# lukifer23/Matrix0

Hardware: AMD Instinct MI355X
Metric: self-play games/sec at 800 sims/move, ResNet-24 53M; 1/2/4/8 MI355X (higher is better)
Workload: dtype f16

## Files before the change

### include/m0_engine.h

```cpp
#ifndef M0_ENGINE_H
#define M0_ENGINE_H

#include <stdint.h>

#ifdef __cplusplus
extern "C" {
#endif

#define M0_OK 0
#define M0_ERR_INVALID (-1)
#define M0_ERR_UNSUPPORTED (-2)
#define M0_ERR_HIP (-3)
#define M0_ERR_STATE (-4)
#define M0_ERR_NONFINITE (-5)

#define M0_POLICY_SIZE 4672
#define M0_PLANES 19

#define M0_ACT_RELU 1
#define M0_ACT_SILU 2
#define M0_ACT_LEAKY 3

#define M0_SSL_PIECE 1
#define M0_SSL_THREAT 2
#define M0_SSL_PIN 4
#define M0_SSL_FORK 8
#define M0_SSL_CONTROL 16

typedef struct m0_net_cfg {
    int planes;
    int channels;
    int blocks;
    int attention;
    int attention_heads;
    int attention_every_k;
    int attention_relbias;
    float attention_unmasked_mix;
    int se;
    float se_ratio;
    int chess_features;
    int piece_square_tables;
    int policy_factor_rank;
    int norm_group;
    int activation;
    int value_activation;
    int preact;
    int self_supervised;
    int ssl_tasks;
    int infer_attention_stride;
} m0_net_cfg;

typedef struct m0_net m0_net;

const char* m0_last_error(void);
const char* m0_version(void);
int m0_device_count(void);

m0_net* m0_net_create(const m0_net_cfg* cfg, int hip_device);
void m0_net_destroy(m0_net* net);
int m0_net_load_weight(m0_net* net, const char* name, const void* data, int dtype, const int64_t* shape, int ndim);
int m0_net_finalize(m0_net* net);
int m0_net_infer(m0_net* net, const float* planes, int B, float* policy, float* value, float* ssl);
int m0_net_ssl_channels(const m0_net* net);
int64_t m0_net_param_count(const m0_net* net);
double m0_net_flops_per_position(const m0_net* net, int with_ssl);
int m0_net_bench_forward(m0_net* net, int B, int iters, int with_ssl, float* ms_per_forward);
int m0_net_profile_enable(m0_net* net, int on);
int m0_net_profile_get(m0_net* net, double* conv_ms, double* conv_flop, int64_t* launches, int reset);
int m0_net_profile_get_tail(m0_net* net, double* tail_ms, int64_t* tail_launches);


typedef struct m0_dist m0_dist;
int m0_dist_unique_id(void* id128);
m0_dist* m0_dist_create(int rank, int world, const void* id128, int hip_device);
void m0_dist_destroy(m0_dist* d);
int m0_dist_rank(const m0_dist* d);
int m0_dist_world(const m0_dist* d);
int m0_net_broadcast_weights(m0_net* net, m0_dist* d, int root);

int m0_encode_fens(int hip_device, const char* const* fens, int n, float* planes, uint8_t* mask, int32_t* nlegal,
                   uint16_t* moves, int32_t* idx);
int m0_encode_fens_nhwc(int hip_device, const char* const* fens, int n, uint16_t* nhwc);
int m0_decode_move_fen(int hip_device, const char* fen, int action_idx, char* uci_out);
int m0_ssl_targets_fens(int hip_device, const char* const* fens, int n, float* out);
int m0_move_to_index_fen(int hip_device, const char* fen, const char* uci, int32_t* idx);

typedef struct m0_selfplay_cfg {
    int num_simulations;
    double cpuct, cpuct_start, cpuct_end;
    int cpuct_plies;
    int use_c_base; double cpuct_c_base, cpuct_c_init;
    double dirichlet_alpha, dirichlet_frac;
    int dirichlet_plies;
    double selection_jitter, fpu_reduction, draw_penalty, virtual_loss;
    int legal_softmax, enable_entropy_noise, no_instant_backtrack, value_from_white;
    int inference_batch_size;
    double playout_random_frac;
    int max_game_len, min_resign_plies, opening_random_plies;
    double resign_threshold; int resign_window, resign_consecutive_bad; double resign_min_entropy, resign_value_margin;
    double temperature_start, temperature_end; int temperature_moves;
    int low_visit_threshold;
    int draw_enabled, draw_min_plies, draw_window, draw_min_unique, draw_halfmove_cap, draw_material_threshold, draw_stalemate;
    int concurrent_games;
    int total_games;
    int first_game_index;
    int arena_nodes;
    uint64_t seed;
    int virtual_loss_active;
    int ssl_in_forward;
    int ssl_targets;
    int record_games;
    int arena_mode;
    double arena_temp;
    int arena_temp_plies;
    int fresh_tree_per_move;
    int tt_merge;
    int raw_legal_priors;
    int max_children;
    double min_child_prior;
    int root_reinfer;
    int eval_cache;
    int eval_cache_entries;
    int tail_split;
    int arena_eval_cache;
    int arena_paired_openings;
} m0_selfplay_cfg;

typedef struct m0_selfplay m0_selfplay;

typedef struct m0_selfplay_stats {
    uint64_t steps, evals, sims, plies, games_finished, games_started;
    double ms_total, ms_net, ms_tree, ms_host;
    uint64_t arena_overflows;
    uint64_t ssl_dropped;
    uint64_t evals_cached;
    int active_games;
    uint64_t rows_tail;
} m0_selfplay_stats;

typedef struct m0_game_record {
    int game_index, moves, resigned, resigner , draw, total_plies ;
    float result;
    float avg_policy_entropy, avg_sims;
    double secs;
    const float* s;
    const float* pi;
    const float* z;
    const uint8_t* legal_mask;
    const float* search_values;
    const uint16_t* played;
    const float* ssl;
    void* owner;
    const char* start_fen;
} m0_game_record;

m0_selfplay* m0_selfplay_create(m0_net* net, const m0_selfplay_cfg* cfg);
void m0_selfplay_destroy(m0_selfplay* sp);
int m0_selfplay_step(m0_selfplay* sp, int steps);
int m0_selfplay_stats_get(m0_selfplay* sp, m0_selfplay_stats* out);
int m0_selfplay_poll(m0_selfplay* sp, m0_game_record* out);
void m0_game_record_free(m0_game_record* rec);
int m0_selfplay_running(m0_selfplay* sp);
int m0_selfplay_set_openings(m0_selfplay* sp, const char* const* fens, int n);
int m0_selfplay_ext_select(m0_selfplay* sp, int* rows, float* planes, int max_rows);
int m0_selfplay_ext_expand(m0_selfplay* sp, const float* logits, const float* values, int rows);
int m0_selfplay_last_batch_nhwc(m0_selfplay* sp, uint16_t* nhwc, int max_rows, int* rows);

m0_selfplay* m0_arena_create(m0_net* net_a, m0_net* net_b, const m0_selfplay_cfg* cfg);
m0_selfplay* m0_arena_create_ext(const m0_selfplay_cfg* cfg);
int m0_arena_ext_select(m0_selfplay* sp, int* rows_a, int* rows_b, float* planes_a, float* planes_b, int max_rows);
int m0_arena_ext_expand(m0_selfplay* sp, const float* logits_a, const float* values_a, int rows_a, const float* logits_b,
                        const float* values_b, int rows_b);
int m0_arena_choose_move(const int32_t* visits, int n, double temp, int ply, int temp_plies, double u);
int m0_san_legal_fen(const char* fen, uint16_t* moves, char* san, int* nlegal);
int m0_san_game(const uint16_t* moves, int n, char* out, int cap);
int m0_san_game_fen(const char* fen, const uint16_t* moves, int n, char* out, int cap);
int m0_fen_after(const char* fen, const char* const* ucis, int n, char* fen_out, int cap);

int m0_search_begin(m0_selfplay* sp, int g, const char* fen, int sims, int dirichlet, int game_uid);
int m0_search_select(m0_selfplay* sp, int* rows, float* planes, int max_rows);
int m0_search_expand(m0_selfplay* sp, const float* logits, const float* values, int rows);
int m0_search_result(m0_selfplay* sp, int g, int* nchild, int32_t* child_n, uint16_t* child_mv, int32_t* child_idx,
                     double* child_prior, double* child_q, double* root_q, int* root_n, int* finished);
int m0_search_advance(m0_selfplay* sp, int g, int slot, int sims, int dirichlet);

int m0_sample_move_index(const int32_t* visits, int n, double temperature, double u);
int m0_playout_cap(int sims, double frac, double u);
double m0_temperature_for(int fullmove_number, double t_start, double t_end, int t_moves);
int m0_rules_probe(const m0_selfplay_cfg* cfg, const char* fen, const char* const* ucis, int n, int* flags, float* result);

#ifdef __cplusplus
}
#endif
#endif
```

### matrix0_amd/csrc/capi_net.hip

```cpp
#include <hip/hip_runtime.h>
#include <math.h>
#include <string.h>
#include <mutex>
#include <string>
#include <vector>
#include "../../include/m0_engine.h"
#include "net.h"
#include "capi_common.h"

thread_local std::string g_m0_last_error;

void m0_set_error(const std::string& s) { g_m0_last_error = s; }

struct m0_net {
    Net* net = nullptr;
    int device = 0;
    hipStream_t stream = nullptr;
    std::mutex mu;
    float* planes_dev = nullptr;
    float* logits_dev = nullptr;
    float* value_dev = nullptr;
    float* ssl_dev = nullptr;
    int cap = 0;
};

Net* m0_net_impl(m0_net* n) { return n ? n->net : nullptr; }
hipStream_t m0_net_stream(m0_net* n) { return n ? n->stream : nullptr; }
int m0_net_device(m0_net* n) { return n ? n->device : 0; }
void m0_net_lock(m0_net* n) { if (n) n->mu.lock(); }
void m0_net_unlock(m0_net* n) { if (n) n->mu.unlock(); }

hipError_t create_stream_cu_mask_env(const char* env_name, hipStream_t* stream) {
    const char* mk = getenv(env_name);
    if (!mk || !*mk) return hipStreamCreateWithFlags(stream, hipStreamNonBlocking);
    uint32_t words[8] = {0, 0, 0, 0, 0, 0, 0, 0};
    int nw = 0;
    for (const char* q = mk; *q && nw < 8; ++nw) {
        char* end = nullptr;
        words[nw] = (uint32_t)strtoul(q, &end, 16);
        if (end == q) break;
        q = (*end == ',') ? end + 1 : end;
    }
    return hipExtStreamCreateWithCUMask(stream, 8, words);
}

extern "C" {

const char* m0_last_error(void) { return g_m0_last_error.c_str(); }
const char* m0_version(void) { return "m0engine 0.2 (gfx950)"; }
int m0_device_count(void) {
    int n = 0;
    if (hipGetDeviceCount(&n) != hipSuccess) { (void)hipGetLastError(); return 0; }
    return n;
}

m0_net* m0_net_create(const m0_net_cfg* cfg, int hip_device) {
    if (!cfg) { m0_set_error("cfg is null"); return nullptr; }
    const char* why = Net::check_supported(*cfg);
    if (why) { m0_set_error(std::string("unsupported network config: ") + why); return nullptr; }
    int ndev = 0;
    if (hipGetDeviceCount(&ndev) != hipSuccess || ndev <= 0) {
        m0_set_error("no HIP device available (the engine has no CPU fallback)");
        return nullptr;
    }
    if (hip_device < 0 || hip_device >= ndev) { m0_set_error("hip_device out of range"); return nullptr; }
    if (hipSetDevice(hip_device) != hipSuccess) { m0_set_error("hipSetDevice failed"); return nullptr; }
    m0_net* h = new m0_net();
    h->device = hip_device;
    const hipError_t se = create_stream_cu_mask_env("M0_NET_CU_MASK", &h->stream);
    if (se != hipSuccess) {
        m0_set_error("hipStreamCreate failed");
        delete h;
        return nullptr;
    }
    h->net = new Net(*cfg, hip_device, h->stream);
    return h;
}

void m0_net_destroy(m0_net* n) {
    if (!n) return;
    (void)hipSetDevice(n->device);
    if (n->stream) { (void)hipStreamSynchronize(n->stream); }
    if (n->planes_dev) (void)hipFree(n->planes_dev);
    if (n->logits_dev) (void)hipFree(n->logits_dev);
    if (n->value_dev) (void)hipFree(n->value_dev);
    if (n->ssl_dev) (void)hipFree(n->ssl_dev);
    delete n->net;
    if (n->stream) (void)hipStreamDestroy(n->stream);
    delete n;
}

int m0_net_load_weight(m0_net* n, const char* name, const void* data, int dtype, const int64_t* shape, int ndim) {
    if (!n) { m0_set_error("net is null"); return M0_ERR_INVALID; }
    std::lock_guard<std::mutex> lk(n->mu);
    std::string err;
    int rc = n->net->load(name, data, dtype, shape, ndim, err);
    if (rc != M0_OK) m0_set_error(err);
    return rc;
}

int m0_net_finalize(m0_net* n) {
    if (!n) { m0_set_error("net is null"); return M0_ERR_INVALID; }
    std::lock_guard<std::mutex> lk(n->mu);
    std::string err;
    int rc = n->net->finalize(err);
    if (rc != M0_OK) m0_set_error(err);
    return rc;
}

static int ensure_io(m0_net* n, int B) {
    if (B <= n->cap) return M0_OK;
    if (n->planes_dev) (void)hipFree(n->planes_dev);
    if (n->logits_dev) (void)hipFree(n->logits_dev);
    if (n->value_dev) (void)hipFree(n->value_dev);
    if (n->ssl_dev) (void)hipFree(n->ssl_dev);
    n->planes_dev = n->logits_dev = n->value_dev = n->ssl_dev = nullptr;
    n->cap = 0;
    int cap = B < 64 ? 64 : B;
    const int P = n->net->cfg().planes;
    int sslc = n->net->ssl_channels_total();
    if (hipMalloc((void**)&n->planes_dev, (size_t)cap * P * 64 * 4) != hipSuccess ||
        hipMalloc((void**)&n->logits_dev, (size_t)cap * M0_POLICY_SIZE * 4) != hipSuccess ||
        hipMalloc((void**)&n->value_dev, (size_t)cap * 4) != hipSuccess ||
        hipMalloc((void**)&n->ssl_dev, (size_t)cap * (sslc > 0 ? sslc : 1) * 64 * 4) != hipSuccess) {
        m0_set_error("hipMalloc failed for I/O staging");
        return M0_ERR_HIP;
    }
    n->cap = cap;
    return M0_OK;
}

int m0_net_infer(m0_net* n, const float* planes, int B, float* policy, float* value, float* ssl) {
    if (!n || !planes || !policy || !value) { m0_set_error("null argument"); return M0_ERR_INVALID; }
    if (B <= 0) { m0_set_error("batch must be positive"); return M0_ERR_INVALID; }
    std::lock_guard<std::mutex> lk(n->mu);
    if (hipSetDevice(n->device) != hipSuccess) { m0_set_error("hipSetDevice failed"); return M0_ERR_HIP; }
    int rc = ensure_io(n, B);
    if (rc != M0_OK) return rc;
    const int P = n->net->cfg().planes;
    const int sslc = n->net->ssl_channels_total();
    if (ssl && sslc == 0) { m0_set_error("ssl output requested but the net has no SSL heads"); return M0_ERR_INVALID; }
    std::string err;
    hipError_t e = hipMemcpyAsync(n->planes_dev, planes, (size_t)B * P * 64 * 4, hipMemcpyHostToDevice, n->stream);
    if (e != hipSuccess) { m0_set_error(std::string("H2D copy: ") + hipGetErrorString(e)); return M0_ERR_HIP; }
    rc = n->net->forward(n->planes_dev, nullptr, B, n->logits_dev, n->value_dev, ssl ? n->ssl_dev : nullptr, n->stream, err);
    if (rc != M0_OK) { m0_set_error(err); return rc; }
    (void)hipMemcpyAsync(policy, n->logits_dev, (size_t)B * M0_POLICY_SIZE * 4, hipMemcpyDeviceToHost, n->stream);
    (void)hipMemcpyAsync(value, n->value_dev, (size_t)B * 4, hipMemcpyDeviceToHost, n->stream);
    if (ssl) (void)hipMemcpyAsync(ssl, n->ssl_dev, (size_t)B * sslc * 64 * 4, hipMemcpyDeviceToHost, n->stream);
    e = hipStreamSynchronize(n->stream);
    if (e != hipSuccess) { m0_set_error(std::string("forward failed: ") + hipGetErrorString(e)); return M0_ERR_HIP; }
    for (size_t i = 0, nn = (size_t)B * M0_POLICY_SIZE; i < nn; ++i)
        if (!isfinite(policy[i])) { m0_set_error("network produced non-finite policy logits"); return M0_ERR_NONFINITE; }
    for (int i = 0; i < B; ++i)
        if (!isfinite(value[i])) { m0_set_error("network produced non-finite value"); return M0_ERR_NONFINITE; }
    return M0_OK;
}

int m0_net_ssl_channels(const m0_net* n) { return n ? n->net->ssl_channels_total() : 0; }
int64_t m0_net_param_count(const m0_net* n) { return n ? (int64_t)n->net->param_count() : 0; }
double m0_net_flops_per_position(const m0_net* n, int with_ssl) { return n ? n->net->flops_per_position(with_ssl != 0) : 0.0; }

int m0_net_profile_enable(m0_net* n, int on) {
    if (!n) { m0_set_error("net is null"); return M0_ERR_INVALID; }
    std::lock_guard<std::mutex> lk(n->mu);
    n->net->set_profile(on != 0);
    return M0_OK;
}

int m0_net_profile_get(m0_net* n, double* conv_ms, double* conv_flop, int64_t* launches, int reset) {
    if (!n) { m0_set_error("net is null"); return M0_ERR_INVALID; }
    std::lock_guard<std::mutex> lk(n->mu);
    if (conv_ms) *conv_ms = n->net->prof_conv_ms();
    if (conv_flop) *conv_flop = n->net->prof_conv_flop();
    if (launches) *launches = n->net->prof_conv_launches();
    if (reset) n->net->reset_profile();
    return M0_OK;
}

int m0_net_profile_get_tail(m0_net* n, double* tail_ms, int64_t* tail_launches) {
    if (!n) { m0_set_error("net is null"); return M0_ERR_INVALID; }
    std::lock_guard<std::mutex> lk(n->mu);
    if (tail_ms) *tail_ms = n->net->prof_tail_ms();
    if (tail_launches) *tail_launches = n->net->prof_tail_launches();
    return M0_OK;
}

int m0_net_bench_forward(m0_net* n, int B, int iters, int with_ssl, float* ms_per_forward) {
    if (!n || !ms_per_forward || B <= 0 || iters <= 0) { m0_set_error("invalid argument"); return M0_ERR_INVALID; }
    std::lock_guard<std::mutex> lk(n->mu);
    if (hipSetDevice(n->device) != hipSuccess) { m0_set_error("hipSetDevice failed"); return M0_ERR_HIP; }
    int rc = ensure_io(n, B);
    if (rc != M0_OK) return rc;
    std::string err;
    if (!(with_ssl & 2)) {
        const int P = n->net->cfg().planes;
        std::vector<float> h((size_t)B * P * 64, 0.f);
        uint64_t s = 0x9E3779B97F4A7C15ull;
        for (size_t i = 0; i < h.size(); ++i) {
            s ^= s << 13; s ^= s >> 7; s ^= s << 17;
            int p = (int)((i / 64) % P);
            if (p < 12) h[i] = ((s >> 20) % 100) < 8 ? 1.f : 0.f;
            else h[i] = (float)((((i / 64 / P) * 7 + p) % 10) / 10.0);
        }
        (void)hipMemcpy(n->planes_dev, h.data(), h.size() * 4, hipMemcpyHostToDevice);
    }
    float* ssl = ((with_ssl & 1) && n->net->ssl_channels_total() > 0) ? n->ssl_dev : nullptr;
    rc = n->net->forward(n->planes_dev, nullptr, B, n->logits_dev, n->value_dev, ssl, n->stream, err);
    if (rc != M0_OK) { m0_set_error(err); return rc; }
    hipEvent_t e0, e1;
    (void)hipEventCreate(&e0); (void)hipEventCreate(&e1);
    (void)hipEventRecord(e0, n->stream);
    for (int i = 0; i < iters; ++i) {
        rc = n->net->forward(n->planes_dev, nullptr, B, n->logits_dev, n->value_dev, ssl, n->stream, err);
        if (rc != M0_OK) { m0_set_error(err); return rc; }
    }
    (void)hipEventRecord(e1, n->stream);
    hipError_t e = hipEventSynchronize(e1);
    if (e != hipSuccess) { m0_set_error(std::string("bench forward failed: ") + hipGetErrorString(e)); return M0_ERR_HIP; }
    float ms = 0.f;
    (void)hipEventElapsedTime(&ms, e0, e1);
    (void)hipEventDestroy(e0); (void)hipEventDestroy(e1);
    *ms_per_forward = ms / iters;
    n->net->harvest_profile();
    return M0_OK;
}

}
```

### matrix0_amd/csrc/capi_selfplay.hip

```cpp
#include <string.h>
#include <algorithm>
#include <memory>
#include "selfplay_engine.h"

using namespace m0;

static void fill_tree_cfg(const m0_selfplay_cfg& c, bool arena, TreeCfg& t) {
    t.fpu_reduction = c.fpu_reduction; t.draw_penalty = c.draw_penalty; t.virtual_loss = c.virtual_loss;
    t.selection_jitter = c.selection_jitter; t.cpuct = c.cpuct; t.cpuct_start = c.cpuct_start; t.cpuct_end = c.cpuct_end;
    t.cpuct_plies = c.cpuct_plies; t.use_c_base = c.use_c_base; t.cpuct_c_base = c.cpuct_c_base; t.cpuct_c_init = c.cpuct_c_init;
    t.dirichlet_alpha = c.dirichlet_alpha; t.dirichlet_frac = c.dirichlet_frac; t.legal_softmax = c.legal_softmax;
    t.enable_entropy_noise = c.enable_entropy_noise; t.no_instant_backtrack = c.no_instant_backtrack;
    t.virtual_loss_active = c.virtual_loss_active; t.leaves_per_step = c.inference_batch_size;
    t.tt_merge = c.tt_merge; t.raw_legal_priors = c.raw_legal_priors; t.max_children = c.max_children;
    t.min_child_prior = c.min_child_prior;
    t.eval_cache = ((arena ? c.arena_eval_cache : c.eval_cache) && c.legal_softmax && !c.raw_legal_priors && !c.tt_merge) ? 1 : 0;
}

static void alloc_tree_arenas(m0_selfplay* sp) {
    const m0_selfplay_cfg& c = sp->cfg;
    long want = c.arena_nodes > 0 ? c.arena_nodes : (long)(c.num_simulations * 1.3 + 64) * 96;
    if (want < 4096) want = 4096;
    sp->cap = (int)want;
    const size_t N = (size_t)sp->G * 2 * sp->cap;
    TreeArrays& t = sp->d.t;
    t.cap = sp->cap;
    t.prior = dalloc<double>(sp, N); t.w = dalloc<double>(sp, N); t.q = dalloc<double>(sp, N);
    t.n = dalloc<int>(sp, N); t.vl = dalloc<int>(sp, N); t.cbase = dalloc<int>(sp, N);
    t.nch = dalloc<int16_t>(sp, N); t.mv = dalloc<uint16_t>(sp, N); t.midx = dalloc<uint16_t>(sp, N);
    sp->d.games = dalloc<GameDev>(sp, sp->G);
    const size_t LS = (size_t)sp->L + 1;
    sp->d.samples = dalloc<Sample>(sp, (size_t)sp->G * LS);
    sp->d.paths = dalloc<int>(sp, (size_t)sp->G * LS * M0_MAX_DEPTH);
    sp->d.leaf_moves = dalloc<uint16_t>(sp, (size_t)sp->G * LS * M0_MAX_CHILDREN);
}

static bool alloc_position_tables(m0_selfplay* sp) {
    sp->d.tt_sides = 1;
    if (!sp->cfg.tt_merge) return true;
    const size_t LS = (size_t)sp->L + 1;
    int tc = 1024;
    while (tc < 2 * sp->cap) tc <<= 1;
    sp->d.tt_cap = tc;
    sp->d.tt_sides = sp->cfg.arena_mode ? 2 : 1;
    sp->d.search_nodes = (int)std::min<long>((long)sp->cfg.num_simulations * 48 + 4 * M0_MAX_CHILDREN, (long)sp->cap / 2);
    sp->d.epaths = dalloc<int>(sp, (size_t)sp->G * LS * M0_MAX_DEPTH);
    sp->d.tt_keys = dalloc<uint64_t>(sp, (size_t)sp->G * sp->d.tt_sides * tc);
    sp->d.tt_nodes = dalloc<int>(sp, (size_t)sp->G * sp->d.tt_sides * tc);
    if (sp->d.epaths && sp->d.tt_keys && sp->d.tt_nodes) return true;
    m0_set_error("hipMalloc failed for the position tables (tt_merge): lower concurrent_games or arena_nodes");
    return false;
}

static bool alloc_eval_cache(m0_selfplay* sp) {
    if (!sp->tc.eval_cache) return true;
    const size_t LS = (size_t)sp->L + 1;
    int entries = sp->cfg.eval_cache_entries > 0 ? sp->cfg.eval_cache_entries : 16384;
    int sets = 64;
    while (sets * 4 < entries) sets <<= 1;
    EvalCache& ec = sp->d.ec;
    ec.sets = sets;
    ec.sides = sp->cfg.arena_mode ? 2 : 1;
    const size_t entries_all = (size_t)sp->G * ec.sides * sets * 4;
    ec.keys = dalloc<uint64_t>(sp, entries_all);
    ec.stamps = dalloc<uint32_t>(sp, entries_all);
    ec.payload = dalloc<float>(sp, entries_all * M0_EC_WORDS);
    ec.hit_stage = dalloc<float>(sp, (size_t)sp->G * LS * M0_EC_WORDS);
    if (ec.keys && ec.stamps && ec.payload && ec.hit_stage) return true;
    m0_set_error("hipMalloc failed for the evaluation cache: lower eval_cache_entries or concurrent_games");
    return false;
}

static bool alloc_batch_buffers(m0_selfplay* sp) {
    const int nreg = sp->cfg.arena_mode ? 2 : 1;
    sp->d.hist = dalloc<uint64_t>(sp, (size_t)sp->G * M0_HIST_CAP);
    sp->d.results = dalloc<RootResult>(sp, sp->G);
    sp->d.row_counter = dalloc<int>(sp, 4);
    sp->d.x0 = dalloc<_Float16>(sp, (size_t)(nreg * sp->rows_max + 4) * 64 * 32);
    sp->logits_dev = dalloc<float>(sp, (size_t)nreg * sp->rows_max * 4672);
    sp->values_dev = dalloc<float>(sp, (size_t)nreg * sp->rows_max + 4);
    sp->d.net_row_base = sp->rows_max;
    if (sp->cfg.ssl_in_forward && sp->net && sp->net->ssl_channels_total() > 0)
        sp->ssl_dev = dalloc<float>(sp, (size_t)sp->rows_max * sp->net->ssl_channels_total() * 64);
    if (sp->cfg.ssl_targets) {
        sp->ssl_cap = sp->cfg.max_game_len > 0 ? sp->cfg.max_game_len + 1 : 513;
        sp->ssl_pos_dev = dalloc<Pos>(sp, sp->ssl_cap);
        sp->ssl_out_dev = dalloc<float>(sp, (size_t)sp->ssl_cap * 17 * 64);
        if (!sp->ssl_pos_dev || !sp->ssl_out_dev) {
            m0_set_error("hipMalloc failed for the SSL target staging buffers");
            return false;
        }
    }
    sp->ids_dev = dalloc<int>(sp, sp->G);
    sp->slots_dev = dalloc<int>(sp, sp->G);
    sp->d.logits = sp->logits_dev; sp->d.values = sp->values_dev;
    sp->d.G = sp->G; sp->d.L = sp->L;
    return true;
}

static bool make_tail_view(m0_selfplay* sp) {
    if (!(sp->cfg.tail_split && sp->net && !sp->cfg.arena_mode && sp->net->cfg().channels > 256 && sp->net->cfg().channels <= 320 &&
          sp->rows_max >= 2048)) return true;
    if (create_stream_cu_mask_env("M0_TAIL_CU_MASK", &sp->stream_tail) != hipSuccess ||
        hipEventCreateWithFlags(&sp->ev_sel, hipEventDisableTiming) != hipSuccess ||
        hipEventCreateWithFlags(&sp->ev_tail, hipEventDisableTiming) != hipSuccess) {
        m0_set_error("hipStreamCreate / hipEventCreate failed (tail split)");
        return false;
    }
    sp->net_tail = sp->net->shared_view(sp->stream_tail);
    std::string werr;
    sp->half_split = sp->cfg.tail_split == 2;
    if (sp->net_tail->ensure_workspace(sp->half_split ? sp->rows_max / 2 + 1024 : 1023, werr) != M0_OK) {
        m0_set_error("tail split: " + werr);
        return false;
    }
    return true;
}

static bool build_engine(m0_selfplay* sp) {
    alloc_tree_arenas(sp);
    if (!alloc_position_tables(sp) || !alloc_eval_cache(sp) || !alloc_batch_buffers(sp)) return false;
    if (sp->alloc_failed) {
        m0_set_error("hipMalloc failed for the search arenas (lower concurrent_games or arena_nodes)");
        return false;
    }
    sp->hg.assign(sp->G, GameDev());
    for (auto& g : sp->hg) memset(&g, 0, sizeof(GameDev));
    sp->games.assign(sp->G, HostGame());
    sp->hres.resize(sp->G);
    sp->hsamples.resize((size_t)sp->G * (sp->L + 1));
    sp->prev_done.assign(sp->G, 0);
    (void)hipEventCreate(&sp->ev0); (void)hipEventCreate(&sp->ev1); (void)hipEventCreate(&sp->ev2); (void)hipEventCreate(&sp->ev3);
    if (!make_tail_view(sp)) return false;
    std::string err;
    if (sp->net && sp->net->ensure_workspace(sp->rows_max, err) != M0_OK) { m0_set_error(err); return false; }
    if (sp->net && sp->net_b && sp->net_b->ensure_workspace(sp->rows_max, err) != M0_OK) { m0_set_error(err); return false; }
    if (hipStreamSynchronize(sp->stream) != hipSuccess) {
        m0_set_error(std::string("clearing the search arenas failed: ") + hipGetErrorString(hipGetLastError()));
        return false;
    }
    return true;
}

extern "C" {

static m0_selfplay* selfplay_create_impl(m0_net* nh, m0_net* nh_b, const m0_selfplay_cfg* cfg, bool arena = false) {
    if (!cfg) { m0_set_error("cfg is null"); return nullptr; }
    if (cfg->concurrent_games <= 0 || cfg->inference_batch_size <= 0 || cfg->num_simulations <= 0) {
        m0_set_error("concurrent_games, inference_batch_size and num_simulations must be positive");
        return nullptr;
    }
    int ndev = 0;
    if (hipGetDeviceCount(&ndev) != hipSuccess || ndev <= 0) { m0_set_error("no HIP device available (no CPU fallback)"); return nullptr; }
    std::unique_ptr<m0_selfplay, decltype(&m0_selfplay_destroy)> owner(new m0_selfplay(), &m0_selfplay_destroy);
    m0_selfplay* sp = owner.get();
    sp->cfg = *cfg;
    sp->nethandle = nh;
    sp->nethandle_b = nh_b;
    sp->net = m0_net_impl(nh);
    sp->net_b = m0_net_impl(nh_b);
    sp->cfg.arena_mode = (nh_b || arena) ? 1 : 0;
    if (sp->cfg.arena_mode) sp->cfg.eval_cache = 0;
    else { sp->cfg.arena_eval_cache = 0; sp->cfg.arena_paired_openings = 0; }
    fill_tree_cfg(sp->cfg, sp->cfg.arena_mode != 0, sp->tc);
    sp->device = nh ? m0_net_device(nh) : 0;
    if (nh) forward_gate_join(sp);
    (void)hipSetDevice(sp->device);
    if (nh) sp->stream = m0_net_stream(nh);
    else { (void)hipStreamCreateWithFlags(&sp->stream, hipStreamNonBlocking); sp->own_stream = true; }
    sp->G = cfg->concurrent_games;
    sp->L = cfg->inference_batch_size;
    sp->rows_max = (sp->G * (sp->L + 1) + 3) & ~3;
    memset(&sp->stats, 0, sizeof(sp->stats));
    memset(&sp->d, 0, sizeof(sp->d));
    return build_engine(sp) ? owner.release() : nullptr;
}

m0_selfplay* m0_selfplay_create(m0_net* nh, const m0_selfplay_cfg* cfg) { return selfplay_create_impl(nh, nullptr, cfg); }

m0_selfplay* m0_arena_create(m0_net* net_a, m0_net* net_b, const m0_selfplay_cfg* cfg) {
    if (!net_a || !net_b) { m0_set_error("m0_arena_create needs two networks"); return nullptr; }
    if (m0_net_device(net_a) != m0_net_device(net_b)) { m0_set_error("both networks must live on the same HIP device"); return nullptr; }
    if (cfg && (cfg->ssl_in_forward || cfg->ssl_targets)) { m0_set_error("arena games carry no SSL outputs"); return nullptr; }
    return selfplay_create_impl(net_a, net_b, cfg);
}

m0_selfplay* m0_arena_create_ext(const m0_selfplay_cfg* cfg) {
    if (cfg && (cfg->ssl_in_forward || cfg->ssl_targets)) { m0_set_error("arena games carry no SSL outputs"); return nullptr; }
    return selfplay_create_impl(nullptr, nullptr, cfg, true);
}

void m0_selfplay_destroy(m0_selfplay* sp) {
    if (!sp) return;
    forward_gate_leave(sp);
    (void)hipSetDevice(sp->device);
    if (sp->stream) (void)hipStreamSynchronize(sp->stream);
    if (sp->stream_tail) (void)hipStreamSynchronize(sp->stream_tail);
    delete sp->net_tail;
    if (sp->ev_sel) (void)hipEventDestroy(sp->ev_sel);
    if (sp->ev_tail) (void)hipEventDestroy(sp->ev_tail);
    if (sp->stream_tail) (void)hipStreamDestroy(sp->stream_tail);
    for (void* p : sp->allocs) (void)hipFree(p);
    for (auto& r : sp->done_meta) delete (GameRecordOwner*)r.owner;
    if (sp->ev0) { (void)hipEventDestroy(sp->ev0); (void)hipEventDestroy(sp->ev1); (void)hipEventDestroy(sp->ev2); (void)hipEventDestroy(sp->ev3); }
    if (sp->own_stream && sp->stream) (void)hipStreamDestroy(sp->stream);
    delete sp;
}

int m0_selfplay_set_openings(m0_selfplay* sp, const char* const* fens, int n) {
    if (!sp || n < 0 || (n > 0 && !fens)) { m0_set_error("invalid argument"); return M0_ERR_INVALID; }
    std::lock_guard<std::mutex> lk(sp->mu);
    if (sp->stats.games_started != 0) { m0_set_error("set the opening book before the first step"); return M0_ERR_STATE; }
    std::vector<Pos> book(n);
    for (int i = 0; i < n; ++i)
        if (!fens[i] || parse_fen(fens[i], book[i]) != 0) { m0_set_error(std::string("bad FEN at index ") + std::to_string(i)); return M0_ERR_INVALID; }
    sp->book.swap(book);
    sp->book_fens.assign(fens, fens + n);
    return M0_OK;
}

static int leaf_planes(m0_selfplay* sp, int rows_a, float* planes_a, int rows_b, float* planes_b) {
    if (sync_games_d2h(sp) != 0) { m0_set_error("device sync failed"); return M0_ERR_HIP; }
    (void)hipMemcpy(sp->hsamples.data(), sp->d.samples, sizeof(Sample) * (size_t)sp->G * (sp->L + 1), hipMemcpyDeviceToHost);
    const int base = sp->d.net_row_base;
    for (int g = 0; g < sp->G; ++g) {
        if (!sp->hg[g].active) continue;
        for (int s = 0; s < sp->hg[g].nsamples; ++s) {
            const Sample& smp = sp->hsamples[(size_t)g * (sp->L + 1) + s];
            if (!sample_owns_row(smp.kind) || smp.row < 0) continue;
            if (smp.row < rows_a) encode_planes_f32(smp.pos, planes_a + (size_t)smp.row * 19 * 64);
            else if (smp.row >= base && smp.row < base + rows_b) encode_planes_f32(smp.pos, planes_b + (size_t)(smp.row - base) * 19 * 64);
        }
    }
    return M0_OK;
}

static void upload_eval(m0_selfplay* sp, size_t row_base, const float* logits, const float* values, int rows) {
    if (rows <= 0) return;
    (void)hipMemcpyAsync(sp->logits_dev + row_base * 4672, logits, (size_t)rows * 4672 * 4, hipMemcpyHostToDevice, sp->stream);
    (void)hipMemcpyAsync(sp->values_dev + row_base, values, (size_t)rows * 4, hipMemcpyHostToDevice, sp->stream);
}

static int ext_select_impl(m0_selfplay* sp, int* rows_a, int* rows_b, float* planes_a, float* planes_b, int max_rows) {
    (void)hipSetDevice(sp->device);
    if (sp->ext_pending) { m0_set_error("m0_selfplay_ext_expand outstanding"); return M0_ERR_STATE; }
    if (!planes_a || (sp->cfg.arena_mode && !planes_b) || max_rows < sp->G * (sp->L + 1)) {
        m0_set_error("planes buffer too small: concurrent_games * (inference_batch_size + 1) rows are required");
        return M0_ERR_INVALID;
    }
    int rc = start_first_games(sp);
    if (rc != M0_OK) return rc;
    int r = 0;
    if (run_select(sp, &r) != 0) { m0_set_error(std::string("select failed: ") + hipGetErrorString(hipGetLastError())); return M0_ERR_HIP; }
    const int rb = sp->cfg.arena_mode ? sp->rows2[1] : 0;
    if (r > sp->rows_max || rb > sp->rows_max) { m0_set_error("row counter overflow"); return M0_ERR_STATE; }
    *rows_a = r;
    if (rows_b) *rows_b = rb;
    sp->last_rows = r;
    sp->last_rows_b = rb;
    sp->ext_pending = true;
    if (r + rb > 0) return leaf_planes(sp, r, planes_a, rb, planes_b);
    return M0_OK;
}

static int ext_expand_impl(m0_selfplay* sp, const float* logits_a, const float* values_a, int rows_a, const float* logits_b,
                           const float* values_b, int rows_b) {
    (void)hipSetDevice(sp->device);
    if (!sp->ext_pending) { m0_set_error("no m0_selfplay_ext_select outstanding"); return M0_ERR_STATE; }
    if (rows_a != sp->last_rows || rows_b != sp->last_rows_b) { m0_set_error("rows does not match the last select"); return M0_ERR_INVALID; }
    if ((rows_a > 0 && (!logits_a || !values_a)) || (rows_b > 0 && (!logits_b || !values_b))) { m0_set_error("null argument"); return M0_ERR_INVALID; }
    upload_eval(sp, 0, logits_a, values_a, rows_a);
    upload_eval(sp, (size_t)sp->d.net_row_base, logits_b, values_b, rows_b);
    sp->ext_pending = false;
    std::string err;
    (void)hipEventRecord(sp->ev0, sp->stream); (void)hipEventRecord(sp->ev1, sp->stream);
    int rc = step_back(sp, rows_a + rows_b, now_ms(), err);
    if (rc != M0_OK) m0_set_error(err);
    return rc;
}

int m0_selfplay_ext_select(m0_selfplay* sp, int* rows, float* planes, int max_rows) {
    if (!sp || !rows) { m0_set_error("null argument"); return M0_ERR_INVALID; }
    std::lock_guard<std::mutex> lk(sp->mu);
    if (sp->cfg.arena_mode) { m0_set_error("a match engine has two evaluators: use m0_arena_ext_select"); return M0_ERR_STATE; }
    return ext_select_impl(sp, rows, nullptr, planes, nullptr, max_rows);
}

int m0_selfplay_ext_expand(m0_selfplay* sp, const float* logits, const float* values, int rows) {
    if (!sp) { m0_set_error("null argument"); return M0_ERR_INVALID; }
    std::lock_guard<std::mutex> lk(sp->mu);
    if (sp->cfg.arena_mode) { m0_set_error("a match engine has two evaluators: use m0_arena_ext_expand"); return M0_ERR_STATE; }
    return ext_expand_impl(sp, logits, values, rows, nullptr, nullptr, 0);
}

int m0_arena_ext_select(m0_selfplay* sp, int* rows_a, int* rows_b, float* planes_a, float* planes_b, int max_rows) {
    if (!sp || !rows_a || !rows_b) { m0_set_error("null argument"); return M0_ERR_INVALID; }
    std::lock_guard<std::mutex> lk(sp->mu);
    if (!sp->cfg.arena_mode) { m0_set_error("not a match engine"); return M0_ERR_STATE; }
    return ext_select_impl(sp, rows_a, rows_b, planes_a, planes_b, max_rows);
}

int m0_arena_ext_expand(m0_selfplay* sp, const float* logits_a, const float* values_a, int rows_a, const float* logits_b,
                        const float* values_b, int rows_b) {
    if (!sp) { m0_set_error("null argument"); return M0_ERR_INVALID; }
    std::lock_guard<std::mutex> lk(sp->mu);
    if (!sp->cfg.arena_mode) { m0_set_error("not a match engine"); return M0_ERR_STATE; }
    return ext_expand_impl(sp, logits_a, values_a, rows_a, logits_b, values_b, rows_b);
}

int m0_selfplay_step(m0_selfplay* sp, int steps) {
    if (!sp) { m0_set_error("sp is null"); return M0_ERR_INVALID; }
    std::lock_guard<std::mutex> lk(sp->mu);
    (void)hipSetDevice(sp->device);
    std::string err;
    if (sp->ext_pending) { m0_set_error("m0_selfplay_ext_expand outstanding"); return M0_ERR_STATE; }
    { int rc0 = start_first_games(sp); if (rc0 != M0_OK) return rc0; }
    for (int i = 0; i < steps; ++i) {
        if (sp->stats.active_games == 0 && sp->stats.steps > 0) break;
        int rc = one_step(sp, err);
        if (rc != M0_OK) { m0_set_error(err); return rc; }
    }
    return M0_OK;
}

int m0_selfplay_stats_get(m0_selfplay* sp, m0_selfplay_stats* out) {
    if (!sp || !out) { m0_set_error("null argument"); return M0_ERR_INVALID; }
    std::lock_guard<std::mutex> lk(sp->mu);
    *out = sp->stats;
    return M0_OK;
}

int m0_selfplay_poll(m0_selfplay* sp, m0_game_record* out) {
    if (!sp || !out) { m0_set_error("null argument"); return M0_ERR_INVALID; }
    std::lock_guard<std::mutex> lk(sp->mu);
    if (sp->done_meta.empty()) return 0;
    *out = sp->done_meta.front();
    sp->done_meta.pop_front();
    return 1;
}

void m0_game_record_free(m0_game_record* rec) {
    if (rec && rec->owner) { delete (GameRecordOwner*)rec->owner; rec->owner = nullptr; }
}

int m0_selfplay_running(m0_selfplay* sp) {
    if (!sp) return 0;
    std::lock_guard<std::mutex> lk(sp->mu);
    if (sp->stats.games_started == 0) return 1;
    if (sp->stats.active_games > 0) return 1;
    return (sp->cfg.total_games <= 0 || sp->next_game < sp->cfg.total_games) ? 1 : 0;
}

int m0_search_begin(m0_selfplay* sp, int g, const char* fen, int sims, int dirichlet, int game_uid) {
    if (!sp || !fen || g < 0 || g >= sp->G || sims <= 0) { m0_set_error("invalid argument"); return M0_ERR_INVALID; }
    std::lock_guard<std::mutex> lk(sp->mu);
    (void)hipSetDevice(sp->device);
    Pos p;
    if (parse_fen(fen, p) != 0) { m0_set_error("bad FEN"); return M0_ERR_INVALID; }
    if (sync_games_d2h(sp) != 0) { m0_set_error("device sync failed"); return M0_ERR_HIP; }
    HostGame& hgm = sp->games[g];
    hgm = HostGame();
    hgm.in_use = true; hgm.pos = p; hgm.game_index = game_uid;
    seed_game_dev(sp->hg[g], sp->cfg.seed, game_uid);
    sp->hg[g].evals = 0;
    arm_search(sp, g, p, hgm.win, sims, dirichlet != 0, true);
    std::vector<int> ids{g}, slots{-1};
    if (apply_advances(sp, ids, slots) != 0) { m0_set_error("advance failed"); return M0_ERR_HIP; }
    return M0_OK;
}

int m0_search_select(m0_selfplay* sp, int* rows, float* planes, int max_rows) {
    if (!sp || !rows) { m0_set_error("null argument"); return M0_ERR_INVALID; }
    std::lock_guard<std::mutex> lk(sp->mu);
    (void)hipSetDevice(sp->device);
    int r = 0;
    if (run_select(sp, &r) != 0) { m0_set_error(std::string("select failed: ") + hipGetErrorString(hipGetLastError())); return M0_ERR_HIP; }
    *rows = r;
    sp->last_rows = r;
    if (planes && r > 0) {
        if (r > max_rows) { m0_set_error("planes buffer too small"); return M0_ERR_INVALID; }
        return leaf_planes(sp, r, planes, 0, nullptr);
    }
    return M0_OK;
}

int m0_search_expand(m0_selfplay* sp, const float* logits, const float* values, int rows) {
    if (!sp) { m0_set_error("null argument"); return M0_ERR_INVALID; }
    std::lock_guard<std::mutex> lk(sp->mu);
    (void)hipSetDevice(sp->device);
    if (rows != sp->last_rows || rows > sp->rows_max) { m0_set_error("rows does not match the last select"); return M0_ERR_INVALID; }
    if (rows > 0 && (!logits || !values)) { m0_set_error("null argument"); return M0_ERR_INVALID; }
    upload_eval(sp, 0, logits, values, rows);
    if (launch_expand(sp->d, sp->tc, sp->stream) != hipSuccess) { m0_set_error("expand launch failed"); return M0_ERR_HIP; }
    if (sync_games_d2h(sp) != 0) { m0_set_error(std::string("expand failed: ") + hipGetErrorString(hipGetLastError())); return M0_ERR_HIP; }
    sp->stats.evals += (uint64_t)rows;
    return M0_OK;
}

int m0_search_result(m0_selfplay* sp, int g, int* nchild, int32_t* child_n, uint16_t* child_mv, int32_t* child_idx,
                     double* child_prior, double* child_q, double* root_q, int* root_n, int* finished) {
    if (!sp || g < 0 || g >= sp->G) { m0_set_error("invalid argument"); return M0_ERR_INVALID; }
    std::lock_guard<std::mutex> lk(sp->mu);
    (void)hipSetDevice(sp->device);
    if (finished) *finished = sp->hg[g].finished;
    if (!sp->hg[g].finished) { if (nchild) *nchild = 0; return M0_OK; }
    (void)hipMemcpy(&sp->hres[g], sp->d.results + g, sizeof(RootResult), hipMemcpyDeviceToHost);
    const RootResult& R = sp->hres[g];
    if (nchild) *nchild = R.nchild;
    for (int i = 0; i < R.nchild; ++i) {
        if (child_n) child_n[i] = R.child_n[i];
        if (child_mv) child_mv[i] = R.child_mv[i];
        if (child_idx) child_idx[i] = R.child_idx[i];
        if (child_prior) child_prior[i] = R.child_prior[i];
        if (child_q) child_q[i] = R.child_q[i];
    }
    if (root_q) *root_q = R.root_n > 0 ? R.root_q : sp->hg[g].root_v;
    if (root_n) *root_n = R.root_n;
    return M0_OK;
}

int m0_search_advance(m0_selfplay* sp, int g, int slot, int sims, int dirichlet) {
    if (!sp || g < 0 || g >= sp->G || sims <= 0) { m0_set_error("invalid argument"); return M0_ERR_INVALID; }
    std::lock_guard<std::mutex> lk(sp->mu);
    (void)hipSetDevice(sp->device);
    if (sync_games_d2h(sp) != 0) { m0_set_error("device sync failed"); return M0_ERR_HIP; }
    if (!sp->hg[g].finished) { m0_set_error("search not finished"); return M0_ERR_STATE; }
    (void)hipMemcpy(&sp->hres[g], sp->d.results + g, sizeof(RootResult), hipMemcpyDeviceToHost);
    const RootResult& R = sp->hres[g];
    if (slot < 0 || slot >= R.nchild) { m0_set_error("child slot out of range"); return M0_ERR_INVALID; }
    HostGame& hgm = sp->games[g];
    hgm.play(R.child_mv[slot]);
    const bool fresh = sp->cfg.fresh_tree_per_move || sp->cfg.tt_merge;
    arm_search(sp, g, hgm.pos, hgm.win, sims, dirichlet != 0, fresh);
    std::vector<int> ids{g}, slots{fresh ? -1 : slot};
    if (apply_advances(sp, ids, slots) != 0) { m0_set_error("advance failed"); return M0_ERR_HIP; }
    return M0_OK;
}

int m0_selfplay_last_batch_nhwc(m0_selfplay* sp, uint16_t* out, int max_rows, int* rows) {
    if (!sp || !out || !rows) { m0_set_error("null argument"); return M0_ERR_INVALID; }
    std::lock_guard<std::mutex> lk(sp->mu);
    (void)hipSetDevice(sp->device);
    const int r = sp->last_rows;
    if (r > max_rows) { m0_set_error("output buffer too small"); return M0_ERR_INVALID; }
    *rows = r;
    if (r > 0) {
        if (hipMemcpyAsync(out, sp->d.x0, (size_t)r * 64 * 32 * 2, hipMemcpyDeviceToHost, sp->stream) != hipSuccess ||
            hipStreamSynchronize(sp->stream) != hipSuccess) { m0_set_error("copy failed"); return M0_ERR_HIP; }
    }
    return M0_OK;
}

}
```

### matrix0_amd/csrc/net.h

```cpp
#pragma once
#include <hip/hip_runtime.h>
#include <stdint.h>
#include <map>
#include <string>
#include <vector>
#include "../../include/m0_engine.h"
#include "net_kernels.h"

struct HostTensor {
    std::vector<float> data;
    std::vector<int64_t> shape;
};

struct PackedGemm {
    _Float16* w = nullptr;
    float* bias = nullptr;
    int taps = 1, Cin = 0, N = 0;
    bool pp = false;
};

struct NormParams {
    float* gamma = nullptr;
    float* beta = nullptr;
};

struct ResBlockW {
    PackedGemm conv1, conv2;
    NormParams bn1, bn2;
    float *se_w1 = nullptr, *se_b1 = nullptr, *se_w2 = nullptr, *se_b2 = nullptr;
    void* se_wf = nullptr;
    int se_hidden = 0;
};

struct AttnW {
    PackedGemm qkv, proj;
    NormParams ln;
    float* rel_bias = nullptr;
    void* blk_w = nullptr;
    _Float16* blk_bias = nullptr;
};

struct TowerLayer {
    int kind;
    int index;
    bool skip;
    int next_bn1 = -1;
};

struct SslHeadW {
    PackedGemm c0, c1;
    NormParams n;
    int out_ch = 0;
};

struct ConvNormOpts {
    const float* posenc = nullptr;
    const _Float16* res = nullptr;
    const NormParams* next_bn1 = nullptr;
};

class Net {
public:
    explicit Net(const m0_net_cfg& cfg, int device, hipStream_t stream);
    ~Net();
    Net* shared_view(hipStream_t stream) const;
    static const char* check_supported(const m0_net_cfg& cfg);
    int load(const char* name, const void* data, int dtype, const int64_t* shape, int ndim, std::string& err);
    int finalize(std::string& err);
    bool ready() const { return finalized_; }
    const std::vector<void*>& device_buffers() const { return dev_allocs_; }
    const std::vector<size_t>& device_buffer_bytes() const { return dev_sizes_; }

    int forward(const float* planes_dev, const _Float16* nhwc_dev, int B, float* logits_dev, float* value_dev,
                float* ssl_dev, hipStream_t st, std::string& err);
    int ensure_workspace(int B, std::string& err);
    int ssl_channels_total() const;
    const m0_net_cfg& cfg() const { return cfg_; }
    size_t param_count() const { return nparams_; }
    double flops_per_position(bool with_ssl) const;
    _Float16* input_nhwc() { return X0_; }
    void set_profile(bool on) { profile_ = on; }
    void harvest_profile();
    double prof_conv_ms() const { return prof_ms_; }
    double prof_conv_flop() const { return prof_flop_; }
    long prof_conv_launches() const { return prof_launches_; }
    void reset_profile() { prof_ms_ = 0; prof_flop_ = 0; prof_launches_ = 0; prof_tail_ms_ = 0; prof_tail_launches_ = 0; }
    double prof_tail_ms() const { return prof_tail_ms_; }
    long prof_tail_launches() const { return prof_tail_launches_; }

private:
    m0_net_cfg cfg_;
    int device_;
    hipStream_t stream_ = nullptr;
    struct Switches { bool fuse_tail = true, fuse_attn = true; } sw_;
    struct Plan {
        bool fuse_tail = false;
        bool fuse_attn = false;
        bool gn_small = false;
        int act = 0, vact = 0;
        int first_bn1 = -1;
    } plan_;
    bool finalized_ = false;
    size_t nparams_ = 0;
    std::map<std::string, HostTensor> sd_;
    std::vector<void*> dev_allocs_;
    std::vector<size_t> dev_sizes_;
    std::vector<void*> ws_allocs_;

    int C_ = 0, Cs_ = 0 ;
    int Cp_ = 0;
    PackedGemm stem_;
    NormParams stem_n_;
    float* posenc_ = nullptr;
    PackedGemm pst_, inter_;
    NormParams pst_n_, inter_n_;
    std::vector<ResBlockW> res_;
    std::vector<AttnW> att_;
    std::vector<TowerLayer> tower_;
    PackedGemm ph_conv_, pfc1_, pfc2_;
    PackedGemm hv_;
    NormParams hv_n_;
    NormParams ph_n_;
    float logit_scale_ = 1.f;
    PackedGemm vh0_, vh3_, vfc1_, vfc2_, vgate_, vfc3_;
    NormParams vh1_n_, vh4_n_;
    std::vector<SslHeadW> ssl_;
    uint64_t* mask_dev_ = nullptr;

    bool profile_ = false;
    std::vector<hipEvent_t> pev_;
    std::vector<double> pflop_;
    std::vector<char> ptail_;
    size_t pev_used_ = 0;
    double prof_ms_ = 0, prof_flop_ = 0, prof_tail_ms_ = 0;
    long prof_launches_ = 0, prof_tail_launches_ = 0;

    int wsB_ = 0, wsM_ = 0;
    _Float16 *X0_ = nullptr, *XA_ = nullptr, *XB_ = nullptr, *T1_ = nullptr, *T2_ = nullptr, *QKV_ = nullptr,
             *O_ = nullptr, *AA_ = nullptr;
    float *S1_ = nullptr, *S2_ = nullptr, *G_ = nullptr;
    _Float16 *PH_ = nullptr, *PH2_ = nullptr, *VH_ = nullptr, *VH2_ = nullptr, *F1_ = nullptr, *F2_ = nullptr,
             *F3_ = nullptr, *F4_ = nullptr, *SH_ = nullptr, *SH2_ = nullptr, *SO_ = nullptr;
    float* VAL_ = nullptr;
    float* SPK_ = nullptr;

    const HostTensor* get(const std::string& k, std::string& err);
    int pack_gemm(PackedGemm& g, const std::string& wkey, const std::string& bkey, int taps, int Cin_real,
                  int Cin_pad, int N_real, int N_pad, int k_perm_ch, std::string& err, int qkv_heads = 0,
                  int qkv_heads_pad = 0);
    int pack_attn_block(AttnW& a, const std::string& prefix, std::string& err);
    int pack_chess_features(std::string& err);
    int pack_se(ResBlockW& r, const std::string& prefix, std::string& err);
    int pack_attn(AttnW& a, bool skip, const std::string& prefix, std::string& err);
    void upload_attn_mask();
    int pack_joint_head(std::string& err);
    int pack_ssl_heads(std::string& err);
    void make_plan();
    int upload_norm(NormParams& n, const std::string& prefix, int C_real, int C_pad, std::string& err);
    float* upload_f32(const std::vector<float>& v);
    void* dalloc(size_t bytes, bool ws);
    const NormParams* bn1(int res_index) const { return res_index < 0 ? nullptr : &res_[res_index].bn1; }
    template <class Launch>
    hipError_t profiled(bool on, hipStream_t st, double flop, bool tail, Launch&& launch);
    hipError_t run_gemm(const PackedGemm& g, GemmArgs a, hipStream_t st);
    hipError_t conv_norm_act(const PackedGemm& g, const NormParams& n, const _Float16* in, _Float16* out, _Float16* scratch,
                             int Mrows, hipStream_t st, const ConvNormOpts& o = ConvNormOpts());
    hipError_t se_gate(const ResBlockW& r, const float* stats, int boards, hipStream_t st);
};
```

### matrix0_amd/csrc/net.hip

```cpp
#include "net.h"
#include <math.h>
#include <string.h>
#include <algorithm>
#include <stdlib.h>

static inline int ceil_to(int v, int m) { return (v + m - 1) / m * m; }

static const char* kSslNames[5] = {"piece", "threat", "pin", "fork", "control"};
static const int kSslOut[5] = {13, 1, 1, 1, 3};

const char* Net::check_supported(const m0_net_cfg& c) {
    if (!c.norm_group) return "HIP path supports norm='group' only (BatchNorm configs are not built)";
    if (!c.preact) return "HIP path supports preact=true only";
    if (c.channels % 32 != 0 || c.channels < 32 || c.channels > 384) return "channels must be a multiple of 32 in [32,384]";
    if (c.planes < 1 || c.planes > 32) return "planes must be in [1,32]";
    if (c.attention && (c.attention_heads <= 0 || c.channels % c.attention_heads != 0 ||
                        c.channels / c.attention_heads != 16))
        return "attention head_dim (channels/attention_heads) must be 16";
    if (c.activation != M0_ACT_SILU && c.activation != M0_ACT_RELU) return "activation must be silu or relu";
    if (c.blocks < 1) return "blocks must be >= 1";
    if (c.policy_factor_rank < 0) return "policy_factor_rank must be >= 0";
    if (c.self_supervised && c.ssl_tasks && (c.channels / 2) % 16 != 0) return "ssl heads need channels/2 % 16 == 0";
    return nullptr;
}

Net::Net(const m0_net_cfg& cfg, int device, hipStream_t stream) : cfg_(cfg), device_(device), stream_(stream) {
    auto off = [](const char* name) { const char* e = getenv(name); return e && e[0] == '0'; };
    sw_.fuse_tail = !off("M0_FUSE_TAIL");
    sw_.fuse_attn = !off("M0_FUSE_ATTN");
    C_ = cfg.channels;
    Cp_ = (C_ > 256 && C_ < 320) ? 320 : C_;
    Cs_ = ceil_to(std::max(16, C_ / 2), 32);
    int k = cfg.attention_every_k;
    int stride = std::max(1, cfg.infer_attention_stride);
    int att_seen = 0;
    for (int i = 0; i < cfg.blocks; ++i) {
        tower_.push_back({0, (int)res_.size(), false});
        res_.emplace_back();
        if (cfg.attention && k > 0 && (i % k) == (k - 1)) {
            ++att_seen;
            bool skip = stride > 1 && (att_seen % stride) != 0;
            tower_.push_back({1, (int)att_.size(), skip});
            att_.emplace_back();
        }
    }
}

Net* Net::shared_view(hipStream_t stream) const {
    Net* v = new Net(*this);
    v->stream_ = stream;
    v->dev_allocs_.clear(); v->dev_sizes_.clear();
    v->ws_allocs_.clear(); v->wsB_ = 0; v->wsM_ = 0;
    v->sd_.clear();
    v->pev_.clear(); v->pflop_.clear(); v->ptail_.clear(); v->pev_used_ = 0; v->profile_ = false;
    v->prof_ms_ = v->prof_flop_ = v->prof_tail_ms_ = 0; v->prof_launches_ = v->prof_tail_launches_ = 0;
    return v;
}

Net::~Net() {
    for (hipEvent_t e : pev_) (void)hipEventDestroy(e);
    for (void* p : dev_allocs_) (void)hipFree(p);
    for (void* p : ws_allocs_) (void)hipFree(p);
}

void* Net::dalloc(size_t bytes, bool ws) {
    void* p = nullptr;
    if (bytes == 0) bytes = 16;
    if (hipMalloc(&p, bytes) != hipSuccess) return nullptr;
    (void)hipMemsetAsync(p, 0, bytes, stream_);
    if (!ws) (void)hipStreamSynchronize(stream_);
    (ws ? ws_allocs_ : dev_allocs_).push_back(p);
    if (!ws) dev_sizes_.push_back(bytes);
    return p;
}

float* Net::upload_f32(const std::vector<float>& v) {
    float* d = (float*)dalloc(v.size() * 4, false);
    if (d && !v.empty()) (void)hipMemcpy(d, v.data(), v.size() * 4, hipMemcpyHostToDevice);
    return d;
}

int Net::load(const char* name, const void* data, int dtype, const int64_t* shape, int ndim, std::string& err) {
    if (finalized_) { err = "weights already finalized"; return M0_ERR_STATE; }
    if (!name || (!data && ndim >= 0)) { err = "null argument"; return M0_ERR_INVALID; }
    HostTensor t;
    size_t n = 1;
    for (int i = 0; i < ndim; ++i) { t.shape.push_back(shape[i]); n *= (size_t)shape[i]; }
    t.data.resize(n);
    if (dtype == 0) memcpy(t.data.data(), data, n * 4);
    else if (dtype == 1) {
        const _Float16* h = (const _Float16*)data;
        for (size_t i = 0; i < n; ++i) t.data[i] = (float)h[i];
    } else { err = "dtype must be 0 (f32) or 1 (f16)"; return M0_ERR_INVALID; }
    std::string key(name);
    if (cfg_.policy_factor_rank > 0 && key.rfind("policy_fc.", 0) == 0) key = "policy_fc1." + key.substr(10);
    sd_[key] = std::move(t);
    return M0_OK;
}

const HostTensor* Net::get(const std::string& k, std::string& err) {
    auto it = sd_.find(k);
    if (it == sd_.end()) { err = "missing state-dict key: " + k; return nullptr; }
    return &it->second;
}

int Net::pack_gemm(PackedGemm& g, const std::string& wkey, const std::string& bkey, int taps, int Cin_real,
                   int Cin_pad, int N_real, int N_pad, int k_perm_ch, std::string& err, int qkv_heads, int qkv_heads_pad) {
    const HostTensor* w = get(wkey, err);
    if (!w) return M0_ERR_INVALID;
    size_t expect = (size_t)N_real * Cin_real * taps;
    if (w->data.size() != expect) { err = "shape mismatch for " + wkey; return M0_ERR_INVALID; }
    nparams_ += expect;
    const int KC = conv_gemm_kc(Cin_pad, N_pad);
    const int nchunk = Cin_pad / KC;
    const bool pp = KC == 64 && taps == 9;
    const int nblk = N_pad / 320;
    std::vector<_Float16> p((size_t)taps * Cin_pad * N_pad, (_Float16)0.f);
    for (int nr = 0; nr < N_real; ++nr)
        for (int k = 0; k < Cin_real; ++k)
            for (int t = 0; t < taps; ++t) {
                float v = w->data[((size_t)nr * Cin_real + k) * taps + t];
                int n = nr;
                if (qkv_heads > 0) {
                    const int d = nr % 16, th = nr / 16, hh = th % qkv_heads, tt = th / qkv_heads;
                    n = (tt * qkv_heads_pad + hh) * 16 + d;
                }
                int kk = k;
                if (k_perm_ch > 0) {
                    int c = k / 64, sq = k % 64;
                    kk = sq * k_perm_ch + c;
                }
                int chunk = kk / KC, kc = kk % KC;
                if (pp) {
                    const int kt = chunk * 9 + t, by = n / 320, nl = n % 320, h = kc >> 5, k32 = kc & 31;
                    const int kx = (((k32 >> 3) ^ ((4 - ((nl >> 2) & 3)) & 3)) << 3) | (k32 & 7);
                    p[((((size_t)kt * nblk + by) * 2 + h) * 320 + nl) * 32 + kx] = (_Float16)v;
                    continue;
                }
                if (KC == 64)
                    kc = (((kc >> 3) ^ ((n >> 1) & 7)) << 3) | (kc & 7);
                p[(((size_t)t * nchunk + chunk) * N_pad + n) * KC + kc] = (_Float16)v;
            }
    g.w = (_Float16*)dalloc(p.size() * 2, false);
    if (!g.w) { err = "hipMalloc failed"; return M0_ERR_HIP; }
    (void)hipMemcpy(g.w, p.data(), p.size() * 2, hipMemcpyHostToDevice);
    g.taps = taps; g.Cin = Cin_pad; g.N = N_pad; g.pp = pp;
    g.bias = nullptr;
    if (!bkey.empty()) {
        const HostTensor* b = get(bkey, err);
        if (!b) return M0_ERR_INVALID;
        if ((int)b->data.size() != N_real) { err = "shape mismatch for " + bkey; return M0_ERR_INVALID; }
        nparams_ += N_real;
        std::vector<float> bp(N_pad, 0.f);
        std::copy(b->data.begin(), b->data.end(), bp.begin());
        g.bias = upload_f32(bp);
    }
    return M0_OK;
}

int Net::pack_attn_block(AttnW& a, const std::string& prefix, std::string& err) {
    const HostTensor* wq = get(prefix + ".qkv.weight", err); if (!wq) return M0_ERR_INVALID;
    const HostTensor* wp = get(prefix + ".proj.weight", err); if (!wp) return M0_ERR_INVALID;
    const int Cr = C_, Hr = cfg_.attention_heads;
    if (Cp_ != 320 || Cr != Hr * 16 || wq->data.size() != (size_t)3 * Cr * Cr || wp->data.size() != (size_t)Cr * Cr) {
        err = "shape mismatch for " + prefix; return M0_ERR_INVALID;
    }
    std::vector<_Float16> buf(attn_block_pack_bytes() / 2, (_Float16)0.f);
    auto qkv_w = [&](int type, int h, int d, int k) -> float {
        return (h < Hr && k < Cr) ? wq->data[(size_t)((type * Hr + h) * 16 + d) * Cr + k] : 0.f;
    };
    auto proj_w = [&](int oc, int h, int d) -> float {
        return (oc < Cr && h < Hr) ? wp->data[(size_t)oc * Cr + h * 16 + d] : 0.f;
    };
    for (int g = 0; g < 10; ++g) {
        for (int pc = 0; pc < 5; ++pc) {
            const size_t base = (size_t)(g * 7 + pc) * 6144;
            for (int col = 0; col < 96; ++col) {
                const int J = col >> 4, type = J >> 1, hl = J & 1, d = col & 15;
                for (int k = 0; k < 64; ++k) {
                    const int pos = (k >> 3) ^ ((col >> 1) & 7);
                    buf[base + (size_t)col * 64 + pos * 8 + (k & 7)] = (_Float16)qkv_w(type, 2 * g + hl, d, 64 * pc + k);
                }
            }
        }
        for (int hh = 0; hh < 2; ++hh) {
            const size_t base = (size_t)(g * 7 + 5 + hh) * 6144;
            for (int cl = 0; cl < 160; ++cl)
                for (int k = 0; k < 32; ++k) {
                    const int pos = (k >> 3) ^ ((4 - ((cl >> 2) & 3)) & 3);
                    buf[base + (size_t)cl * 32 + pos * 8 + (k & 7)] = (_Float16)proj_w(160 * hh + cl, 2 * g + (k >> 4), k & 15);
                }
        }
    }
    a.blk_w = dalloc(buf.size() * 2, false);
    if (!a.blk_w) { err = "hipMalloc failed"; return M0_ERR_HIP; }
    (void)hipMemcpy(a.blk_w, buf.data(), buf.size() * 2, hipMemcpyHostToDevice);
    std::vector<_Float16> bb((size_t)20 * 2 * 64 * 32, (_Float16)0.f);
    if (cfg_.attention_relbias) {
        const HostTensor* rb = get(prefix + ".rel_bias", err); if (!rb) return M0_ERR_INVALID;
        for (int h = 0; h < Hr; ++h)
            for (int qt = 0; qt < 2; ++qt)
                for (int lane = 0; lane < 64; ++lane)
                    for (int e = 0; e < 32; ++e) {
                        const int kt = e >> 4, r = e & 15;
                        const int q = qt * 32 + (lane & 31), key = kt * 32 + 8 * (r >> 2) + 4 * (lane >> 5) + (r & 3);
                        bb[(((size_t)h * 2 + qt) * 64 + lane) * 32 + e] =
                            (_Float16)(rb->data[((size_t)h * 64 + q) * 64 + key] * 1.44269504088896f);
                    }
    }
    a.blk_bias = (_Float16*)dalloc(bb.size() * 2, false);
    if (!a.blk_bias) { err = "hipMalloc failed"; return M0_ERR_HIP; }
    (void)hipMemcpy(a.blk_bias, bb.data(), bb.size() * 2, hipMemcpyHostToDevice);
    return M0_OK;
}

int Net::upload_norm(NormParams& n, const std::string& prefix, int C_real, int C_pad, std::string& err) {
    const HostTensor* g = get(prefix + ".weight", err);
    if (!g) return M0_ERR_INVALID;
    const HostTensor* b = get(prefix + ".bias", err);
    if (!b) return M0_ERR_INVALID;
    if ((int)g->data.size() != C_real || (int)b->data.size() != C_real) { err = "shape mismatch for " + prefix; return M0_ERR_INVALID; }
    nparams_ += 2 * (size_t)C_real;
    std::vector<float> gp(C_pad, 0.f), bp(C_pad, 0.f);
    std::copy(g->data.begin(), g->data.end(), gp.begin());
    std::copy(b->data.begin(), b->data.end(), bp.begin());
    n.gamma = upload_f32(gp);
    n.beta = upload_f32(bp);
    return M0_OK;
}

#define TRY(x) do { int rc_ = (x); if (rc_ != M0_OK) return rc_; } while (0)

int Net::pack_chess_features(std::string& err) {
    const int C = C_, P = Cp_;
    const HostTensor* pe = get("chess_features.position_encoding", err);
    if (!pe) return M0_ERR_INVALID;
    if ((int)pe->data.size() != C * 64) { err = "shape mismatch for position_encoding"; return M0_ERR_INVALID; }
    nparams_ += pe->data.size();
    std::vector<float> t((size_t)64 * P, 0.f);
    for (int c = 0; c < C; ++c)
        for (int n = 0; n < 64; ++n) t[(size_t)n * P + c] = pe->data[(size_t)c * 64 + n];
    posenc_ = upload_f32(t);
    if (cfg_.piece_square_tables) {
        TRY(pack_gemm(pst_, "chess_features.pst_conv.weight", "", 1, C, P, C, P, 0, err));
        TRY(upload_norm(pst_n_, "chess_features.pst_norm", C, P, err));
    }
    TRY(pack_gemm(inter_, "chess_features.interaction_conv.weight", "", 9, C, P, C, P, 0, err));
    return upload_norm(inter_n_, "chess_features.interaction_norm", C, P, err);
}

int Net::pack_se(ResBlockW& r, const std::string& p, std::string& err) {
    const int C = C_, P = Cp_;
    const int hd = std::max(8, (int)(C * cfg_.se_ratio));
    r.se_hidden = hd;
    const HostTensor* w1 = get(p + ".se_fc1.weight", err); if (!w1) return M0_ERR_INVALID;
    const HostTensor* b1 = get(p + ".se_fc1.bias", err); if (!b1) return M0_ERR_INVALID;
    const HostTensor* w2 = get(p + ".se_fc2.weight", err); if (!w2) return M0_ERR_INVALID;
    const HostTensor* b2 = get(p + ".se_fc2.bias", err); if (!b2) return M0_ERR_INVALID;
    if ((int)w1->data.size() != hd * C || (int)w2->data.size() != hd * C || (int)b1->data.size() != hd ||
        (int)b2->data.size() != C) { err = "shape mismatch for " + p + ".se_*"; return M0_ERR_INVALID; }
    nparams_ += (size_t)2 * hd * C + hd + C;
    std::vector<float> w1t((size_t)P * hd, 0.f);
    for (int j = 0; j < hd; ++j)
        for (int c = 0; c < C; ++c) w1t[(size_t)c * hd + j] = w1->data[(size_t)j * C + c];
    r.se_w1 = upload_f32(w1t);
    r.se_b1 = upload_f32(b1->data);
    std::vector<float> w2t((size_t)hd * P, 0.f);
    for (int c = 0; c < C; ++c)
        for (int j = 0; j < hd; ++j) w2t[(size_t)j * P + c] = w2->data[(size_t)c * hd + j];
    r.se_w2 = upload_f32(w2t);
    if (P == 320 && hd <= TAIL_SE_HMAX) {
        const int NT1 = (hd + 15) / 16, KS2 = (hd + 31) / 32;
        std::vector<_Float16> wf((size_t)(10 * NT1 + 20 * KS2) * 512, (_Float16)0.f);
        for (int nt = 0; nt < NT1; ++nt)
            for (int ks = 0; ks < 10; ++ks)
                for (int l = 0; l < 64; ++l)
                    for (int e = 0; e < 8; ++e) {
                        const int c = 32 * ks + 8 * (l >> 4) + e, j = 16 * nt + (l & 15);
                        if (j < hd) wf[((size_t)(nt * 10 + ks) * 64 + l) * 8 + e] = (_Float16)w1t[(size_t)c * hd + j];
                    }
        for (int nt = 0; nt < 20; ++nt)
            for (int ks = 0; ks < KS2; ++ks)
                for (int l = 0; l < 64; ++l)
                    for (int e = 0; e < 8; ++e) {
                        const int j = 32 * ks + 8 * (l >> 4) + e, c = 16 * nt + (l & 15);
                        if (j < hd) wf[((size_t)(10 * NT1 + nt * KS2 + ks) * 64 + l) * 8 + e] = (_Float16)w2t[(size_t)j * P + c];
                    }
        r.se_wf = dalloc(wf.size() * 2, false);
        if (!r.se_wf) { err = "hipMalloc failed"; return M0_ERR_HIP; }
        (void)hipMemcpy(r.se_wf, wf.data(), wf.size() * 2, hipMemcpyHostToDevice);
    }
    std::vector<float> b2p(P, 0.f);
    std::copy(b2->data.begin(), b2->data.end(), b2p.begin());
    r.se_b2 = upload_f32(b2p);
    return M0_OK;
}

int Net::pack_attn(AttnW& a, bool skip, const std::string& p, std::string& err) {
    const int C = C_, P = Cp_;
    if (skip) {
        for (const char* k : {".qkv.weight", ".proj.weight", ".norm.weight", ".norm.bias", ".rel_bias"}) {
            auto it = sd_.find(p + k);
            if (it != sd_.end()) nparams_ += it->second.data.size();
        }
        return M0_OK;
    }
    TRY(pack_gemm(a.qkv, p + ".qkv.weight", "", 1, C, P, 3 * C, 3 * P, 0, err, P != C ? cfg_.attention_heads : 0, P / 16));
    TRY(pack_gemm(a.proj, p + ".proj.weight", "", 1, C, P, C, P, 0, err));
    TRY(upload_norm(a.ln, p + ".norm", C, P, err));
    if (P == 320) TRY(pack_attn_block(a, p, err));
    if (cfg_.attention_relbias) {
        const HostTensor* rb = get(p + ".rel_bias", err); if (!rb) return M0_ERR_INVALID;
        if ((int)rb->data.size() != cfg_.attention_heads * 4096) { err = "shape mismatch for rel_bias"; return M0_ERR_INVALID; }
        nparams_ += rb->data.size();
        std::vector<float> rbs((size_t)(P / 16) * 4096, 0.f);
        for (size_t i = 0; i < rb->data.size(); ++i) rbs[i] = rb->data[i] * 1.44269504088896f;
        a.rel_bias = upload_f32(rbs);
    }
    return M0_OK;
}

void Net::upload_attn_mask() {
    std::vector<uint64_t> m(64, 0);
    for (int i = 0; i < 64; ++i)
        for (int j = 0; j < 64; ++j) {
            int dr = i / 8 - j / 8, dc = i % 8 - j % 8;
            int adr = abs(dr), adc = abs(dc);
            bool vis = dr == 0 || dc == 0 || adr == adc || (adr == 2 && adc == 1) || (adr == 1 && adc == 2) ||
                       (adr <= 1 && adc <= 1);
            if (vis) m[i] |= (1ull << j);
        }
    mask_dev_ = (uint64_t*)dalloc(64 * 8, false);
    (void)hipMemcpy(mask_dev_, m.data(), 64 * 8, hipMemcpyHostToDevice);
}

int Net::pack_joint_head(std::string& err) {
    const int nch = Cp_ / 32;
    std::vector<_Float16> a((size_t)nch * 64 * 32), b((size_t)nch * 128 * 32), c((size_t)nch * 192 * 32);
    (void)hipMemcpy(a.data(), ph_conv_.w, a.size() * 2, hipMemcpyDeviceToHost);
    (void)hipMemcpy(b.data(), vh0_.w, b.size() * 2, hipMemcpyDeviceToHost);
    for (int ch = 0; ch < nch; ++ch) {
        std::copy(a.begin() + (size_t)ch * 64 * 32, a.begin() + (size_t)(ch + 1) * 64 * 32, c.begin() + (size_t)ch * 192 * 32);
        std::copy(b.begin() + (size_t)ch * 128 * 32, b.begin() + (size_t)(ch + 1) * 128 * 32, c.begin() + ((size_t)ch * 192 + 64) * 32);
    }
    hv_.w = (_Float16*)dalloc(c.size() * 2, false);
    if (!hv_.w) { err = "hipMalloc failed"; return M0_ERR_HIP; }
    (void)hipMemcpy(hv_.w, c.data(), c.size() * 2, hipMemcpyHostToDevice);
    hv_.taps = 1; hv_.Cin = Cp_; hv_.N = 192; hv_.pp = false; hv_.bias = nullptr;
    std::vector<float> g(192), be(192);
    (void)hipMemcpy(g.data(), ph_n_.gamma, 64 * 4, hipMemcpyDeviceToHost);
    (void)hipMemcpy(g.data() + 64, vh1_n_.gamma, 128 * 4, hipMemcpyDeviceToHost);
    (void)hipMemcpy(be.data(), ph_n_.beta, 64 * 4, hipMemcpyDeviceToHost);
    (void)hipMemcpy(be.data() + 64, vh1_n_.beta, 128 * 4, hipMemcpyDeviceToHost);
    hv_n_.gamma = upload_f32(g); hv_n_.beta = upload_f32(be);
    if (!hv_n_.gamma || !hv_n_.beta) { err = "hipMalloc failed"; return M0_ERR_HIP; }
    return M0_OK;
}

int Net::pack_ssl_heads(std::string& err) {
    for (int t = 0; t < 5; ++t) {
        if (!(cfg_.ssl_tasks & (1 << t))) continue;
        SslHeadW h;
        h.out_ch = kSslOut[t];
        std::string p = std::string("ssl_heads.") + kSslNames[t];
        TRY(pack_gemm(h.c0, p + ".0.weight", "", 1, C_, Cp_, C_ / 2, Cs_, 0, err));
        TRY(upload_norm(h.n, p + ".1", C_ / 2, Cs_, err));
        TRY(pack_gemm(h.c1, p + ".3.weight", "", 1, C_ / 2, Cs_, h.out_ch, 32, 0, err));
        ssl_.push_back(h);
    }
    return M0_OK;
}

void Net::make_plan() {
    const bool big = conv_gemm_tile_n(Cp_, Cp_) == 320;
    plan_.fuse_tail = big && sw_.fuse_tail &&
                      (!cfg_.se || (res_[0].se_hidden <= TAIL_SE_HMAX && res_[0].se_hidden % 4 == 0));
    plan_.fuse_attn = big && sw_.fuse_attn;
    plan_.gn_small = Cp_ % 64 == 0;
    plan_.act = cfg_.activation == M0_ACT_SILU ? ACT_SILU : ACT_RELU;
    plan_.vact = cfg_.value_activation == M0_ACT_SILU ? ACT_SILU : (cfg_.value_activation == M0_ACT_LEAKY ? ACT_LEAKY : ACT_RELU);
    int next = -1;
    for (size_t i = tower_.size(); i-- > 0;) {
        TowerLayer& L = tower_[i];
        if (L.kind == 1 && L.skip) continue;
        L.next_bn1 = next;
        next = L.kind == 0 ? L.index : -1;
    }
    plan_.first_bn1 = next;
}

int Net::finalize(std::string& err) {
    if (finalized_) return M0_OK;
    if (hipSetDevice(device_) != hipSuccess) { err = "hipSetDevice failed"; return M0_ERR_HIP; }
    const int C = C_, P = Cp_;
    nparams_ = 0;
    TRY(pack_gemm(stem_, "stem.0.weight", "", 9, cfg_.planes, 32, C, P, 0, err));
    TRY(upload_norm(stem_n_, "stem.1", C, P, err));
    if (cfg_.chess_features) TRY(pack_chess_features(err));
    int ti = 0;
    for (auto& L : tower_) {
        std::string p = "tower." + std::to_string(ti++);
        if (L.kind == 0) {
            ResBlockW& r = res_[L.index];
            TRY(pack_gemm(r.conv1, p + ".conv1.weight", "", 9, C, P, C, P, 0, err));
            TRY(pack_gemm(r.conv2, p + ".conv2.weight", "", 9, C, P, C, P, 0, err));
            TRY(upload_norm(r.bn1, p + ".bn1", C, P, err));
            TRY(upload_norm(r.bn2, p + ".bn2", C, P, err));
            if (cfg_.se) TRY(pack_se(r, p, err));
        } else {
            TRY(pack_attn(att_[L.index], L.skip, p, err));
        }
    }
    upload_attn_mask();
    TRY(pack_gemm(ph_conv_, "policy_head.0.weight", "", 1, C, P, 64, 64, 0, err));
    TRY(upload_norm(ph_n_, "policy_head.1", 64, 64, err));
    if (cfg_.policy_factor_rank > 0) {
        int r = cfg_.policy_factor_rank, rp = ceil_to(r, 32);
        TRY(pack_gemm(pfc1_, "policy_fc1.weight", "policy_fc1.bias", 1, 4096, 4096, r, rp, 64, err));
        TRY(pack_gemm(pfc2_, "policy_fc2.weight", "policy_fc2.bias", 1, r, rp, M0_POLICY_SIZE, M0_POLICY_SIZE, 0, err));
    } else {
        TRY(pack_gemm(pfc1_, "policy_fc.weight", "policy_fc.bias", 1, 4096, 4096, M0_POLICY_SIZE, M0_POLICY_SIZE, 64, err));
    }
    {
        const HostTensor* ls = get("_policy_logit_scale_raw", err); if (!ls) return M0_ERR_INVALID;
        nparams_ += 1;
        double raw = ls->data.empty() ? 0.0 : ls->data[0];
        double sp = raw > 20.0 ? raw : log1p(exp(raw));
        logit_scale_ = (float)std::min(5.0, sp + 1e-3);
    }
    TRY(pack_gemm(vh0_, "value_head.0.weight", "", 1, C, P, 128, 128, 0, err));
    TRY(upload_norm(vh1_n_, "value_head.1", 128, 128, err));
    TRY(pack_gemm(vh3_, "value_head.3.weight", "", 1, 128, 128, 128, 128, 0, err));
    TRY(upload_norm(vh4_n_, "value_head.4", 128, 128, err));
    TRY(pack_joint_head(err));
    const int h1 = 2 * C, h1p = ceil_to(h1, 32), h2 = C, h2p = ceil_to(C, 32);
    TRY(pack_gemm(vfc1_, "value_fc1.weight", "value_fc1.bias", 1, 8192, 8192, h1, h1p, 128, err));
    TRY(pack_gemm(vfc2_, "value_fc2.weight", "value_fc2.bias", 1, h1, h1p, h2, h2p, 0, err));
    TRY(pack_gemm(vgate_, "value_gate.0.weight", "value_gate.0.bias", 1, h2, h2p, h2, h2p, 0, err));
    TRY(pack_gemm(vfc3_, "value_fc3.weight", "value_fc3.bias", 1, h2, h2p, 1, 32, 0, err));
    if (cfg_.self_supervised) TRY(pack_ssl_heads(err));
    sd_.clear();
    (void)hipDeviceSynchronize();
    make_plan();
    finalized_ = true;
    return M0_OK;
}

int Net::ssl_channels_total() const {
    int n = 0;
    for (auto& h : ssl_) n += h.out_ch;
    return n;
}

double Net::flops_per_position(bool with_ssl) const {
    const double C = C_;
    double mac = 64.0 * cfg_.planes * 9 * C;
    if (cfg_.chess_features) mac += 64.0 * C * C * (cfg_.piece_square_tables ? 1 : 0) + 64.0 * C * C * 9;
    for (auto& L : tower_) {
        if (L.kind == 0) {
            mac += 2 * 64.0 * C * C * 9;
            if (cfg_.se) mac += 2.0 * C * res_[L.index].se_hidden;
        } else if (!L.skip) {
            mac += 64.0 * C * 3 * C + 64.0 * C * C;
            double nb = (cfg_.attention_unmasked_mix > 0.f && cfg_.attention_unmasked_mix < 1.f) ? 2.0 : 1.0;
            mac += 64.0 * 64.0 * C * (1.0 + nb);
        }
    }
    mac += 64.0 * C * 64;
    if (cfg_.policy_factor_rank > 0) mac += 4096.0 * cfg_.policy_factor_rank + (double)cfg_.policy_factor_rank * M0_POLICY_SIZE;
    else mac += 4096.0 * M0_POLICY_SIZE;
    mac += 64.0 * C * 128 + 64.0 * 128 * 128 + 8192.0 * 2 * C + 2.0 * C * C + C * C + C;
    if (with_ssl) for (auto& h : ssl_) mac += 64.0 * C * (C / 2) + 64.0 * (C / 2) * h.out_ch;
    return 2.0 * mac;
}

int Net::ensure_workspace(int B, std::string& err) {
    const int Bp = ceil_to(B, 4);
    const int Mfc = ceil_to(B, 256);
    if (Bp <= wsB_ && Mfc <= wsM_) return M0_OK;
    if (hipSetDevice(device_) != hipSuccess) { err = "hipSetDevice failed"; return M0_ERR_HIP; }
    (void)hipDeviceSynchronize();
    for (void* p : ws_allocs_) (void)hipFree(p);
    ws_allocs_.clear();
    const size_t C = Cp_;
    const size_t nb = Bp, nh = std::max(Bp, Mfc);
    const size_t Cst = std::max<size_t>(C, 128);
    auto H = [&](size_t elems) { return (_Float16*)dalloc(elems * 2, true); };
    auto F = [&](size_t elems) { return (float*)dalloc(elems * 4, true); };
    X0_ = H(nb * 64 * 32);
    XA_ = H(nb * 64 * C); XB_ = H(nb * 64 * C); T1_ = H(nb * 64 * C); T2_ = H(nb * 64 * C); AA_ = H(nb * 64 * C);
    QKV_ = H(nb * 64 * 3 * C); O_ = H(nb * 64 * C);
    S1_ = F(nb * Cst * 2); S2_ = F(nb * Cst * 2); G_ = F(nb * Cst);
    PH_ = H(nh * 64 * 64); PH2_ = H(nh * 64 * 64);
    VH_ = H(nh * 64 * 128); VH2_ = H(nh * 64 * 128);
    const size_t rp = cfg_.policy_factor_rank > 0 ? ceil_to(cfg_.policy_factor_rank, 32) : 32;
    F1_ = H((size_t)Mfc * rp);
    F2_ = H((size_t)Mfc * ceil_to(2 * C_, 32)); F3_ = H((size_t)Mfc * ceil_to(C_, 32)); F4_ = H((size_t)Mfc * ceil_to(C_, 32));
    SH_ = H(nb * 64 * Cs_); SH2_ = H(nb * 64 * Cs_); SO_ = H(nb * 64 * 32);
    VAL_ = F((size_t)Mfc * 32);
    SPK_ = F((size_t)8 * Mfc * ceil_to(2 * C_, 32));
    if (!X0_ || !XA_ || !XB_ || !AA_ || !T1_ || !T2_ || !QKV_ || !O_ || !S1_ || !S2_ || !PH_ || !PH2_ || !VH_ ||
        !VH2_ || !F1_ || !F2_ || !F3_ || !F4_ || !SH_ || !SH2_ || !SO_ || !VAL_ || !SPK_) {
        err = "workspace hipMalloc failed";
        wsB_ = wsM_ = 0;
        return M0_ERR_HIP;
    }
    if (hipStreamSynchronize(stream_) != hipSuccess || hipGetLastError() != hipSuccess) {
        err = "workspace clear failed"; wsB_ = wsM_ = 0; return M0_ERR_HIP;
    }
    wsB_ = Bp; wsM_ = Mfc;
    return M0_OK;
}

static GemmArgs gemm_args(const PackedGemm& g, const _Float16* in, void* out, int Mrows, int epi_act = ACT_NONE) {
    GemmArgs a;
    memset(&a, 0, sizeof(a));
    a.in = in; a.w = g.w; a.out = out; a.bias = g.bias;
    a.Mrows = Mrows; a.Mvalid = Mrows; a.Cin = g.Cin; a.N = g.N; a.Npad = g.N; a.ldo = g.N;
    a.epi_act = epi_act; a.out_scale = 1.f; a.w_pp = g.pp ? 1 : 0;
    return a;
}

static EwArgs ew_args(const _Float16* t, _Float16* y, int C, int act) {
    EwArgs e;
    memset(&e, 0, sizeof(e));
    e.t = t; e.y = y; e.C = C; e.act = act;
    return e;
}
static void ew_next_bn1(EwArgs& e, const NormParams* next_bn1, _Float16* y2) {
    if (next_bn1) { e.y2 = y2; e.gn2_gamma = next_bn1->gamma; e.gn2_beta = next_bn1->beta; }
}

static double conv3x3_flop(const PackedGemm& g, int rows) { return 2.0 * (double)rows * (double)g.N * (double)g.Cin * 9.0; }

template <class Launch>
hipError_t Net::profiled(bool on, hipStream_t st, double flop, bool tail, Launch&& launch) {
    if (!on) return launch();
    if (pev_used_ + 2 > pev_.size()) {
        for (int i = 0; i < 2; ++i) { hipEvent_t e; if (hipEventCreate(&e) != hipSuccess) return hipErrorOutOfMemory; pev_.push_back(e); }
    }
    (void)hipEventRecord(pev_[pev_used_], st);
    hipError_t rc = launch();
    (void)hipEventRecord(pev_[pev_used_ + 1], st);
    pev_used_ += 2;
    pflop_.push_back(flop);
    ptail_.push_back(tail ? 1 : 0);
    return rc;
}

hipError_t Net::run_gemm(const PackedGemm& g, GemmArgs a, hipStream_t st) {
    const bool big = conv_gemm_tile_n(g.Cin, g.N) == 320;
    const bool splitk = g.taps == 1 && big && g.Cin >= 4096 && (g.Cin >> 6) % 8 == 0 && !a.gn_gamma && !a.mul && !a.out_stats &&
                        !a.out_f32 && a.out_scale == 1.f && SPK_ != nullptr && (size_t)g.N <= (size_t)ceil_to(2 * C_, 32) &&
                        a.Mrows <= wsM_;
    return profiled(profile_ && g.taps == 9 && big, st, conv3x3_flop(g, a.Mvalid), false, [&]() -> hipError_t {
        if (!splitk) return launch_conv_gemm(a, g.taps, st);
        _Float16* out = (_Float16*)a.out;
        const int act = a.epi_act;
        a.out = SPK_; a.bias = nullptr; a.epi_act = ACT_NONE; a.out_f32 = 1; a.ksplit = 8;
        hipError_t rc = launch_conv_gemm(a, g.taps, st);
        return rc != hipSuccess ? rc : launch_splitk_reduce(SPK_, 8, a.Mrows, g.N, g.bias, act, out, st);
    });
}

hipError_t Net::se_gate(const ResBlockW& r, const float* stats, int boards, hipStream_t st) {
    SeGateArgs g;
    g.t_stats = stats; g.w1 = r.se_w1; g.b1 = r.se_b1; g.w2 = r.se_w2; g.b2 = r.se_b2;
    g.gate = G_; g.B = boards; g.C = Cp_; g.hidden = r.se_hidden; g.act = plan_.act;
    return launch_se_gate(g, st);
}

hipError_t Net::conv_norm_act(const PackedGemm& g, const NormParams& n, const _Float16* in, _Float16* out, _Float16* scratch,
                              int Mrows, hipStream_t st, const ConvNormOpts& o) {
    const bool big = conv_gemm_tile_n(g.Cin, g.N) == 320;
    GemmArgs a = gemm_args(g, in, out, Mrows);
    if (big && o.res && plan_.fuse_tail) {
        a.epi_act = plan_.act; a.res = o.res; a.pre_gamma = n.gamma; a.pre_beta = n.beta;
        if (o.next_bn1) { a.y2 = AA_; a.gn_gamma = o.next_bn1->gamma; a.gn_beta = o.next_bn1->beta; }
        return launch_conv_gemm(a, g.taps, st);
    }
    const bool epilogue = big ? g.taps == 9
                              : plan_.gn_small && (g.taps == 9 ? g.Cin == 32 : g.N == 32 || g.N == 64 || g.N == 128 || g.N == 160);
    if (epilogue && !o.res && !o.next_bn1) {
        a.gn_gamma = n.gamma; a.gn_beta = n.beta; a.epi_act = plan_.act; a.posenc = o.posenc;
        return run_gemm(g, a, st);
    }
    a.out = scratch; a.out_stats = S1_;
    hipError_t rc = run_gemm(g, a, st);
    if (rc != hipSuccess) return rc;
    EwArgs e = ew_args(scratch, out, g.N, plan_.act);
    e.t_stats = S1_; e.gn_gamma = n.gamma; e.gn_beta = n.beta; e.res = o.res; e.posenc = o.posenc;
    ew_next_bn1(e, o.next_bn1, AA_);
    return launch_ew_board(e, Mrows / 64, st);
}

void Net::harvest_profile() {
    for (size_t i = 0; i + 1 < pev_used_; i += 2) {
        float ms = 0.f;
        if (hipEventElapsedTime(&ms, pev_[i], pev_[i + 1]) == hipSuccess) {
            prof_ms_ += ms; prof_flop_ += pflop_[i / 2]; prof_launches_++;
            if (ptail_[i / 2]) { prof_tail_ms_ += ms; prof_tail_launches_++; }
        }
    }
    pev_used_ = 0;
    pflop_.clear();
    ptail_.clear();
}

#define KCHK(x)                                                                           \
    do {                                                                                  \
        hipError_t e_ = (x);                                                              \
        if (e_ != hipSuccess) {                                                           \
            err = std::string("kernel launch failed: ") + #x + ": " + hipGetErrorString(e_); \
            return M0_ERR_HIP;                                                            \
        }                                                                                 \
    } while (0)

int Net::forward(const float* planes_dev, const _Float16* nhwc_dev, int B, float* logits_dev, float* value_dev,
                 float* ssl_dev, hipStream_t st, std::string& err) {
    if (!finalized_) { err = "weights not finalized"; return M0_ERR_STATE; }
    if (B <= 0) { err = "batch must be positive"; return M0_ERR_INVALID; }
    TRY(ensure_workspace(B, err));
    const int Bp = ceil_to(B, 4);
    const int Mc = Bp * 64;
    const int Mfc = ceil_to(B, 256);
    const int act = plan_.act, vact = plan_.vact;
    const int C = Cp_;

    const _Float16* x0 = nhwc_dev;
    if (!x0) {
        if (!planes_dev) { err = "no input"; return M0_ERR_INVALID; }
        KCHK(launch_planes_to_nhwc(planes_dev, X0_, B, cfg_.planes, st));
        x0 = X0_;
    }
    _Float16* xa = XA_;
    _Float16* xb = XB_;
    const NormParams* first_bn1 = bn1(plan_.first_bn1);
    ConvNormOpts so;
    if (cfg_.chess_features) so.posenc = posenc_; else so.next_bn1 = first_bn1;
    KCHK(conv_norm_act(stem_, stem_n_, x0, xa, T1_, Mc, st, so));
    if (cfg_.chess_features) {
        if (cfg_.piece_square_tables) {
            ConvNormOpts po;
            po.res = xa;
            KCHK(conv_norm_act(pst_, pst_n_, xa, xb, T1_, Mc, st, po));
            std::swap(xa, xb);
        }
        ConvNormOpts io;
        io.res = xa; io.next_bn1 = first_bn1;
        KCHK(conv_norm_act(inter_, inter_n_, xa, xb, T1_, Mc, st, io));
        std::swap(xa, xb);
    }
    for (const TowerLayer& L : tower_) {
        const NormParams* next_bn1 = bn1(L.next_bn1);
        if (L.kind == 0) {
            const ResBlockW& r = res_[L.index];
            KCHK(conv_norm_act(r.conv1, r.bn2, AA_, T1_, T2_, Mc, st));
            if (plan_.fuse_tail) {
                GemmArgs a = gemm_args(r.conv2, T1_, xb, Mc, act);
                a.res = xa;
                if (next_bn1) { a.y2 = AA_; a.gn_gamma = next_bn1->gamma; a.gn_beta = next_bn1->beta; }
                if (cfg_.se) { a.se_w1 = r.se_w1; a.se_b1 = r.se_b1; a.se_w2 = r.se_w2; a.se_b2 = r.se_b2; a.se_hidden = r.se_hidden;
                               a.se_wf = r.se_wf; }
                KCHK(profiled(profile_, st, conv3x3_flop(r.conv2, Mc), true, [&] { return launch_conv_gemm(a, 9, st); }));
            } else {
                GemmArgs a = gemm_args(r.conv2, T1_, T2_, Mc);
                a.out_stats = S2_;
                KCHK(run_gemm(r.conv2, a, st));
                EwArgs e = ew_args(T2_, xb, C, act);
                e.t_stats = S2_; e.res = xa;
                if (cfg_.se) { KCHK(se_gate(r, S2_, Bp, st)); e.gate = G_; }
                ew_next_bn1(e, next_bn1, AA_);
                KCHK(launch_ew_board(e, Bp, st));
            }
        } else {
            if (L.skip) continue;
            const AttnW& w = att_[L.index];
            const float inv_sqrt_d = 1.f / sqrtf((float)(C_ / cfg_.attention_heads));
            if (plan_.fuse_attn && w.blk_w != nullptr) {
                AttnBlockArgs ab;
                memset(&ab, 0, sizeof(ab));
                ab.x = xa; ab.wpack = w.blk_w; ab.bias = w.blk_bias; ab.mask = mask_dev_;
                ab.ln_g = w.ln.gamma; ab.ln_b = w.ln.beta; ab.y = xb;
                if (next_bn1) { ab.y2 = AA_; ab.gn2_gamma = next_bn1->gamma; ab.gn2_beta = next_bn1->beta; }
                ab.B = Bp; ab.ln_count = C_; ab.act = act; ab.mix = cfg_.attention_unmasked_mix; ab.inv_sqrt_d = inv_sqrt_d;
                KCHK(launch_attn_block(ab, st));
            } else {
                KCHK(run_gemm(w.qkv, gemm_args(w.qkv, xa, QKV_, Mc), st));
                AttnArgs aa;
                aa.qkv = QKV_; aa.rel_bias = w.rel_bias; aa.mask = mask_dev_; aa.o = O_;
                aa.B = Bp; aa.H = C / 16; aa.C = C; aa.mix = cfg_.attention_unmasked_mix;
                aa.inv_sqrt_d = inv_sqrt_d;
                KCHK(launch_attn_core(aa, st));
                KCHK(run_gemm(w.proj, gemm_args(w.proj, O_, T1_, Mc), st));
                EwArgs e = ew_args(T1_, xb, C, act);
                e.res = xa; e.ln_g = w.ln.gamma; e.ln_b = w.ln.beta; e.ln_count = C_;
                ew_next_bn1(e, next_bn1, AA_);
                KCHK(launch_ew_board(e, Bp, st));
            }
        }
        std::swap(xa, xb);
    }
    const bool joint = plan_.gn_small;
    if (joint) {
        GemmArgs a = gemm_args(hv_, xa, PH2_, Mc, act);
        a.gn_gamma = hv_n_.gamma; a.gn_beta = hv_n_.beta;
        a.ldo = 64; a.out2 = VH2_; a.ldo2 = 128; a.nsplit = 64;
        KCHK(launch_conv_gemm(a, 1, st));
    } else {
        KCHK(conv_norm_act(ph_conv_, ph_n_, xa, PH2_, PH_, Mc, st));
    }
    const bool factored = cfg_.policy_factor_rank > 0;
    if (factored) KCHK(run_gemm(pfc1_, gemm_args(pfc1_, PH2_, F1_, Mfc, ACT_RELU), st));
    const PackedGemm& plast = factored ? pfc2_ : pfc1_;
    GemmArgs pl = gemm_args(plast, factored ? F1_ : PH2_, logits_dev, Mfc);
    pl.Mvalid = B; pl.out_f32 = 1; pl.out_scale = logit_scale_;
    KCHK(run_gemm(plast, pl, st));
    if (!joint) KCHK(conv_norm_act(vh0_, vh1_n_, xa, VH2_, VH_, Mc, st));
    _Float16* vflat = joint ? VH_ : VH2_;
    KCHK(conv_norm_act(vh3_, vh4_n_, VH2_, vflat, VH_, Mc, st));
    KCHK(run_gemm(vfc1_, gemm_args(vfc1_, vflat, F2_, Mfc, vact), st));
    KCHK(run_gemm(vfc2_, gemm_args(vfc2_, F2_, F3_, Mfc, vact), st));
    GemmArgs vg = gemm_args(vgate_, F3_, F4_, Mfc, ACT_SIGMOID);
    vg.mul = F3_;
    KCHK(run_gemm(vgate_, vg, st));
    GemmArgs v3 = gemm_args(vfc3_, F4_, VAL_, Mfc, ACT_TANH);
    v3.out_f32 = 1;
    KCHK(run_gemm(vfc3_, v3, st));
    KCHK(hipMemcpy2DAsync(value_dev, 4, VAL_, 32 * 4, 4, B, hipMemcpyDeviceToDevice, st));
    if (ssl_dev && !ssl_.empty()) {
        const int ctot = ssl_channels_total();
        int coff = 0;
        for (auto& h : ssl_) {
            KCHK(conv_norm_act(h.c0, h.n, xa, SH2_, SH_, Mc, st));
            KCHK(run_gemm(h.c1, gemm_args(h.c1, SH2_, SO_, Mc), st));
            KCHK(launch_nhwc_to_nchw_f32(SO_, ssl_dev, B, 32, h.out_ch, ctot, coff, st));
            coff += h.out_ch;
        }
    }
    return M0_OK;
}
```

### matrix0_amd/csrc/net_kernels.h

```cpp
#pragma once
#include <hip/hip_runtime.h>
#include <stdint.h>

enum { ACT_NONE = 0, ACT_RELU = 1, ACT_SILU = 2, ACT_LEAKY = 3, ACT_SIGMOID = 4, ACT_TANH = 5 };

constexpr int TAIL_SE_HMAX = 96;

struct GemmArgs {
    const _Float16* in;
    const _Float16* w;
    void* out;
    const float* gn_gamma;
    const float* gn_beta;
    const float* bias;
    const _Float16* mul;
    float* out_stats;
    int Mrows;
    int Mvalid;
    int Cin;
    int N;
    int Npad;
    int ldo;
    int epi_act;
    int out_f32;
    float out_scale;
    int ksplit;
    int w_pp;
    const _Float16* res;
    const float* pre_gamma;
    const float* pre_beta;
    _Float16* y2;
    const float* se_w1;
    const float* se_b1;
    const float* se_w2;
    const float* se_b2;
    int se_hidden;
    const void* se_wf;
    const float* posenc;
    void* out2;
    int ldo2;
    int nsplit;
};

struct EwArgs {
    const _Float16* t;
    const float* t_stats;
    const float* gn_gamma;
    const float* gn_beta;
    const float* gate;
    const _Float16* res;
    const float* posenc;
    const float* ln_g;
    const float* ln_b;
    int ln_count;
    _Float16* y;
    float* out_stats;
    _Float16* y2;
    const float* gn2_gamma;
    const float* gn2_beta;
    int C;
    int act;
};

struct SeGateArgs {
    const float* t_stats;
    const float* w1;
    const float* b1;
    const float* w2;
    const float* b2;
    float* gate;
    int B, C, hidden, act;
};

struct AttnArgs {
    const _Float16* qkv;
    const float* rel_bias;
    const uint64_t* mask;
    _Float16* o;
    int B, H, C;
    float mix;
    float inv_sqrt_d;
};

struct AttnBlockArgs {
    const _Float16* x;
    const void* wpack;
    const _Float16* bias;
    const uint64_t* mask;
    const float* ln_g;
    const float* ln_b;
    const float* gn2_gamma;
    const float* gn2_beta;
    _Float16* y;
    _Float16* y2;
    int B;
    int ln_count;
    int act;
    float mix;
    float inv_sqrt_d;
};
hipError_t launch_attn_block(const AttnBlockArgs& a, hipStream_t st);
hipError_t launch_splitk_reduce(const float* part, int splits, int M, int N, const float* bias, int act, _Float16* out,
                                hipStream_t st);
size_t attn_block_pack_bytes();

hipError_t launch_conv_gemm(const GemmArgs& a, int taps, hipStream_t st);
int conv_gemm_tile_n(int Cin, int Npad);
int conv_gemm_kc(int Cin, int Npad);
hipError_t launch_ew_board(const EwArgs& a, int boards, hipStream_t st);
hipError_t launch_se_gate(const SeGateArgs& a, hipStream_t st);
hipError_t launch_attn_core(const AttnArgs& a, hipStream_t st);
hipError_t launch_planes_to_nhwc(const float* x, void* y, int B, int P, hipStream_t st);
hipError_t launch_nhwc_to_nchw_f32(const void* x, float* y, int B, int ld, int n, int ctot, int coff, hipStream_t st);
```

### matrix0_amd/csrc/net_kernels.hip

```cpp
#include "kernel_common.h"
#include "conv_epilogue.h"

template <int TAPS, int WN, int NT, int KC, int EPI = 0, int ACT = 0>
__global__ __launch_bounds__(256 * WN) void conv_gemm_kernel(GemmArgs a) {
    constexpr int NB = WN * NT * 32;
    constexpr int NTHR = 256 * WN;
    constexpr int AST = KC + 8;
    constexpr int APIX = (TAPS == 9) ? 100 : 64;
    constexpr int A_ELEMS = 4 * APIX * AST;
    constexpr int W_ELEMS = NB * AST;
    constexpr int A_PIECES = 4 * 64 * KC / 8;
    constexpr int W_PIECES = NB * KC / 8;
    constexpr int A_PER = (A_PIECES + NTHR - 1) / NTHR;
    constexpr int W_PER = (W_PIECES + NTHR - 1) / NTHR;
    constexpr int K8 = KC / 8;

    extern __shared__ __attribute__((aligned(16))) char smem[];
    _Float16* A_lds = reinterpret_cast<_Float16*>(smem);
    _Float16* W_lds = A_lds + A_ELEMS;

    const int tid = threadIdx.x;
    const int lane = tid & 63;
    const int wave = tid >> 6;
    const int wm = wave % 4;
    const int wn = wave / 4;
    const int m0 = blockIdx.x * 256;
    const int n0 = blockIdx.y * NB;
    const int Cin = a.Cin;
    const int nchunk = Cin / KC;
    const int Npad = a.Npad;

    if (TAPS == 9) {
        for (int i = tid; i < A_ELEMS / 8; i += NTHR)
            reinterpret_cast<uint4*>(A_lds)[i] = make_uint4(0, 0, 0, 0);
    }
    __syncthreads();

    float16v acc[2][NT];
    static_for<0, 2>([&](auto mi) __attribute__((always_inline)) {
        static_for<0, NT>([&](auto ni) __attribute__((always_inline)) {
            acc[decltype(mi)::value][decltype(ni)::value] = float16v{0.f, 0.f, 0.f, 0.f, 0.f, 0.f, 0.f, 0.f,
                                                                      0.f, 0.f, 0.f, 0.f, 0.f, 0.f, 0.f, 0.f};
        });
    });

    int apix[2];
#pragma unroll
    for (int mi = 0; mi < 2; ++mi) {
        int px = mi * 32 + (lane & 31);
        if (TAPS == 9) apix[mi] = wm * 100 + ((px >> 3) + 1) * 10 + (px & 7) + 1;
        else apix[mi] = wm * 64 + px;
    }
    const int khalf = 8 * (lane >> 5);

    uint4 areg[A_PER];
    uint4 wreg[W_PER];

    auto load_A = [&](int chunk) {
#pragma unroll
        for (int i = 0; i < A_PER; ++i) {
            int p = tid + i * NTHR;
            if (A_PIECES % NTHR == 0 || p < A_PIECES) {
                int row = p / K8, c8 = p % K8;
                areg[i] = *reinterpret_cast<const uint4*>(a.in + (size_t)(m0 + row) * Cin + chunk * KC + c8 * 8);
            }
        }
    };
    auto store_A = [&](int chunk) {
#pragma unroll
        for (int i = 0; i < A_PER; ++i) {
            int p = tid + i * NTHR;
            if (A_PIECES % NTHR == 0 || p < A_PIECES) {
                int row = p / K8, c8 = p % K8;
                int b = row >> 6, px = row & 63;
                uint4 v = areg[i];
                int pix = (TAPS == 9) ? (b * 100 + ((px >> 3) + 1) * 10 + (px & 7) + 1) : row;
                *reinterpret_cast<uint4*>(A_lds + pix * AST + c8 * 8) = v;
            }
        }
    };
    auto load_W = [&](int step) {
        int chunk = step / TAPS, tap = step % TAPS;
        const _Float16* src = a.w + ((size_t)(tap * nchunk + chunk) * Npad + n0) * KC;
#pragma unroll
        for (int i = 0; i < W_PER; ++i) {
            int p = tid + i * NTHR;
            if (W_PIECES % NTHR == 0 || p < W_PIECES)
                wreg[i] = *reinterpret_cast<const uint4*>(src + (size_t)p * 8);
        }
    };
    auto store_W = [&](int buf) {
#pragma unroll
        for (int i = 0; i < W_PER; ++i) {
            int p = tid + i * NTHR;
            if (W_PIECES % NTHR == 0 || p < W_PIECES) {
                int n = p / K8, k8 = p % K8;
                *reinterpret_cast<uint4*>(W_lds + buf * W_ELEMS + n * AST + k8 * 8) = wreg[i];
            }
        }
    };

    const int nsteps = nchunk * TAPS;
    load_A(0);
    load_W(0);
    for (int s = 0; s < nsteps; ++s) {
        const int chunk = s / TAPS, tap = s % TAPS;
        if (tap == 0) {
            if (s > 0) __syncthreads();
            store_A(chunk);
        }
        store_W(s & 1);
        __syncthreads();
        if (s + 1 < nsteps) {
            load_W(s + 1);
            if ((s + 1) % TAPS == 0) load_A((s + 1) / TAPS);
        }
        const int tapoff = (TAPS == 9) ? ((tap / 3 - 1) * 10 + (tap % 3 - 1)) : 0;
        const _Float16* Wb = W_lds + (s & 1) * W_ELEMS + (wn * NT * 32 + (lane & 31)) * AST + khalf;
        static_for<0, KC / 16>([&](auto kk_) __attribute__((always_inline)) {
            constexpr int kk = decltype(kk_)::value;
            half8 af0 = *reinterpret_cast<const half8*>(A_lds + (apix[0] + tapoff) * AST + kk * 16 + khalf);
            half8 af1 = *reinterpret_cast<const half8*>(A_lds + (apix[1] + tapoff) * AST + kk * 16 + khalf);
            static_for<0, NT>([&](auto ni_) __attribute__((always_inline)) {
                constexpr int ni = decltype(ni_)::value;
                half8 bf = *reinterpret_cast<const half8*>(Wb + ni * 32 * AST + kk * 16);
                acc[0][ni] = __builtin_amdgcn_mfma_f32_32x32x16_f16(af0, bf, acc[0][ni], 0, 0, 0);
                acc[1][ni] = __builtin_amdgcn_mfma_f32_32x32x16_f16(af1, bf, acc[1][ni], 0, 0, 0);
            });
        });
    }

    if constexpr (EPI == 1) {
        __syncthreads();
        char* lds_wave = smem + wave * (64 * 64 * NT);
        const int cb = n0 + wn * NT * 32;
        const int r31 = lane & 31, half = lane >> 5;
        GemmArgs o = a;
        int lc = cb;
        if (a.out2 != nullptr && cb >= a.nsplit) { o.out = a.out2; o.ldo = a.ldo2; lc = cb - a.nsplit; }
        o.out = reinterpret_cast<_Float16*>(o.out) + lc;
        char* wbase = conv_stage_base<NT>(lds_wave, lane);
        static_for<0, NT>([&](auto ni_) __attribute__((always_inline)) {
            constexpr int ni = decltype(ni_)::value;
            const int col = cb + ni * 32 + r31;
            float s = 0.f, ss = 0.f;
            static_for<0, 2>([&](auto mi_) __attribute__((always_inline)) {
                const float16v av = acc[decltype(mi_)::value][ni];
                static_for<0, 16>([&](auto r_) __attribute__((always_inline)) { const float v = av[decltype(r_)::value]; s += v; ss += v * v; });
            });
#pragma unroll
            for (int o2 = 1; o2 <= 8; o2 <<= 1) { s += __shfl_xor(s, o2); ss += __shfl_xor(ss, o2); }
            s += __shfl_xor(s, 32); ss += __shfl_xor(ss, 32);
            const float mean = s * (1.f / 1024.f);
            float var = ss * (1.f / 1024.f) - mean * mean;
            var = var > 0.f ? var : 0.f;
            const float g = rsqrtf(var + 1e-5f) * a.gn_gamma[col];
            const float sh = a.gn_beta[col] - mean * g;
            static_for<0, 2>([&](auto mi_) __attribute__((always_inline)) {
                constexpr int mi = decltype(mi_)::value;
                float v[16];
                static_for<0, 16>([&](auto r_) __attribute__((always_inline)) {
                    constexpr int r = decltype(r_)::value;
                    v[r] = act_fast<ACT>(acc[mi][ni][r] * g + sh);
                });
                if (a.posenc != nullptr) {
                    static_for<0, 16>([&](auto r_) __attribute__((always_inline)) {
                        constexpr int r = decltype(r_)::value;
                        const int sq = mi * 32 + (r & 3) + 8 * (r >> 2) + 4 * half;
                        v[r] += a.posenc[(size_t)sq * a.N + col];
                    });
                }
                conv_stage_tile<NT, mi, ni>(v, wbase, lane);
            });
        });
        conv_stage_flush<NT>(o, lds_wave, m0, 0, wm, 0, lane);
        return;
    }
    const int ldo = a.ldo;
    const int rowbase = m0 + wm * 64 + 4 * (lane >> 5);
    const int colbase = n0 + wn * NT * 32 + (lane & 31);
    const int epi_act = a.epi_act;
    const float oscale = a.out_scale;
    const bool has_mul = a.mul != nullptr;
    const bool f32out = a.out_f32 != 0;
    const bool want_stats = a.out_stats != nullptr;
    static_for<0, NT>([&](auto ni_) __attribute__((always_inline)) {
        constexpr int ni = decltype(ni_)::value;
        const int col = colbase + ni * 32;
        const float bias = a.bias != nullptr ? a.bias[col] : 0.f;
        float s = 0.f, ss = 0.f;
        static_for<0, 2>([&](auto mi_) __attribute__((always_inline)) {
            constexpr int mi = decltype(mi_)::value;
            const float16v av = acc[mi][ni];
            static_for<0, 16>([&](auto r_) __attribute__((always_inline)) {
                constexpr int r = decltype(r_)::value;
                const int row = rowbase + mi * 32 + (r & 3) + 8 * (r >> 2);
                float v = av[r] + bias;
                if (epi_act != ACT_NONE) v = act_apply(v, epi_act);
                if (has_mul) v *= (float)a.mul[(size_t)row * ldo + col];
                v *= oscale;
                s += v; ss += v * v;
                if (row < a.Mvalid) {
                    if (f32out) reinterpret_cast<float*>(a.out)[(size_t)row * ldo + col] = v;
                    else reinterpret_cast<_Float16*>(a.out)[(size_t)row * ldo + col] = (_Float16)v;
                }
            });
        });
        if (want_stats) {
            s += __shfl_xor(s, 32);
            ss += __shfl_xor(ss, 32);
            if (lane < 32) {
                float* st = a.out_stats + ((size_t)(m0 / 64 + wm) * a.N + col) * 2;
                st[0] = s; st[1] = ss;
            }
        }
    });
}


template <int TAPS, int WN, int NT, int KC>
static size_t conv_gemm_lds(int Cin) {
    constexpr int NB = WN * NT * 32;
    constexpr int AST = KC + 8;
    constexpr int APIX = (TAPS == 9) ? 100 : 64;
    (void)Cin;
    const size_t main_loop = (size_t)(4 * APIX * AST + 2 * NB * AST) * 2 + 64;
    const size_t staging = (size_t)WN * 4 * 64 * 64 * NT;
    return main_loop > staging ? main_loop : staging;
}

template <int TAPS, int WN, int NT, int KC, int EPI = 0, int ACT = 0>
static hipError_t launch_conv_gemm_t(const GemmArgs& a, hipStream_t st) {
    constexpr int NB = WN * NT * 32;
    size_t lds = conv_gemm_lds<TAPS, WN, NT, KC>(a.Cin);
    static DeviceOnce once;
    hipError_t e = once.run([] {
        return hipFuncSetAttribute(reinterpret_cast<const void*>(&conv_gemm_kernel<TAPS, WN, NT, KC, EPI, ACT>),
                                   hipFuncAttributeMaxDynamicSharedMemorySize, 160 * 1024);
    });
    if (e != hipSuccess) return e;
    dim3 grid(a.Mrows / 256, a.Npad / NB);
    hipLaunchKernelGGL((conv_gemm_kernel<TAPS, WN, NT, KC, EPI, ACT>), grid, dim3(256 * WN), lds, st, a);
    return hipGetLastError();
}
template <int ACT>
static hipError_t launch_conv_gemm_gn(const GemmArgs& a, int taps, hipStream_t st) {
    if (a.bias != nullptr || a.mul != nullptr || a.out_stats != nullptr || a.out_f32 || a.out_scale != 1.f || a.Npad != a.N)
        return hipErrorInvalidValue;
    if (taps == 9) return a.Npad % 64 == 0 && a.out2 == nullptr ? launch_conv_gemm_t<9, 1, 2, 32, 1, ACT>(a, st) : hipErrorInvalidValue;
    if (a.posenc != nullptr) return hipErrorInvalidValue;
    if (a.out2 != nullptr) return a.Npad == 192 && a.nsplit == 64 ? launch_conv_gemm_t<1, 3, 2, 32, 1, ACT>(a, st) : hipErrorInvalidValue;
    if (a.Npad == 160) return launch_conv_gemm_t<1, 1, 5, 32, 1, ACT>(a, st);
    if (a.Npad == 128) return launch_conv_gemm_t<1, 2, 2, 32, 1, ACT>(a, st);
    if (a.Npad == 64) return launch_conv_gemm_t<1, 1, 2, 32, 1, ACT>(a, st);
    if (a.Npad == 32) return launch_conv_gemm_t<1, 1, 1, 32, 1, ACT>(a, st);
    return hipErrorInvalidValue;
}

hipError_t launch_conv_big(const GemmArgs& a, int taps, hipStream_t st);
hipError_t launch_conv_zs(const GemmArgs& a, hipStream_t st);

int conv_gemm_tile_n(int Cin, int Npad) {
    return (Npad % 320 == 0 && Cin % 64 == 0) ? 320 : 32;
}
int conv_gemm_kc(int Cin, int Npad) {
    return (Npad % 320 == 0 && Cin % 64 == 0) ? 64 : 32;
}

hipError_t launch_conv_gemm(const GemmArgs& a, int taps, hipStream_t st) {
    if (a.Mrows % 256 != 0 || a.Cin % 32 != 0 || a.Npad % 32 != 0) return hipErrorInvalidValue;
    const bool big = conv_gemm_tile_n(a.Cin, a.Npad) == 320;
    if (a.gn_gamma != nullptr && !big) {
        if (a.epi_act == ACT_SILU) return launch_conv_gemm_gn<ACT_SILU>(a, taps, st);
        if (a.epi_act == ACT_RELU) return launch_conv_gemm_gn<ACT_RELU>(a, taps, st);
        return hipErrorInvalidValue;
    }
    if (taps == 9) {
        if (big) {
            if (!a.w_pp) return hipErrorInvalidValue;
            return launch_conv_zs(a, st);
        }
        return launch_conv_gemm_t<9, 1, 1, 32>(a, st);
    } else if (taps == 1) {
        if (big) return a.w_pp ? hipErrorInvalidValue : launch_conv_big(a, 1, st);
        if (a.Mrows / 256 >= 256 && a.Npad % 64 == 0) return launch_conv_gemm_t<1, 1, 2, 32>(a, st);
        return launch_conv_gemm_t<1, 1, 1, 32>(a, st);
    }
    return hipErrorInvalidValue;
}

__global__ __launch_bounds__(768) void ew_board_kernel(EwArgs a) {
    extern __shared__ __attribute__((aligned(16))) char smem[];
    const int C = a.C, NC = C >> 3;
    float* sc = reinterpret_cast<float*>(smem);
    float* sh = sc + C;
    float* tot = sh + C;
    float* rowbuf = tot + 2 * C;
    float* red = rowbuf + 128;
    const int tid = threadIdx.x, lane = tid & 63, wave = tid >> 6;
    const int nthr = blockDim.x, nw = nthr >> 6;
    const int chunk = tid % NC, sg = tid / NC;
    const int c0 = chunk * 8;
    const int b = blockIdx.x;
    const _Float16* t = a.t + (size_t)b * 64 * C + (size_t)(sg * 4) * C + c0;
    const _Float16* res = a.res ? a.res + (size_t)b * 64 * C + (size_t)(sg * 4) * C + c0 : nullptr;
    const float* tst = a.t_stats ? a.t_stats + (size_t)b * C * 2 : nullptr;

    const bool gn = a.gn_gamma != nullptr;
    const bool se = (!gn) && a.gate != nullptr;
    float gatev[8];
    {
        const float4 g0 = se ? *reinterpret_cast<const float4*>(a.gate + (size_t)b * C + c0) : make_float4(1.f, 1.f, 1.f, 1.f);
        const float4 g1 = se ? *reinterpret_cast<const float4*>(a.gate + (size_t)b * C + c0 + 4) : make_float4(1.f, 1.f, 1.f, 1.f);
        gatev[0] = g0.x; gatev[1] = g0.y; gatev[2] = g0.z; gatev[3] = g0.w;
        gatev[4] = g1.x; gatev[5] = g1.y; gatev[6] = g1.z; gatev[7] = g1.w;
    }
    float g2w = 0.f, g2b = 0.f;
    if (a.y2 != nullptr && tid < C) { g2w = a.gn2_gamma[tid]; g2b = a.gn2_beta[tid]; }
    half8 tv[4], rv[4];
    static_for<0, 4>([&](auto k_) __attribute__((always_inline)) {
        constexpr int k = decltype(k_)::value;
        tv[k] = *reinterpret_cast<const half8*>(t + k * C);
        rv[k] = res ? *reinterpret_cast<const half8*>(res + k * C) : half8{0, 0, 0, 0, 0, 0, 0, 0};
    });

    if (gn) {
        for (int c = tid; c < C; c += nthr) {
            const int g0 = (c >> 4) << 4;
            float s = 0.f, ss = 0.f;
            for (int j = 0; j < 16; ++j) { s += tst[2 * (g0 + j)]; ss += tst[2 * (g0 + j) + 1]; }
            const float mean = s * (1.f / 1024.f);
            float var = ss * (1.f / 1024.f) - mean * mean;
            var = var > 0.f ? var : 0.f;
            const float g = a.gn_gamma[c] * rsqrtf(var + 1e-5f);
            sc[c] = g;
            sh[c] = a.gn_beta[c] - mean * g;
        }
    }
    __syncthreads();

    float scl[8], shl[8];
    static_for<0, 8>([&](auto i_) __attribute__((always_inline)) {
        constexpr int i = decltype(i_)::value;
        scl[i] = gn ? sc[c0 + i] : gatev[i];
        shl[i] = gn ? sh[c0 + i] : 0.f;
    });
    float x[4][8];
    float pe[4][8];
    if (a.posenc) {
        static_for<0, 4>([&](auto k_) __attribute__((always_inline)) {
            constexpr int k = decltype(k_)::value;
            const float4 p0 = *reinterpret_cast<const float4*>(a.posenc + (sg * 4 + k) * C + c0);
            const float4 p1 = *reinterpret_cast<const float4*>(a.posenc + (sg * 4 + k) * C + c0 + 4);
            pe[k][0] = p0.x; pe[k][1] = p0.y; pe[k][2] = p0.z; pe[k][3] = p0.w;
            pe[k][4] = p1.x; pe[k][5] = p1.y; pe[k][6] = p1.z; pe[k][7] = p1.w;
        });
    }
    static_for<0, 4>([&](auto k_) __attribute__((always_inline)) {
        constexpr int k = decltype(k_)::value;
        static_for<0, 8>([&](auto i_) __attribute__((always_inline)) {
            constexpr int i = decltype(i_)::value;
            float v = (float)tv[k][i];
            if (gn) v = act_apply(v * scl[i] + shl[i], a.act);
            else if (se) v *= scl[i];
            v += (float)rv[k][i];
            if (a.posenc) v += pe[k][i];
            x[k][i] = v;
        });
    });
    if (a.ln_g != nullptr) {
        float2* part = reinterpret_cast<float2*>(red);
        static_for<0, 4>([&](auto k_) __attribute__((always_inline)) {
            constexpr int k = decltype(k_)::value;
            float rs = 0.f, rss = 0.f;
            static_for<0, 8>([&](auto i_) __attribute__((always_inline)) { const float v = x[k][decltype(i_)::value]; rs += v; rss += v * v; });
            part[(sg * 4 + k) * NC + chunk] = make_float2(rs, rss);
        });
        __syncthreads();
        float2* rowp = reinterpret_cast<float2*>(rowbuf);
        for (int u = tid; u < 512; u += nthr) {
            const int sq = u >> 3, p8 = u & 7;
            float rs = 0.f, rss = 0.f;
            for (int ch = p8; ch < NC; ch += 8) { const float2 v = part[sq * NC + ch]; rs += v.x; rss += v.y; }
#pragma unroll
            for (int o = 1; o < 8; o <<= 1) { rs += __shfl_xor(rs, o); rss += __shfl_xor(rss, o); }
            if (p8 == 0) {
                const float cnt = (float)(a.ln_count > 0 ? a.ln_count : C);
                const float mean = rs / cnt;
                float var = rss / cnt - mean * mean;
                var = var > 0.f ? var : 0.f;
                rowp[sq] = make_float2(mean, rsqrtf(var + 1e-5f));
            }
        }
        __syncthreads();
        float lg[8], lb[8];
        static_for<0, 8>([&](auto i_) __attribute__((always_inline)) {
            constexpr int i = decltype(i_)::value;
            lg[i] = a.ln_g[c0 + i]; lb[i] = a.ln_b[c0 + i];
        });
        static_for<0, 4>([&](auto k_) __attribute__((always_inline)) {
            constexpr int k = decltype(k_)::value;
            const float2 mr = rowp[sg * 4 + k];
            static_for<0, 8>([&](auto i_) __attribute__((always_inline)) {
                constexpr int i = decltype(i_)::value;
                x[k][i] = (x[k][i] - mr.x) * mr.y * lg[i] + lb[i];
            });
        });
        __syncthreads();
    }

    _Float16* y = a.y + (size_t)b * 64 * C + (size_t)(sg * 4) * C + c0;
    half8 yv[4];
    float csum[8], csq[8];
    static_for<0, 8>([&](auto i_) __attribute__((always_inline)) { csum[decltype(i_)::value] = 0.f; csq[decltype(i_)::value] = 0.f; });
    static_for<0, 4>([&](auto k_) __attribute__((always_inline)) {
        constexpr int k = decltype(k_)::value;
        static_for<0, 8>([&](auto i_) __attribute__((always_inline)) {
            constexpr int i = decltype(i_)::value;
            yv[k][i] = (_Float16)x[k][i];
            csum[i] += x[k][i]; csq[i] += x[k][i] * x[k][i];
        });
        *reinterpret_cast<half8*>(y + k * C) = yv[k];
    });
    if (a.out_stats == nullptr && a.y2 == nullptr) return;
    static_for<0, 8>([&](auto i_) __attribute__((always_inline)) {
        constexpr int i = decltype(i_)::value;
        reinterpret_cast<float2*>(red)[sg * C + c0 + i] = make_float2(csum[i], csq[i]);
    });
    __syncthreads();
    for (int c = tid; c < C; c += nthr) {
        float s = 0.f, ss = 0.f;
        for (int g = 0; g < 16; ++g) { const float2 v = reinterpret_cast<const float2*>(red)[g * C + c]; s += v.x; ss += v.y; }
        tot[2 * c] = s; tot[2 * c + 1] = ss;
        if (a.out_stats != nullptr) {
            a.out_stats[((size_t)b * C + c) * 2] = s;
            a.out_stats[((size_t)b * C + c) * 2 + 1] = ss;
        }
    }
    if (a.y2 == nullptr) return;
    __syncthreads();
    if (tid < C) {
        const int c = tid, g0 = (c >> 4) << 4;
        float s = 0.f, ss = 0.f;
        for (int j = 0; j < 16; ++j) { s += tot[2 * (g0 + j)]; ss += tot[2 * (g0 + j) + 1]; }
        const float mean = s * (1.f / 1024.f);
        float var = ss * (1.f / 1024.f) - mean * mean;
        var = var > 0.f ? var : 0.f;
        const float g = g2w * rsqrtf(var + 1e-5f);
        sc[c] = g;
        sh[c] = g2b - mean * g;
    }
    __syncthreads();
    _Float16* y2 = a.y2 + (size_t)b * 64 * C + (size_t)(sg * 4) * C + c0;
    static_for<0, 8>([&](auto i_) __attribute__((always_inline)) { constexpr int i = decltype(i_)::value; scl[i] = sc[c0 + i]; shl[i] = sh[c0 + i]; });
    static_for<0, 4>([&](auto k_) __attribute__((always_inline)) {
        constexpr int k = decltype(k_)::value;
        half8 ov;
        static_for<0, 8>([&](auto i_) __attribute__((always_inline)) {
            constexpr int i = decltype(i_)::value;
            ov[i] = (_Float16)act_apply((float)yv[k][i] * scl[i] + shl[i], a.act);
        });
        *reinterpret_cast<half8*>(y2 + k * C) = ov;
    });
}

hipError_t launch_ew_board(const EwArgs& a, int boards, hipStream_t st) {
    if (a.C > 384 || a.C % 32 != 0) return hipErrorInvalidValue;
    const int nthr = 2 * a.C;
    const size_t lds = (size_t)(4 * a.C + 128 + 32 * a.C) * 4;
    hipLaunchKernelGGL(ew_board_kernel, dim3(boards), dim3(nthr), lds, st, a);
    return hipGetLastError();
}

__global__ __launch_bounds__(384) void se_gate_kernel(SeGateArgs a) {
    extern __shared__ __attribute__((aligned(16))) char smem[];
    const int C = a.C, Hd = a.hidden;
    float* pool = reinterpret_cast<float*>(smem);
    float* part = pool + 8 * C;
    float* hid = part + 8 * C;
    const int tid = threadIdx.x, nthr = blockDim.x;
    const int b0 = blockIdx.x * 8;
    const int nb = a.B - b0 < 8 ? a.B - b0 : 8;
    for (int q = 0; q < 8; ++q)
        pool[q * C + tid] = q < nb ? a.t_stats[((size_t)(b0 + q) * C + tid) * 2] * (1.f / 64.f) : 0.f;
    __syncthreads();
    const int parts = nthr / Hd;
    {
        const int j = tid % Hd, p = tid / Hd;
        if (p < parts) {
            const int cpp = (C + parts - 1) / parts;
            const int cbeg = p * cpp, cend = cbeg + cpp < C ? cbeg + cpp : C;
            float s[8] = {0.f, 0.f, 0.f, 0.f, 0.f, 0.f, 0.f, 0.f};
            for (int cb = cbeg; cb < cend; cb += 16) {
                float w[16];
#pragma unroll
                for (int u = 0; u < 16; ++u) w[u] = cb + u < cend ? a.w1[(size_t)(cb + u) * Hd + j] : 0.f;
#pragma unroll
                for (int u = 0; u < 16; ++u) {
                    const int c = cb + u < cend ? cb + u : cbeg;
#pragma unroll
                    for (int q = 0; q < 8; ++q) s[q] = __builtin_fmaf(w[u], pool[q * C + c], s[q]);
                }
            }
#pragma unroll
            for (int q = 0; q < 8; ++q) part[(p * 8 + q) * Hd + j] = s[q];
        }
    }
    __syncthreads();
    for (int i = tid; i < 8 * Hd; i += nthr) {
        const int q = i / Hd, j = i - q * Hd;
        float s = a.b1[j];
        for (int p = 0; p < parts; ++p) s += part[(p * 8 + q) * Hd + j];
        hid[q * Hd + j] = act_apply(s, a.act);
    }
    __syncthreads();
    {
        const int c = tid;
        const float bias = a.b2[c];
        float s[8] = {bias, bias, bias, bias, bias, bias, bias, bias};
        for (int jb = 0; jb < Hd; jb += 16) {
            float w[16];
#pragma unroll
            for (int u = 0; u < 16; ++u) w[u] = jb + u < Hd ? a.w2[(size_t)(jb + u) * C + c] : 0.f;
#pragma unroll
            for (int u = 0; u < 16; ++u) {
                const int j = jb + u < Hd ? jb + u : 0;
#pragma unroll
                for (int q = 0; q < 8; ++q) s[q] = __builtin_fmaf(w[u], hid[q * Hd + j], s[q]);
            }
        }
        for (int q = 0; q < nb; ++q) a.gate[(size_t)(b0 + q) * C + c] = 1.f / (1.f + __expf(-s[q]));
    }
}

hipError_t launch_se_gate(const SeGateArgs& a, hipStream_t st) {
    if (a.C > 384 || a.C % 32 != 0 || a.hidden < 1 || a.hidden > a.C) return hipErrorInvalidValue;
    const size_t lds = (size_t)(8 * a.C + 8 * a.C + 8 * a.hidden) * 4;
    hipLaunchKernelGGL(se_gate_kernel, dim3((a.B + 7) / 8), dim3(a.C), lds, st, a);
    return hipGetLastError();
}

#define ATT_BOARDS 16
__global__ __launch_bounds__(256) void attn_core_kernel(AttnArgs a) {
    constexpr int VROW = 68;
    __shared__ __attribute__((aligned(16))) _Float16 Vt[4][16][VROW];
    __shared__ __attribute__((aligned(16))) _Float16 Bs[4][64][VROW];
    __shared__ __attribute__((aligned(16))) _Float16 Ms[64][VROW];
    const int tid = threadIdx.x, lane = tid & 63, wave = tid >> 6;
    const int H = a.H, C = a.C;
    const int hgroups = (H + 3) >> 2;
    const int hg = blockIdx.x % hgroups, bgroup = blockIdx.x / hgroups;
    const int h = hg * 4 + wave;
    const bool hlive = h < H;
    const int r31 = lane & 31, half = lane >> 5;
    if (a.rel_bias != nullptr) {
        for (int i = tid; i < 4 * 64 * 16; i += 256) {
            const int hh = i >> 10, q = (i >> 4) & 63, k4 = (i & 15) * 4;
            if (hg * 4 + hh < H) {
                const float4 v = *reinterpret_cast<const float4*>(a.rel_bias + ((size_t)(hg * 4 + hh) * 64 + q) * 64 + k4);
                typedef _Float16 half4s __attribute__((ext_vector_type(4)));
                *reinterpret_cast<half4s*>(&Bs[hh][q][k4]) = half4s{(_Float16)v.x, (_Float16)v.y, (_Float16)v.z, (_Float16)v.w};
            }
        }
    }
    for (int i = tid; i < 64 * 16; i += 256) {
        const int q = i >> 4, k4 = (i & 15) * 4;
        const uint64_t m = a.mask[q] >> k4;
        typedef _Float16 half4s __attribute__((ext_vector_type(4)));
        *reinterpret_cast<half4s*>(&Ms[q][k4]) = half4s{(_Float16)(float)(m & 1), (_Float16)(float)((m >> 1) & 1),
                                                        (_Float16)(float)((m >> 2) & 1), (_Float16)(float)((m >> 3) & 1)};
    }
    __syncthreads();
    for (int it = 0; it < ATT_BOARDS; ++it) {
    const int b = bgroup * ATT_BOARDS + it;
    const bool live = hlive && b < a.B;
    if (!live) continue;
    const _Float16* base = a.qkv + (size_t)b * 64 * 3 * C;
    {
        const _Float16* vp = base + (size_t)lane * 3 * C + (2 * H + h) * 16;
        const half8 v0 = *reinterpret_cast<const half8*>(vp), v1 = *reinterpret_cast<const half8*>(vp + 8);
#pragma unroll
        for (int d = 0; d < 8; ++d) { Vt[wave][d][lane] = v0[d]; Vt[wave][8 + d][lane] = v1[d]; }
    }
    half8 kf[2], qf[2];
#pragma unroll
    for (int t = 0; t < 2; ++t) {
        kf[t] = *reinterpret_cast<const half8*>(base + (size_t)(t * 32 + r31) * 3 * C + (1 * H + h) * 16 + 8 * half);
        qf[t] = *reinterpret_cast<const half8*>(base + (size_t)(t * 32 + r31) * 3 * C + (0 * H + h) * 16 + 8 * half);
    }
    const float16v zero = {0.f, 0.f, 0.f, 0.f, 0.f, 0.f, 0.f, 0.f, 0.f, 0.f, 0.f, 0.f, 0.f, 0.f, 0.f, 0.f};
    typedef _Float16 half4v __attribute__((ext_vector_type(4)));
    half8 vf[2][2];
    {
        const _Float16* vrow = &Vt[wave][lane & 15][0];
        static_for<0, 2>([&](auto kt_) __attribute__((always_inline)) {
            static_for<0, 2>([&](auto jb_) __attribute__((always_inline)) {
                constexpr int kt = decltype(kt_)::value, jb = decltype(jb_)::value;
                const half4v lo = *reinterpret_cast<const half4v*>(vrow + kt * 32 + 16 * jb + 4 * half);
                const half4v hi = *reinterpret_cast<const half4v*>(vrow + kt * 32 + 16 * jb + 8 + 4 * half);
                vf[kt][jb] = half8{lo[0], lo[1], lo[2], lo[3], hi[0], hi[1], hi[2], hi[3]};
            });
        });
    }
    float wm_, wu_;
    if (a.mix > 0.f && a.mix < 1.f) { wm_ = 1.f - a.mix; wu_ = 1.f - (1.f - a.mix); }
    else if (a.mix >= 1.f) { wm_ = 1.f; wu_ = 0.f; }
    else { wm_ = 0.f; wu_ = 1.f; }
    const float isd = a.inv_sqrt_d * 1.44269504088896f;
    const float clampv = 50.f * 1.44269504088896f;
    static_for<0, 2>([&](auto qt_) __attribute__((always_inline)) {
        constexpr int qt = decltype(qt_)::value;
        const int q = qt * 32 + r31;
        const half8 qfr = qf[qt];
        float16v st[2];
        st[0] = __builtin_amdgcn_mfma_f32_32x32x16_f16(kf[0], qfr, zero, 0, 0, 0);
        st[1] = __builtin_amdgcn_mfma_f32_32x32x16_f16(kf[1], qfr, zero, 0, 0, 0);
        const _Float16* rb = a.rel_bias ? &Bs[wave][q][0] : nullptr;
        const _Float16* vm = &Ms[q][0];
        float e[2][16];
        float su = 0.f, sm = 0.f;
        static_for<0, 2>([&](auto kt_) __attribute__((always_inline)) {
            constexpr int kt = decltype(kt_)::value;
            static_for<0, 4>([&](auto g_) __attribute__((always_inline)) {
                constexpr int g = decltype(g_)::value;
                const int key0 = kt * 32 + 8 * g + 4 * half;
                half4v bias = {0, 0, 0, 0};
                if (rb) bias = *reinterpret_cast<const half4v*>(rb + key0);
                const half4v vis = *reinterpret_cast<const half4v*>(vm + key0);
                static_for<0, 4>([&](auto j_) __attribute__((always_inline)) {
                    constexpr int j = decltype(j_)::value;
                    float d = st[kt][4 * g + j] * isd + (float)bias[j];
                    d = __builtin_amdgcn_fmed3f(d, -clampv, clampv);
                    const float eu = __builtin_amdgcn_exp2f(d);
                    e[kt][4 * g + j] = eu;
                    su += eu;
                    sm += eu * (float)vis[j];
                });
            });
        });
        su += __shfl_xor(su, 32);
        sm += __shfl_xor(sm, 32);
        const float cu = wu_ / su, cm = wm_ / sm;
        float16v oacc = zero;
        static_for<0, 2>([&](auto kt_) __attribute__((always_inline)) {
            constexpr int kt = decltype(kt_)::value;
            static_for<0, 2>([&](auto jb_) __attribute__((always_inline)) {
                constexpr int jb = decltype(jb_)::value;
                half8 pf;
                const half4v v0 = *reinterpret_cast<const half4v*>(vm + kt * 32 + 16 * jb + 4 * half);
                const half4v v1 = *reinterpret_cast<const half4v*>(vm + kt * 32 + 16 * jb + 8 + 4 * half);
                static_for<0, 8>([&](auto u_) __attribute__((always_inline)) {
                    constexpr int u = decltype(u_)::value;
                    constexpr int r = 8 * jb + u;
                    const float vis = (float)(u < 4 ? v0[u & 3] : v1[u & 3]);
                    pf[u] = (_Float16)(e[kt][r] * (vis * cm + cu));
                });
                oacc = __builtin_amdgcn_mfma_f32_32x32x16_f16(vf[kt][jb], pf, oacc, 0, 0, 0);
            });
        });
        typedef _Float16 half2v_ __attribute__((ext_vector_type(2)));
        union { half2v_ h2[2]; uint32_t u[2]; } lo4, hi4, rcv;
        lo4.h2[0] = half2v_{(_Float16)oacc[0], (_Float16)oacc[1]}; lo4.h2[1] = half2v_{(_Float16)oacc[2], (_Float16)oacc[3]};
        hi4.h2[0] = half2v_{(_Float16)oacc[4], (_Float16)oacc[5]}; hi4.h2[1] = half2v_{(_Float16)oacc[6], (_Float16)oacc[7]};
        rcv.u[0] = __shfl_xor(half ? lo4.u[0] : hi4.u[0], 32);
        rcv.u[1] = __shfl_xor(half ? lo4.u[1] : hi4.u[1], 32);
        uint4 ov;
        if (half == 0) ov = make_uint4(lo4.u[0], lo4.u[1], rcv.u[0], rcv.u[1]);
        else ov = make_uint4(rcv.u[0], rcv.u[1], hi4.u[0], hi4.u[1]);
        *reinterpret_cast<uint4*>(a.o + ((size_t)b * 64 + q) * C + h * 16 + 8 * half) = ov;
    });
    }
}

hipError_t launch_attn_core(const AttnArgs& a, hipStream_t st) {
    const int hgroups = (a.H + 3) / 4, bgroups = (a.B + ATT_BOARDS - 1) / ATT_BOARDS;
    hipLaunchKernelGGL(attn_core_kernel, dim3((unsigned)(hgroups * bgroups)), dim3(256), 0, st, a);
    return hipGetLastError();
}

__global__ void planes_to_nhwc_kernel(const float* __restrict__ x, _Float16* __restrict__ y, int B, int P) {
    long i = (long)blockIdx.x * blockDim.x + threadIdx.x;
    long total = (long)B * 64 * 32;
    if (i >= total) return;
    int c = (int)(i % 32);
    long bn = i / 32;
    int n = (int)(bn % 64);
    long b = bn / 64;
    float v = (c < P) ? x[(b * P + c) * 64 + n] : 0.f;
    y[i] = (_Float16)v;
}

hipError_t launch_planes_to_nhwc(const float* x, void* y, int B, int P, hipStream_t st) {
    long total = (long)B * 64 * 32;
    hipLaunchKernelGGL(planes_to_nhwc_kernel, dim3((unsigned)((total + 255) / 256)), dim3(256), 0, st, x,
                       reinterpret_cast<_Float16*>(y), B, P);
    return hipGetLastError();
}

__global__ void nhwc_to_nchw_f32_kernel(const _Float16* __restrict__ x, float* __restrict__ y, int B, int ld, int n,
                                        int ctot, int coff) {
    long i = (long)blockIdx.x * blockDim.x + threadIdx.x;
    long total = (long)B * n * 64;
    if (i >= total) return;
    int sq = (int)(i % 64);
    long bc = i / 64;
    int c = (int)(bc % n);
    long b = bc / n;
    y[(b * ctot + coff + c) * 64 + sq] = (float)x[(b * 64 + sq) * ld + c];
}

hipError_t launch_nhwc_to_nchw_f32(const void* x, float* y, int B, int ld, int n, int ctot, int coff, hipStream_t st) {
    long total = (long)B * n * 64;
    hipLaunchKernelGGL(nhwc_to_nchw_f32_kernel, dim3((unsigned)((total + 255) / 256)), dim3(256), 0, st,
                       reinterpret_cast<const _Float16*>(x), y, B, ld, n, ctot, coff);
    return hipGetLastError();
}
```

### matrix0_amd/csrc/selfplay.hip

```cpp
#include <math.h>
#include <string.h>
#include <atomic>
#include "selfplay_engine.h"

namespace m0 {

static bool nn_cache_miss(m0_selfplay* sp, uint64_t key) {
    auto it = sp->nn_map.find(key);
    if (it != sp->nn_map.end()) {
        sp->nn_lru.splice(sp->nn_lru.end(), sp->nn_lru, it->second);
        return false;
    }
    sp->nn_lru.push_back(key);
    sp->nn_map[key] = std::prev(sp->nn_lru.end());
    if (sp->nn_lru.size() > 10000) { sp->nn_map.erase(sp->nn_lru.front()); sp->nn_lru.pop_front(); }
    return true;
}

void seed_game_dev(GameDev& g, uint64_t base, int uid) {
    g.seed_jitter = derive_seed(base, uid, PURPOSE_JITTER);
    g.seed_noise = derive_seed(base, uid, PURPOSE_NOISE);
    g.seed_dir = derive_seed(base, uid, PURPOSE_DIRICHLET);
    g.ctr_jitter = g.ctr_noise = g.ctr_dir = 0;
}

int sync_games_d2h(m0_selfplay* sp) {
    if (hipMemcpyAsync(sp->hg.data(), sp->d.games, sizeof(GameDev) * sp->G, hipMemcpyDeviceToHost, sp->stream) != hipSuccess) return -1;
    return hipStreamSynchronize(sp->stream) == hipSuccess ? 0 : -1;
}
static int sync_games_h2d(m0_selfplay* sp) {
    return hipMemcpyAsync(sp->d.games, sp->hg.data(), sizeof(GameDev) * sp->G, hipMemcpyHostToDevice, sp->stream) == hipSuccess ? 0 : -1;
}
static void push_hist(m0_selfplay* sp, int slot, const RepWindow& w) {
    int n = (int)w.keys.size();
    const uint64_t* src = w.keys.data();
    if (n > M0_HIST_CAP) { src += n - M0_HIST_CAP; n = M0_HIST_CAP; }
    sp->hg[slot].hist_len = n;
    if (n > 0) (void)hipMemcpyAsync(sp->d.hist + (size_t)slot * M0_HIST_CAP, src, (size_t)n * 8, hipMemcpyHostToDevice, sp->stream);
}

void arm_search(m0_selfplay* sp, int slot, const Pos& pos, const RepWindow& win, int sims, bool dirichlet, bool fresh) {
    GameDev& g = sp->hg[slot];
    g.root_pos = pos;
    g.active = 1; g.sims_done = 0; g.sims_target = sims;
    g.need_dirichlet = dirichlet ? 1 : 0;
    g.root_q_from_v = 0;
    g.root_fresh = fresh ? 1 : 0;
    g.flip_root_v = (sp->cfg.value_from_white && pos.turn == BLACK) ? 1 : 0;
    g.finished = 0; g.nsamples = 0;
    g.reinfer = (sp->cfg.root_reinfer && !fresh && nn_cache_miss(sp, tkey(pos))) ? 1 : 0;
    sp->prev_done[slot] = 0;
    push_hist(sp, slot, win);
}

static void finish_game(m0_selfplay* sp, int slot, bool resigned, int resigner, bool have_z, float z_in) {
    HostGame& hgm = sp->games[slot];
    const m0_selfplay_cfg& c = sp->cfg;
    float z = z_in;
    if (!have_z) {
        if (is_game_over(hgm.pos, hgm.win, true)) z = game_result(hgm.pos);
        else if (c.arena_mode) z = 0.f;
        else z = hgm.search_values.empty() ? 0.f : hgm.search_values.back();
    }
    sp->stats.games_finished++;
    if ((c.record_games && hgm.nstates > 0) || c.arena_mode) {
        GameRecordOwner* o = new GameRecordOwner();
        o->s.swap(hgm.states); o->pi.swap(hgm.pis); o->legal_mask.swap(hgm.masks);
        o->search_values = hgm.search_values;
        o->z.resize(hgm.nstates);
        for (int i = 0; i < hgm.nstates; ++i) o->z[i] = z * (float)hgm.turns[i];
        o->played.assign(hgm.history.begin(), hgm.history.end());
        if (hgm.book_index >= 0) o->start_fen = sp->book_fens[hgm.book_index];
        if (c.ssl_targets && (int)hgm.rec_pos.size() == hgm.nstates) {
            const int T = hgm.nstates;
            if (T > sp->ssl_cap) {
                Pos* np = dalloc<Pos>(sp, (size_t)T + 64);
                float* no = dalloc<float>(sp, ((size_t)T + 64) * 17 * 64);
                if (np && no) { sp->ssl_pos_dev = np; sp->ssl_out_dev = no; sp->ssl_cap = T + 64; }
                else sp->stats.ssl_dropped++;
            }
            if (T <= sp->ssl_cap) {
                o->ssl.resize((size_t)T * 17 * 64);
                (void)hipMemcpyAsync(sp->ssl_pos_dev, hgm.rec_pos.data(), sizeof(Pos) * T, hipMemcpyHostToDevice, sp->stream);
                (void)launch_ssl_targets(sp->ssl_pos_dev, T, sp->ssl_out_dev, sp->stream);
                (void)hipMemcpyAsync(o->ssl.data(), sp->ssl_out_dev, (size_t)T * 17 * 64 * 4, hipMemcpyDeviceToHost, sp->stream);
                (void)hipStreamSynchronize(sp->stream);
            }
        }
        m0_game_record r;
        memset(&r, 0, sizeof(r));
        r.game_index = hgm.game_index; r.moves = hgm.nstates; r.resigned = resigned ? 1 : 0; r.resigner = resigner;
        r.draw = z == 0.0f ? 1 : 0; r.total_plies = (int)hgm.history.size(); r.result = z;
        r.avg_policy_entropy = (float)(hgm.entropy_sum / (double)(hgm.entropy_count > 0 ? hgm.entropy_count : 1));
        double ss = 0; for (int v : hgm.sims_used) ss += v;
        r.avg_sims = hgm.sims_used.empty() ? 0.f : (float)(ss / (double)hgm.sims_used.size());
        r.secs = (now_ms() - hgm.t0) / 1000.0;
        r.s = o->s.data(); r.pi = o->pi.data(); r.z = o->z.data(); r.legal_mask = o->legal_mask.data();
        r.search_values = o->search_values.data(); r.played = o->played.data(); r.owner = o;
        r.ssl = o->ssl.empty() ? nullptr : o->ssl.data();
        r.start_fen = hgm.book_index >= 0 ? o->start_fen.c_str() : nullptr;
        sp->done_meta.push_back(r);
    }
    hgm.in_use = false;
    sp->hg[slot].active = 0;
}

static void begin_move(m0_selfplay* sp, int slot, int child_slot, std::vector<int>& adv_ids, std::vector<int>& adv_slots) {
    HostGame& hgm = sp->games[slot];
    const m0_selfplay_cfg& c = sp->cfg;
    DrawCfg dc = draw_cfg_from(c);
    if (is_game_over(hgm.pos, hgm.win, c.arena_mode != 0) || hgm.nstates >= c.max_game_len ||
        should_adjudicate_draw(hgm.pos, hgm.win, hgm.history, dc)) {
        finish_game(sp, slot, false, 0, false, 0.f);
        return;
    }
    if (c.arena_mode) {
        child_slot = -1;
        sp->hg[slot].net_id = ((hgm.pos.turn == WHITE) == hgm.a_is_white) ? 0 : 1;
    }
    const bool cap_draws = c.playout_random_frac > 0.0 && c.num_simulations > 0;
    int sims = playout_cap(c.num_simulations, c.playout_random_frac, cap_draws ? hgm.rng.next() : 0.0);
    hgm.cur_sims = sims;
    if (c.fresh_tree_per_move || c.tt_merge) child_slot = -1;
    if (c.arena_mode && c.tt_merge) child_slot = hgm.nstates == 0 ? -3 : -2;
    const bool dir = c.dirichlet_plies < 0 || hgm.nstates < c.dirichlet_plies;
    arm_search(sp, slot, hgm.pos, hgm.win, sims, dir, child_slot < 0);
    adv_ids.push_back(slot);
    adv_slots.push_back(child_slot);
}

static void start_game(m0_selfplay* sp, int slot, std::vector<int>& adv_ids, std::vector<int>& adv_slots) {
    HostGame& hgm = sp->games[slot];
    hgm = HostGame();
    hgm.in_use = true;
    hgm.game_index = sp->cfg.first_game_index + sp->next_game++;
    sp->stats.games_started++;
    parse_fen(START_FEN, hgm.pos);
    hgm.rng = HStream(derive_seed(sp->cfg.seed, hgm.game_index, PURPOSE_GAME));
    if (!sp->book.empty()) {
        const bool paired = sp->cfg.arena_mode && sp->cfg.arena_paired_openings;
        const double u = paired ? HStream(derive_seed(sp->cfg.seed, hgm.game_index / 2, PURPOSE_PAIR_OPENING)).next() : hgm.rng.next();
        size_t k = (size_t)(u * (double)sp->book.size());
        if (k >= sp->book.size()) k = sp->book.size() - 1;
        hgm.pos = sp->book[k];
        hgm.book_index = (int)k;
    }
    hgm.t0 = now_ms();
    hgm.a_is_white = (hgm.game_index % 2) == 0;
    seed_game_dev(sp->hg[slot], sp->cfg.seed, hgm.game_index);
    sp->hg[slot].evals = 0;
    if (sp->cfg.arena_mode && sp->tc.eval_cache) sp->hg[slot].ec_clear = 1;
    for (int i = 0; i < sp->cfg.opening_random_plies; ++i) {
        if (is_game_over(hgm.pos, hgm.win, false)) break;
        Move mv[M0_MAX_MOVES];
        int n = gen_legal(hgm.pos, mv);
        if (n <= 0) break;
        int k = (int)(hgm.rng.next() * n);
        if (k >= n) k = n - 1;
        hgm.play(mv[k]);
    }
    begin_move(sp, slot, -1, adv_ids, adv_slots);
}

static void finish_search(m0_selfplay* sp, int slot, std::vector<int>& adv_ids, std::vector<int>& adv_slots) {
    HostGame& hgm = sp->games[slot];
    const m0_selfplay_cfg& c = sp->cfg;
    const RootResult& R = sp->hres[slot];
    const GameDev& g = sp->hg[slot];
    const int k = R.nchild;
    long total = 0;
    int maxv = 0;
    for (int i = 0; i < k; ++i) { total += R.child_n[i]; if (R.child_n[i] > maxv) maxv = R.child_n[i]; }
    if (k <= 0 || total <= 0) {
        sp->stats.arena_overflows++;
        hgm.nstates = 0;
        hgm.states.clear(); hgm.pis.clear(); hgm.masks.clear(); hgm.search_values.clear(); hgm.turns.clear();
        hgm.sims_used.clear(); hgm.rec_pos.clear();
        finish_game(sp, slot, false, 0, true, 0.f);
        return;
    }
    const double root_q = R.root_n > 0 ? R.root_q : g.root_v;
    const size_t T = (size_t)hgm.nstates;
    if (c.record_games) {
        hgm.pis.resize((T + 1) * 4672, 0.f);
        float* pi = hgm.pis.data() + T * 4672;
        for (int i = 0; i < k; ++i) pi[R.child_idx[i]] = (float)((double)R.child_n[i] / (double)total);
        hgm.states.resize((T + 1) * 19 * 64);
        encode_planes_f32(hgm.pos, hgm.states.data() + T * 19 * 64);
        if (c.ssl_targets) hgm.rec_pos.push_back(hgm.pos);
        hgm.masks.resize((T + 1) * 4672, 0);
        uint8_t* mk = hgm.masks.data() + T * 4672;
        if (c.max_children > 0 || c.min_child_prior > 0.0) {
            Move lm[M0_MAX_MOVES];
            const int nl = gen_legal(hgm.pos, lm);
            for (int i = 0; i < nl; ++i) mk[move_to_index(hgm.pos, lm[i])] = 1;
        } else {
            for (int i = 0; i < k; ++i) mk[R.child_idx[i]] = 1;
        }
    }
    {
        double ent = 0.0;
        for (int i = 0; i < k; ++i) {
            double p = (double)(float)((double)R.child_n[i] / (double)total);
            if (p < 1e-12) p = 1e-12;
            ent -= p * log(p);
        }
        ent -= (double)(4672 - k) * (1e-12 * log(1e-12));
        hgm.entropy_sum += ent; hgm.entropy_count++;
        hgm.resign.recent_entropies.push_back(ent);
        if ((int)hgm.resign.recent_entropies.size() > c.resign_window) hgm.resign.recent_entropies.erase(hgm.resign.recent_entropies.begin());
    }
    double temp = temperature_for(hgm.pos.fullmove, c.temperature_start, c.temperature_end, c.temperature_moves);
    if (c.low_visit_threshold > 0 && maxv < c.low_visit_threshold && temp < 0.8) temp = 0.8;
    std::vector<int32_t> visits(R.child_n, R.child_n + k);
    int pick;
    if (c.arena_mode) {
        const bool sampling = c.arena_temp > 1e-3 && hgm.nstates < c.arena_temp_plies;
        pick = arena_choose_move(visits.data(), k, c.arena_temp, hgm.nstates, c.arena_temp_plies, sampling ? hgm.rng.next() : 0.0);
    } else {
        pick = sample_move_index(visits.data(), k, temp, sample_move_draws(visits.data(), k, temp) ? hgm.rng.next() : 0.0);
    }
    const Move mv = R.child_mv[pick];
    hgm.search_values.push_back((float)root_q);
    hgm.turns.push_back(hgm.pos.turn == WHITE ? 1 : -1);
    hgm.sims_used.push_back(hgm.cur_sims);
    hgm.nstates++;
    sp->stats.plies++;
    if (!c.arena_mode && resign_update(hgm.resign, root_q, hgm.nstates, c)) {
        const bool white = hgm.pos.turn == WHITE;
        finish_game(sp, slot, true, white ? 1 : 2, true, white ? -1.f : 1.f);
        return;
    }
    hgm.play(mv);
    begin_move(sp, slot, pick, adv_ids, adv_slots);
}

int run_select(m0_selfplay* sp, int* rows_out) {
    if (hipMemsetAsync(sp->d.row_counter, 0, 8, sp->stream) != hipSuccess) return -1;
    if (launch_select(sp->d, sp->tc, sp->stream) != hipSuccess) return -1;
    if (hipMemcpyAsync(sp->rows2, sp->d.row_counter, 8, hipMemcpyDeviceToHost, sp->stream) != hipSuccess) return -1;
    if (hipStreamSynchronize(sp->stream) != hipSuccess) return -1;
    *rows_out = sp->rows2[0];
    return 0;
}

int apply_advances(m0_selfplay* sp, std::vector<int>& ids, std::vector<int>& slots) {
    if (sync_games_h2d(sp) != 0) return -1;
    if (!ids.empty()) {
        (void)hipMemcpyAsync(sp->ids_dev, ids.data(), ids.size() * 4, hipMemcpyHostToDevice, sp->stream);
        (void)hipMemcpyAsync(sp->slots_dev, slots.data(), slots.size() * 4, hipMemcpyHostToDevice, sp->stream);
        if (launch_advance(sp->d, sp->ids_dev, sp->slots_dev, (int)ids.size(), sp->stream) != hipSuccess) return -1;
        if (hipStreamSynchronize(sp->stream) != hipSuccess) return -1;
        if (sp->d.tt_sides == 2) {
            if (sync_games_d2h(sp) != 0) return -1;
            bool any = false;
            for (size_t k = 0; k < ids.size(); ++k) {
                if (slots[k] > -2) continue;
                GameDev& g = sp->hg[ids[k]];
                const uint64_t salt = (g.net_id & 1) ? 0x9E3779B97F4A7C15ull : 0ull;
                const uint64_t gsalt = (uint64_t)(uint32_t)sp->games[ids[k]].game_index * 0xD6E8FEB86659FD93ull;
                g.reinfer = (g.root_found && nn_cache_miss(sp, tkey(g.root_pos) ^ salt ^ gsalt)) ? 1 : 0;
                any = any || g.reinfer;
            }
            if (any && sync_games_h2d(sp) != 0) return -1;
        }
    }
    return 0;
}

static void count_active_games(m0_selfplay* sp) {
    int act = 0;
    for (int s = 0; s < sp->G; ++s) act += sp->games[s].in_use ? 1 : 0;
    sp->stats.active_games = act;
}

int start_first_games(m0_selfplay* sp) {
    if (sp->stats.games_started != 0) return M0_OK;
    std::vector<int> ids, slots;
    if (sync_games_d2h(sp) != 0) { m0_set_error("device sync failed"); return M0_ERR_HIP; }
    for (int s = 0; s < sp->G; ++s) {
        if (sp->cfg.total_games > 0 && sp->next_game >= sp->cfg.total_games) break;
        start_game(sp, s, ids, slots);
    }
    if (apply_advances(sp, ids, slots) != 0) { m0_set_error("advance failed"); return M0_ERR_HIP; }
    count_active_games(sp);
    return M0_OK;
}

static constexpr int M0_MAX_DEVICES = 16;
static std::mutex g_forward_gate[M0_MAX_DEVICES];
static std::atomic<int> g_engines_with_net[M0_MAX_DEVICES];
static bool forward_gate_enabled() {
    static const bool on = [] { const char* v = getenv("M0_FORWARD_GATE"); return v && v[0] == '1'; }();
    return on;
}

struct ForwardGate {
    std::mutex* m = nullptr;
    hipStream_t st = nullptr;
    ForwardGate(int device, hipStream_t stream, bool has_rows) : st(stream) {
        if (has_rows && forward_gate_enabled() && (unsigned)device < (unsigned)M0_MAX_DEVICES &&
            g_engines_with_net[device].load(std::memory_order_relaxed) > 1) {
            m = &g_forward_gate[device];
            m->lock();
        }
    }
    void release() {
        if (m) { (void)hipStreamSynchronize(st); m->unlock(); m = nullptr; }
    }
    ~ForwardGate() { release(); }
};

void forward_gate_join(m0_selfplay* sp) {
    if ((unsigned)sp->device < (unsigned)M0_MAX_DEVICES) { g_engines_with_net[sp->device].fetch_add(1); sp->counted = true; }
}
void forward_gate_leave(m0_selfplay* sp) {
    if (sp->counted) g_engines_with_net[sp->device].fetch_sub(1);
}

int step_back(m0_selfplay* sp, int rows, double t0, std::string& err) {
    (void)hipEventRecord(sp->ev2, sp->stream);
    if (launch_expand(sp->d, sp->tc, sp->stream) != hipSuccess) { err = "expand launch failed"; return M0_ERR_HIP; }
    (void)hipEventRecord(sp->ev3, sp->stream);
    if (sync_games_d2h(sp) != 0) { err = std::string("step failed: ") + hipGetErrorString(hipGetLastError()); return M0_ERR_HIP; }
    if (sp->net) sp->net->harvest_profile();
    if (sp->net_b) sp->net_b->harvest_profile();
    float ms_sel = 0, ms_net = 0, ms_exp = 0;
    (void)hipEventElapsedTime(&ms_sel, sp->ev0, sp->ev1);
    (void)hipEventElapsedTime(&ms_net, sp->ev1, sp->ev2);
    (void)hipEventElapsedTime(&ms_exp, sp->ev2, sp->ev3);
    sp->stats.ms_net += ms_net; sp->stats.ms_tree += ms_sel + ms_exp;
    sp->stats.steps++; sp->stats.evals += (uint64_t)rows;
    const double t1 = now_ms();
    bool any = false;
    if (sp->tc.eval_cache) {
        uint64_t h = 0;
        for (int s = 0; s < sp->G; ++s) h += sp->hg[s].cache_hits;
        sp->stats.evals_cached = h;
    }
    for (int s = 0; s < sp->G; ++s) {
        if (!sp->hg[s].active) continue;
        const int delta = sp->hg[s].sims_done - sp->prev_done[s];
        if (delta > 0) { sp->stats.sims += (uint64_t)delta; sp->prev_done[s] = sp->hg[s].sims_done; }
        if (sp->hg[s].finished) any = true;
    }
    std::vector<int> ids, slots;
    if (any) {
        (void)hipMemcpy(sp->hres.data(), sp->d.results, sizeof(RootResult) * sp->G, hipMemcpyDeviceToHost);
        for (int s = 0; s < sp->G; ++s) {
            if (!(sp->hg[s].active && sp->hg[s].finished)) continue;
            if (sp->hg[s].overflow) sp->stats.arena_overflows++;
            finish_search(sp, s, ids, slots);
        }
        for (int s = 0; s < sp->G; ++s) {
            if (sp->games[s].in_use) continue;
            if (sp->cfg.total_games > 0 && sp->next_game >= sp->cfg.total_games) continue;
            start_game(sp, s, ids, slots);
        }
        if (apply_advances(sp, ids, slots) != 0) { err = "advance failed"; return M0_ERR_HIP; }
    }
    count_active_games(sp);
    const double t2 = now_ms();
    sp->stats.ms_host += t2 - t1;
    sp->stats.ms_total += t2 - t0;
    return M0_OK;
}

struct RowSplit { int main_rows, tail_rows; };
static RowSplit split_rows(int rows, bool have_tail, bool half_split) {
    int main_rows = rows;
    if (have_tail && rows >= 2048 && (rows & 1023) != 0) main_rows = rows & ~1023;
    if (have_tail && half_split && rows >= 4096) main_rows = ((rows / 2) + 1023) & ~1023;
    return {main_rows, rows - main_rows};
}

int one_step(m0_selfplay* sp, std::string& err) {
    const double t0 = now_ms();
    (void)hipEventRecord(sp->ev0, sp->stream);
    int rows = 0;
    if (run_select(sp, &rows) != 0) { err = std::string("select failed: ") + hipGetErrorString(hipGetLastError()); return M0_ERR_HIP; }
    (void)hipEventRecord(sp->ev1, sp->stream);
    if (rows > sp->rows_max || sp->rows2[1] > sp->rows_max) { err = "row counter overflow"; return M0_ERR_STATE; }
    ForwardGate gate(sp->device, sp->stream, rows > 0 || sp->rows2[1] > 0);
    if (rows > 0) {
        if (!sp->net) { err = "m0_selfplay_step needs a network (use the split-step API without one)"; return M0_ERR_STATE; }
        const auto [main_rows, tail_rows] = split_rows(rows, sp->net_tail != nullptr, sp->half_split);
        float* ssl = sp->cfg.ssl_in_forward ? sp->ssl_dev : nullptr;
        m0_net_lock(sp->nethandle);
        int rc = M0_OK;
        if (tail_rows > 0) (void)hipEventRecord(sp->ev_sel, sp->stream);
        rc = sp->net->forward(nullptr, sp->d.x0, main_rows, sp->logits_dev, sp->values_dev, ssl, sp->stream, err);
        if (rc == M0_OK && tail_rows > 0) {
            (void)hipStreamWaitEvent(sp->stream_tail, sp->ev_sel, 0);
            const size_t sslw = ssl ? (size_t)sp->net->ssl_channels_total() * 64 : 0;
            rc = sp->net_tail->forward(nullptr, sp->d.x0 + (size_t)main_rows * 64 * 32, tail_rows, sp->logits_dev + (size_t)main_rows * 4672,
                                       sp->values_dev + main_rows, ssl ? ssl + (size_t)main_rows * sslw : nullptr, sp->stream_tail, err);
            (void)hipEventRecord(sp->ev_tail, sp->stream_tail);
            (void)hipStreamWaitEvent(sp->stream, sp->ev_tail, 0);
        }
        m0_net_unlock(sp->nethandle);
        if (rc != M0_OK) return rc;
        sp->stats.rows_tail += (uint64_t)tail_rows;
    }
    if (sp->rows2[1] > 0) {
        if (!sp->net_b) { err = "rows for a second network without one"; return M0_ERR_STATE; }
        const size_t b = (size_t)sp->d.net_row_base;
        m0_net_lock(sp->nethandle_b);
        int rc = sp->net_b->forward(nullptr, sp->d.x0 + b * 64 * 32, sp->rows2[1], sp->logits_dev + b * 4672,
                                    sp->values_dev + b, nullptr, sp->stream, err);
        m0_net_unlock(sp->nethandle_b);
        if (rc != M0_OK) return rc;
        rows += sp->rows2[1];
    }
    gate.release();
    return step_back(sp, rows, t0, err);
}

}
```

### matrix0_amd/csrc/selfplay_engine.h

```cpp
#pragma once
#include <hip/hip_runtime.h>
#include <chrono>
#include <deque>
#include <list>
#include <mutex>
#include <string>
#include <unordered_map>
#include <vector>
#include "../../include/m0_engine.h"
#include "capi_common.h"
#include "chess_core.h"
#include "host_rules.h"
#include "net.h"
#include "tree.h"

namespace m0 {

inline double now_ms() {
    return std::chrono::duration<double, std::milli>(std::chrono::steady_clock::now().time_since_epoch()).count();
}

struct GameRecordOwner {
    std::vector<float> s, pi, z, search_values, ssl;
    std::vector<uint8_t> legal_mask;
    std::vector<uint16_t> played;
    std::string start_fen;
};

struct HostGame : Line {
    bool in_use = false;
    int game_index = 0;
    std::vector<Pos> rec_pos;
    std::vector<float> states, pis, search_values;
    std::vector<int8_t> turns;
    std::vector<uint8_t> masks;
    std::vector<int> sims_used;
    int nstates = 0;
    double entropy_sum = 0.0;
    int entropy_count = 0;
    ResignState resign;
    HStream rng;
    double t0 = 0.0;
    int cur_sims = 0;
    bool a_is_white = true;
    int book_index = -1;
};

}

struct m0_selfplay {
    m0_selfplay_cfg cfg;
    TreeCfg tc;
    m0_net* nethandle = nullptr;
    m0_net* nethandle_b = nullptr;
    Net* net = nullptr;
    Net* net_b = nullptr;
    Net* net_tail = nullptr;
    hipStream_t stream_tail = nullptr;
    hipEvent_t ev_sel = nullptr, ev_tail = nullptr;
    bool half_split = false;
    int device = 0;
    hipStream_t stream = nullptr;
    bool own_stream = false;
    int G = 0, L = 0, cap = 0, rows_max = 0;
    TreeDev d;
    std::vector<void*> allocs;
    bool alloc_failed = false;
    std::vector<GameDev> hg;
    std::vector<m0::HostGame> games;
    std::vector<RootResult> hres;
    float* logits_dev = nullptr;
    float* values_dev = nullptr;
    float* ssl_dev = nullptr;
    m0::Pos* ssl_pos_dev = nullptr;
    float* ssl_out_dev = nullptr;
    int ssl_cap = 0;
    int* ids_dev = nullptr;
    int* slots_dev = nullptr;
    std::deque<m0_game_record> done_meta;
    m0_selfplay_stats stats;
    int next_game = 0;
    hipEvent_t ev0 = nullptr, ev1 = nullptr, ev2 = nullptr, ev3 = nullptr;
    std::mutex mu;
    std::vector<Sample> hsamples;
    std::vector<int> prev_done;
    int last_rows = 0, last_rows_b = 0;
    int rows2[2] = {0, 0};
    std::vector<m0::Pos> book;
    std::vector<std::string> book_fens;
    std::list<uint64_t> nn_lru;
    std::unordered_map<uint64_t, std::list<uint64_t>::iterator> nn_map;
    bool ext_pending = false;
    bool counted = false;
};

namespace m0 {

template <typename T>
T* dalloc(m0_selfplay* sp, size_t count) {
    void* p = nullptr;
    size_t bytes = count * sizeof(T);
    if (bytes == 0) bytes = 16;
    if (hipMalloc(&p, bytes) != hipSuccess) { sp->alloc_failed = true; return nullptr; }
    (void)hipMemsetAsync(p, 0, bytes, sp->stream);
    sp->allocs.push_back(p);
    return (T*)p;
}

void forward_gate_join(m0_selfplay* sp);
void forward_gate_leave(m0_selfplay* sp);
void seed_game_dev(GameDev& g, uint64_t base, int uid);
int sync_games_d2h(m0_selfplay* sp);
void arm_search(m0_selfplay* sp, int slot, const Pos& pos, const RepWindow& win, int sims, bool dirichlet, bool fresh);
int apply_advances(m0_selfplay* sp, std::vector<int>& ids, std::vector<int>& slots);
int start_first_games(m0_selfplay* sp);
int run_select(m0_selfplay* sp, int* rows_out);
int one_step(m0_selfplay* sp, std::string& err);
int step_back(m0_selfplay* sp, int rows, double t0, std::string& err);

}
```

### matrix0_amd/csrc/tree.h

```cpp
#pragma once
#include <hip/hip_runtime.h>
#include <stdint.h>
#include "chess_core.h"
#include "../../include/m0_engine.h"

#define M0_MAX_DEPTH 256
#define M0_HIST_CAP 192
#define M0_MAX_CHILDREN 256
constexpr int M0_NHWC_C = 32;

struct TreeCfg {
    double fpu_reduction;
    double draw_penalty;
    double virtual_loss;
    double selection_jitter;
    double cpuct;
    double cpuct_start, cpuct_end;
    int cpuct_plies;
    int use_c_base;
    double cpuct_c_base, cpuct_c_init;
    double dirichlet_alpha, dirichlet_frac;
    int legal_softmax;
    int enable_entropy_noise;
    int no_instant_backtrack;
    int virtual_loss_active;
    int leaves_per_step;
    int tt_merge;
    int raw_legal_priors;
    int max_children;
    double min_child_prior;
    int eval_cache;
};

#define M0_EC_MAXLEGAL 64
#define M0_EC_WORDS 66
struct EvalCache {
    uint64_t* keys;
    uint32_t* stamps;
    float* payload;
    float* hit_stage;
    int sets;
    int sides;
};

struct GameDev {
    m0::Pos root_pos;
    int root;
    int next;
    int arena;
    int active;
    int sims_done, sims_target;
    int need_dirichlet;
    int root_q_from_v;
    int flip_root_v;
    int root_fresh;
    int hist_len;
    int nsamples;
    int overflow;
    int finished;
    int root_n;
    double root_q;
    double root_v;
    uint64_t seed_jitter, seed_noise, seed_dir;
    uint64_t ctr_jitter, ctr_noise, ctr_dir;
    uint64_t evals;
    int net_id;
    int reinfer;
    uint64_t cache_hits;
    uint32_t cache_clock[2];
    int ec_clear;
    int side_next[2];
    int root_found;
};

enum SampleKind : int {
    SK_NONE = 0,
    SK_EVAL = 1,
    SK_ROOT_INIT = 2,
    SK_TERMINAL = 3,
    SK_ROOT_VALUE = 4,
    SK_CACHED = 5,
    SK_SHARED = 6,
};
M0_HD bool sample_owns_row(int kind) { return kind == SK_EVAL || kind == SK_ROOT_INIT || kind == SK_ROOT_VALUE; }
M0_HD bool sample_holds_inflight(int kind) { return kind == SK_EVAL || kind == SK_TERMINAL || kind == SK_CACHED || kind == SK_SHARED; }

struct Sample {
    m0::Pos pos;
    int kind;
    uint64_t ckey;
    int leaf;
    int depth;
    int row;
    int nlegal;
};
static_assert(sizeof(Sample) == 104, "the host copies Sample arrays device-to-host: the layout must not move");

struct TreeArrays {
    double* prior;
    double* w;
    double* q;
    int* n;
    int* vl;
    int* cbase;
    int16_t* nch;
    uint16_t* mv;
    uint16_t* midx;
    int cap;
};

struct RootResult {
    int nchild;
    int root_n;
    double root_q;
    int child_node[M0_MAX_CHILDREN];
    int child_n[M0_MAX_CHILDREN];
    uint16_t child_mv[M0_MAX_CHILDREN];
    uint16_t child_idx[M0_MAX_CHILDREN];
    double child_prior[M0_MAX_CHILDREN];
    double child_q[M0_MAX_CHILDREN];
};

struct TreeDev {
    TreeArrays t;
    GameDev* games;
    Sample* samples;
    int* paths;
    int* epaths;
    uint64_t* tt_keys;
    int* tt_nodes;
    int tt_cap;
    EvalCache ec;
    int search_nodes;
    int tt_sides;
    uint16_t* leaf_moves;
    uint64_t* hist;
    RootResult* results;
    int* row_counter;
    int net_row_base;
    _Float16* x0;
    const float* logits;
    const float* values;
    int G;
    int L;
};

hipError_t launch_select(const TreeDev& d, const TreeCfg& c, hipStream_t st);
hipError_t launch_expand(const TreeDev& d, const TreeCfg& c, hipStream_t st);
hipError_t launch_advance(const TreeDev& d, const int* game_ids_dev, const int* child_slots_dev, int count, hipStream_t st);

hipError_t launch_encode_positions(const m0::Pos* pos_dev, int n, float* planes_f32_dev ,
                                   _Float16* nhwc_dev , uint8_t* mask_dev ,
                                   int32_t* nlegal_dev, uint16_t* moves_dev , int32_t* idx_dev ,
                                   hipStream_t st);

hipError_t launch_ssl_targets(const m0::Pos* pos_dev, int n, float* out_dev, hipStream_t st);
```

### matrix0_amd/csrc/tree_expand.hip

```cpp
#include "tree_device.h"
#include "eval_cache.h"

struct ExpandScratch {
    float pr[M0_MAX_CHILDREN];
    uint8_t keep[M0_MAX_CHILDREN];
    float total;
    int bad;
};

struct ExpandEnv {
    Arena A;
    int cap;
    GameDev* gd;
    uint64_t* TK; int* TN; int tt_cap;
    ExpandScratch* X;
    int lane;
};
struct LeafLogits {
    const float* row;
    const float* legal;
    float* store;
};
__device__ __forceinline__ LeafLogits logits_of_row(const float* row, float* store) { return LeafLogits{row, nullptr, store}; }
__device__ __forceinline__ LeafLogits logits_of_cache(const float* payload) { return LeafLogits{nullptr, payload + EC_LOGITS, nullptr}; }
constexpr int CPL = M0_MAX_CHILDREN / 64;
static_assert(M0_POLICY_SIZE % 4 == 0, "logit rows are read as 16-byte pieces");

static __device__ float np_sum_f32_dev(const float* a, int n) {
    auto block = [&](const float* b, int m) -> float {
        if (m < 8) { float r = 0.f; for (int i = 0; i < m; ++i) r += b[i]; return r; }
        float r[8];
        for (int j = 0; j < 8; ++j) r[j] = b[j];
        int i;
        for (i = 8; i < m - (m % 8); i += 8)
            for (int j = 0; j < 8; ++j) r[j] += b[i + j];
        float res = ((r[0] + r[1]) + (r[2] + r[3])) + ((r[4] + r[5]) + (r[6] + r[7]));
        for (; i < m; ++i) res += b[i];
        return res;
    };
    if (n <= 128) return block(a, n);
    int n2 = n / 2;
    n2 -= n2 % 8;
    return block(a, n2) + block(a + n2, n - n2);
}

__device__ __forceinline__ bool row_nonfinite(const float* lg, int lane) {
    constexpr int N4 = M0_POLICY_SIZE / 4, PER_LANE = (N4 + 63) / 64;
    const uint4* lg4 = reinterpret_cast<const uint4*>(lg);
    uint4 v[PER_LANE];
#pragma unroll
    for (int k = 0; k < PER_LANE; ++k) { const int j = lane + 64 * k; v[k] = lg4[j < N4 ? j : N4 - 1]; }
    uint32_t acc = 0;
#pragma unroll
    for (int k = 0; k < PER_LANE; ++k) {
        acc |= (uint32_t)((v[k].x & 0x7f800000u) == 0x7f800000u) | (uint32_t)((v[k].y & 0x7f800000u) == 0x7f800000u) |
               (uint32_t)((v[k].z & 0x7f800000u) == 0x7f800000u) | (uint32_t)((v[k].w & 0x7f800000u) == 0x7f800000u);
    }
    return acc != 0;
}

__device__ __forceinline__ void priors_raw(const float* lg, const int (&idx)[CPL], int n, int lane, ExpandScratch* X, float (&pr)[CPL]) {
#pragma unroll
    for (int k = 0; k < CPL; ++k) { const int i = lane + 64 * k; if (i < n) X->pr[i] = lg[idx[k]]; }
    __syncthreads();
    if (lane == 0) X->total = np_sum_f32_dev(X->pr, n);
    __syncthreads();
    const float total = X->total;
    const bool ok = isfinite(total) && total > 0.f;
#pragma unroll
    for (int k = 0; k < CPL; ++k) { const int i = lane + 64 * k; pr[k] = i < n ? (ok ? X->pr[i] / total : 1.0f / (float)n) : 0.f; }
    __syncthreads();
}

__device__ __forceinline__ void priors_uniform(int n, float (&pr)[CPL]) {
#pragma unroll
    for (int k = 0; k < CPL; ++k) pr[k] = 1.0f / (float)n;
}

__device__ __forceinline__ void priors_legal_softmax(const LeafLogits& src, const int (&idx)[CPL], int n, int lane, GameDev* gd,
                                                     const TreeCfg& c, float (&pr)[CPL]) {
    float mx = -3.0e38f;
    double ent = 0.0;
    float l[CPL];
#pragma unroll
    for (int k = 0; k < CPL; ++k) {
        const int i = lane + 64 * k;
        l[k] = i < n ? (src.legal ? src.legal[i] : src.row[idx[k]]) : -3.0e38f;
        mx = fmaxf(mx, l[k]);
        if (src.store && i < n && i < M0_EC_MAXLEGAL) src.store[EC_LOGITS + i] = l[k];
    }
    mx = wave_max_f(mx);
    double e[CPL], sum = 0.0;
#pragma unroll
    for (int k = 0; k < CPL; ++k) { const int i = lane + 64 * k; e[k] = i < n ? exp((double)(l[k] - mx)) : 0.0; sum += e[k]; }
    sum = wave_sum_d(sum);
#pragma unroll
    for (int k = 0; k < CPL; ++k) {
        const int i = lane + 64 * k;
        pr[k] = (float)(e[k] / sum);
        if (i < n) ent -= (double)pr[k] * log((double)pr[k] + 1e-8);
    }
    ent = wave_sum_d(ent);
    const double ratio = ent / fmax(1e-9, log((double)(n > 1 ? n : 1)));
    if (c.enable_entropy_noise && ratio > 0.9) {
        const uint64_t ctr = gd->ctr_noise;
        const uint64_t seed = gd->seed_noise;
        double dd[CPL], ds = 0.0;
#pragma unroll
        for (int k = 0; k < CPL; ++k) {
            const int i = lane + 64 * k;
            dd[k] = 0.0;
            if (i < n) { dd[k] = fmax((double)pr[k] + 0.1 * normal_at(seed, ctr + 2ull * (uint64_t)i), 1e-8); ds += dd[k]; }
        }
        ds = wave_sum_d(ds);
#pragma unroll
        for (int k = 0; k < CPL; ++k) pr[k] = (float)(dd[k] / ds);
        if (lane == 0) gd->ctr_noise = ctr + 2ull * (uint64_t)n;
    }
}

__device__ __forceinline__ void priors_full_softmax(const float* lg, const int (&idx)[CPL], int n, int lane, GameDev* gd,
                                                    const TreeCfg& c, float (&pr)[CPL]) {
    float mx = -3.0e38f;
    double ent = 0.0;
    for (int j = lane; j < M0_POLICY_SIZE; j += 64) mx = fmaxf(mx, lg[j]);
    mx = wave_max_f(mx);
    double sum = 0.0;
    for (int j = lane; j < M0_POLICY_SIZE; j += 64) sum += exp((double)(lg[j] - mx));
    sum = wave_sum_d(sum);
    const double fsum = sum;
    for (int j = lane; j < M0_POLICY_SIZE; j += 64) {
        const double pj = (double)(float)(exp((double)(lg[j] - mx)) / sum);
        ent -= pj * log(pj + 1e-8);
    }
#pragma unroll
    for (int k = 0; k < CPL; ++k) { const int i = lane + 64 * k; pr[k] = i < n ? (float)(exp((double)(lg[idx[k]] - mx)) / sum) : 0.f; }
    ent = wave_sum_d(ent);
    const double ratio = ent / fmax(1e-9, log((double)(n > 1 ? n : 1)));
    if (c.enable_entropy_noise && ratio > 0.9) {
        const uint64_t ctr = gd->ctr_noise;
        const uint64_t seed = gd->seed_noise;
        double ds = 0.0;
        for (int j = lane; j < M0_POLICY_SIZE; j += 64)
            ds += fmax((double)(float)(exp((double)(lg[j] - mx)) / fsum) + 0.1 * normal_at(seed, ctr + 2ull * (uint64_t)j), 1e-8);
        ds = wave_sum_d(ds);
#pragma unroll
        for (int k = 0; k < CPL; ++k) {
            const int i = lane + 64 * k;
            if (i < n) {
                const int j = idx[k];
                pr[k] = (float)(fmax((double)pr[k] + 0.1 * normal_at(seed, ctr + 2ull * (uint64_t)j), 1e-8) / ds);
            }
        }
        if (lane == 0) gd->ctr_noise = ctr + 2ull * (uint64_t)M0_POLICY_SIZE;
    }
}

__device__ __forceinline__ void priors_renormalise(int n, int lane, float (&pr)[CPL]) {
    double tot = 0.0;
#pragma unroll
    for (int k = 0; k < CPL; ++k) { const int i = lane + 64 * k; if (i < n) { if (!(pr[k] >= 0.f) || !isfinite(pr[k])) pr[k] = 0.f; tot += (double)pr[k]; } }
    tot = wave_sum_d(tot);
    const float totf = (float)tot;
    if (totf > 0.f && isfinite(totf)) {
#pragma unroll
        for (int k = 0; k < CPL; ++k) pr[k] = pr[k] / totf;
    } else priors_uniform(n, pr);
}

__device__ __forceinline__ int prune_children(const TreeCfg& c, const float (&pr)[CPL], int n, int lane, ExpandScratch* X, int (&slot)[CPL]) {
#pragma unroll
    for (int k = 0; k < CPL; ++k) slot[k] = lane + 64 * k;
    if (!(c.max_children > 0 || c.min_child_prior > 0.0)) return n;
#pragma unroll
    for (int k = 0; k < CPL; ++k) {
        const int i = lane + 64 * k;
        if (i < n) { X->pr[i] = pr[k]; X->keep[i] = (c.min_child_prior > 0.0 && !((double)pr[k] >= c.min_child_prior)) ? 0 : 1; }
    }
    __syncthreads();
    int kept = 0;
    for (int j = 0; j < n; ++j) kept += X->keep[j];
    const bool topk = c.max_children > 0 && kept > c.max_children;
    const int nkeep = topk ? c.max_children : kept;
#pragma unroll
    for (int k = 0; k < CPL; ++k) {
        const int i = lane + 64 * k;
        slot[k] = -1;
        if (i < n && X->keep[i]) {
            int r = 0;
            if (topk) { for (int j = 0; j < n; ++j) r += (X->keep[j] && (X->pr[j] > pr[k] || (X->pr[j] == pr[k] && j < i))) ? 1 : 0; }
            else { for (int j = 0; j < i; ++j) r += X->keep[j]; }
            if (r < nkeep) slot[k] = r;
        }
    }
    __syncthreads();
    return nkeep;
}

__device__ __forceinline__ bool write_children(const ExpandEnv& E, int leaf, const Pos& pos, const Move (&mvv)[CPL], const int (&idx)[CPL],
                                               const float (&pr)[CPL], const int (&slot)[CPL], int n, int nkeep, bool reg_children) {
    const Arena& A = E.A;
    GameDev* gd = E.gd;
    const int lane = E.lane;
    const int cb = gd->next;
    if (cb + nkeep > E.cap) { if (lane == 0) gd->overflow = 1; return false; }
#pragma unroll
    for (int k = 0; k < CPL; ++k) {
        const int i = lane + 64 * k;
        if (i < n && slot[k] >= 0) {
            const int ci = cb + slot[k];
            node_reset(A, ci, (double)pr[k], mvv[k], (uint16_t)idx[k]);
            if (E.TK && reg_children) {
                Pos q = pos;
                make_move(q, mvv[k]);
                tt_insert(E.TK, E.TN, E.tt_cap, tt_key_of(q), ci);
            }
        }
    }
    if (E.TK && !reg_children && lane == 0) tt_insert(E.TK, E.TN, E.tt_cap, tt_key_of(pos), leaf);
    if (lane == 0) { A.cbase[leaf] = cb; A.nch[leaf] = (int16_t)nkeep; gd->next = cb + nkeep; }
    __syncthreads();
    return true;
}

__device__ __forceinline__ bool expand_node(const ExpandEnv& E, const TreeCfg& c, int leaf, const Pos& pos, const uint16_t* smoves, int n,
                                   const LeafLogits& src, bool is_root, bool reg_children) {
    const int lane = E.lane;
    if (n <= 0) return true;
    bool bad = false;
    if (!src.legal) bad = row_nonfinite(src.row, lane);
    bad = __any(bad);
    if (lane == 0) E.X->bad = bad ? 1 : 0;
    float pr[CPL];
    int idx[CPL];
    Move mvv[CPL];
#pragma unroll
    for (int k = 0; k < CPL; ++k) {
        const int i = lane + 64 * k;
        pr[k] = 0.f; idx[k] = 0; mvv[k] = 0;
        if (i < n) { mvv[k] = smoves[i]; idx[k] = move_to_index(pos, mvv[k]); }
    }
    if (c.raw_legal_priors && c.legal_softmax && !is_root) priors_raw(src.row, idx, n, lane, E.X, pr);
    else if (bad) priors_uniform(n, pr);
    else {
        if (c.legal_softmax) priors_legal_softmax(src, idx, n, lane, E.gd, c, pr);
        else priors_full_softmax(src.row, idx, n, lane, E.gd, c, pr);
        priors_renormalise(n, lane, pr);
    }
    int slot[CPL];
    const int nkeep = prune_children(c, pr, n, lane, E.X, slot);
    return write_children(E, leaf, pos, mvv, idx, pr, slot, n, nkeep, reg_children);
}

__device__ __forceinline__ void expand_evaluated(const TreeDev& d, const TreeCfg& c, const ExpandEnv& E, int g, const Sample& smp,
                                                 const uint16_t* moves, const float* lg, float v) {
    const Arena& A = E.A;
    GameDev* gd = E.gd;
    const int lane = E.lane, kind = smp.kind, leaf = smp.leaf;
    const Pos pos = smp.pos;
    float* cw = nullptr;
    size_t ce = 0;
    const uint64_t ckey = kind == SK_EVAL ? smp.ckey : 0ull;
    if (ckey != 0 && isfinite(v)) {
        ce = ec_choose_victim(d.ec, gd, g, ckey, lane);
        cw = ec_payload(d.ec, ce);
        ec_invalidate(d.ec, ce, lane);
    }
    const bool ok = expand_node(E, c, leaf, pos, moves, smp.nlegal, logits_of_row(lg, cw), kind == SK_ROOT_INIT,
                                !(kind == SK_ROOT_INIT && gd->root_fresh));
    if (c.eval_cache && kind == SK_EVAL && lane == 0 && A.nch[leaf] < 0) A.cbase[leaf] = -1;
    const int sig = cw ? legal_sig(moves, smp.nlegal, lane) : 0;
    if (cw && lane == 0) {
        if (ok && !E.X->bad) ec_publish(d.ec, gd, ce, ckey, v, sig);
    }
}

__device__ __forceinline__ void release_inflight(const TreeDev& d, const TreeCfg& c, const Arena& A, int g, const Sample* S, const int* P,
                                                 int ns, int lane) {
    for (int s = lane; s < ns; s += 64) {
        if (sample_holds_inflight(S[s].kind)) {
            const int* path = (c.tt_merge ? d.epaths + (size_t)g * (d.L + 1) * M0_MAX_DEPTH : P) + (size_t)s * M0_MAX_DEPTH;
            for (int dd = 1; dd <= S[s].depth; ++dd) atomicSub(&A.vl[path[dd]], 1);
        }
    }
}

__device__ __forceinline__ void write_root_result(RootResult* R, const Arena& A, int root, int lane) {
    const int k = A.nch[root] > 0 ? A.nch[root] : 0;
    const int cb = A.cbase[root];
    for (int i = lane; i < k; i += 64) {
        R->child_node[i] = cb + i; R->child_n[i] = A.n[cb + i];
        R->child_mv[i] = A.mv[cb + i]; R->child_idx[i] = A.midx[cb + i];
        R->child_prior[i] = A.prior[cb + i]; R->child_q[i] = A.q[cb + i];
    }
    if (lane == 0) { R->nchild = k; R->root_n = A.n[root]; R->root_q = A.q[root]; }
}

__global__ __launch_bounds__(64) void expand_kernel(TreeDev d, TreeCfg c) {
    __shared__ ExpandScratch X;
    const int g = blockIdx.x, lane = threadIdx.x;
    GameDev* gd = &d.games[g];
    if (!gd->active) return;
    uint64_t* TK = c.tt_merge ? d.tt_keys + tt_table_of(d, g, gd) : nullptr;
    int* TN = c.tt_merge ? d.tt_nodes + tt_table_of(d, g, gd) : nullptr;
    const uint16_t* LM = d.leaf_moves + (size_t)g * (d.L + 1) * M0_MAX_CHILDREN;
    const int ns = gd->nsamples;
    if (ns <= 0) return;
    const Arena A = arena_of(d.t, g, gd->arena);
    const ExpandEnv E{A, d.t.cap, gd, TK, TN, d.tt_cap, &X, lane};
    const Sample* S = d.samples + (size_t)g * (d.L + 1);
    const int* P = d.paths + (size_t)g * (d.L + 1) * M0_MAX_DEPTH;
    const bool may_repeat = c.tt_merge != 0;
    int sims = 0;
    uint64_t evals = 0, hits = 0;
    for (int s = 0; s < ns; ++s) {
        const int kind = S[s].kind;
        const int* path = P + (size_t)s * M0_MAX_DEPTH;
        const uint16_t* moves = LM + (size_t)s * M0_MAX_CHILDREN;
        if (kind == SK_SHARED) {
            const float v = d.values[S[s].row];
            backprop(A, path, S[s].depth, (double)v, lane, may_repeat, NoMirror{});
            ++sims; ++hits;
            __syncthreads();
        } else if (kind == SK_CACHED) {
            const int leaf = S[s].leaf, depth = S[s].depth;
            const float* pay = ec_hit_stage(d, g, s);
            const float v = pay[EC_VALUE];
            if (A.nch[leaf] < 0) {
                const Pos pos = S[s].pos;
                expand_node(E, c, leaf, pos, moves, S[s].nlegal, logits_of_cache(pay), false, true);
            }
            backprop(A, path, depth, (double)v, lane, may_repeat, NoMirror{});
            ++sims; ++hits;
            __syncthreads();
        } else if (kind == SK_EVAL || kind == SK_ROOT_INIT) {
            const int leaf = S[s].leaf, depth = S[s].depth, row = S[s].row;
            const float* lg = d.logits + (size_t)row * M0_POLICY_SIZE;
            const float v = d.values[row];
            if (A.nch[leaf] < 0) expand_evaluated(d, c, E, g, S[s], moves, lg, v);
            ++evals;
            if (kind == SK_EVAL) {
                backprop(A, path, depth, (double)v, lane, may_repeat, NoMirror{});
                ++sims;
            } else {
                const double rv = root_value(gd, v);
                if (lane == 0) {
                    gd->root_v = rv;
                    if (gd->root_q_from_v) { A.q[leaf] = rv; gd->root_q_from_v = 0; }
                }
            }
            __syncthreads();
        } else if (kind == SK_TERMINAL) {
            ++sims;
        } else if (kind == SK_ROOT_VALUE) {
            const double rv = root_value(gd, d.values[S[s].row]);
            if (lane == 0) gd->root_v = rv;
            ++evals;
        }
    }
    if (c.virtual_loss_active) release_inflight(d, c, A, g, S, P, ns, lane);
    __syncthreads();
    const int done = gd->sims_done + sims;
    const int root = gd->root;
    const bool fin = (A.nch[root] >= 0 || gd->overflow) && done >= gd->sims_target;
    if (lane == 0) {
        gd->sims_done = done;
        gd->evals += evals;
        gd->cache_hits += hits;
        gd->finished = fin ? 1 : 0;
        gd->root_n = A.n[root];
        gd->root_q = A.q[root];
    }
    if (fin) write_root_result(d.results + g, A, root, lane);
}

hipError_t launch_expand(const TreeDev& d, const TreeCfg& c, hipStream_t st) {
    hipLaunchKernelGGL(expand_kernel, dim3(d.G), dim3(64), 0, st, d, c);
    return hipGetLastError();
}
```

Measured before the change: 1.135.

## Fork value head onto side stream and flag non-finite logit rows in GEMM epilogue

```diff
diff --git a/include/m0_engine.h b/include/m0_engine.h
--- a/include/m0_engine.h
+++ b/include/m0_engine.h
@@ -61,6 +61,7 @@
 int m0_net_load_weight(m0_net* net, const char* name, const void* data, int dtype, const int64_t* shape, int ndim);
 int m0_net_finalize(m0_net* net);
 int m0_net_infer(m0_net* net, const float* planes, int B, float* policy, float* value, float* ssl);
+int m0_net_debug_row_nonfinite(m0_net* net, uint32_t* out, int rows);
 int m0_net_ssl_channels(const m0_net* net);
 int64_t m0_net_param_count(const m0_net* net);
 double m0_net_flops_per_position(const m0_net* net, int with_ssl);
@@ -180,6 +181,7 @@
 int m0_search_begin(m0_selfplay* sp, int g, const char* fen, int sims, int dirichlet, int game_uid);
 int m0_search_select(m0_selfplay* sp, int* rows, float* planes, int max_rows);
 int m0_search_expand(m0_selfplay* sp, const float* logits, const float* values, int rows);
+int m0_search_expand_flagged(m0_selfplay* sp, const float* logits, const float* values, const uint32_t* row_nonfinite, int rows);
 int m0_search_result(m0_selfplay* sp, int g, int* nchild, int32_t* child_n, uint16_t* child_mv, int32_t* child_idx,
                      double* child_prior, double* child_q, double* root_q, int* root_n, int* finished);
 int m0_search_advance(m0_selfplay* sp, int g, int slot, int sims, int dirichlet);
diff --git a/matrix0_amd/csrc/capi_net.hip b/matrix0_amd/csrc/capi_net.hip
--- a/matrix0_amd/csrc/capi_net.hip
+++ b/matrix0_amd/csrc/capi_net.hip
@@ -157,6 +157,16 @@
     return M0_OK;
 }
 
+int m0_net_debug_row_nonfinite(m0_net* n, uint32_t* out, int rows) {
+    if (!n || !out || rows <= 0) { m0_set_error("invalid argument"); return M0_ERR_INVALID; }
+    std::lock_guard<std::mutex> lk(n->mu);
+    if (hipSetDevice(n->device) != hipSuccess) { m0_set_error("hipSetDevice failed"); return M0_ERR_HIP; }
+    if (!n->net->nonfinite_flags() || rows > n->net->workspace_rows()) { m0_set_error("more rows than the last forward's workspace holds"); return M0_ERR_INVALID; }
+    if (hipMemcpyAsync(out, n->net->nonfinite_flags(), (size_t)rows * 4, hipMemcpyDeviceToHost, n->stream) != hipSuccess ||
+        hipStreamSynchronize(n->stream) != hipSuccess) { m0_set_error("copy failed"); return M0_ERR_HIP; }
+    return M0_OK;
+}
+
 int m0_net_ssl_channels(const m0_net* n) { return n ? n->net->ssl_channels_total() : 0; }
 int64_t m0_net_param_count(const m0_net* n) { return n ? (int64_t)n->net->param_count() : 0; }
 double m0_net_flops_per_position(const m0_net* n, int with_ssl) { return n ? n->net->flops_per_position(with_ssl != 0) : 0.0; }
diff --git a/matrix0_amd/csrc/capi_selfplay.hip b/matrix0_amd/csrc/capi_selfplay.hip
--- a/matrix0_amd/csrc/capi_selfplay.hip
+++ b/matrix0_amd/csrc/capi_selfplay.hip
@@ -79,6 +79,7 @@
     sp->d.x0 = dalloc<_Float16>(sp, (size_t)(nreg * sp->rows_max + 4) * 64 * 32);
     sp->logits_dev = dalloc<float>(sp, (size_t)nreg * sp->rows_max * 4672);
     sp->values_dev = dalloc<float>(sp, (size_t)nreg * sp->rows_max + 4);
+    sp->nonfinite_dev = dalloc<uint32_t>(sp, (size_t)nreg * sp->rows_max + 4);
     sp->d.net_row_base = sp->rows_max;
     if (sp->cfg.ssl_in_forward && sp->net && sp->net->ssl_channels_total() > 0)
         sp->ssl_dev = dalloc<float>(sp, (size_t)sp->rows_max * sp->net->ssl_channels_total() * 64);
@@ -274,7 +275,7 @@
     sp->ext_pending = false;
     std::string err;
     (void)hipEventRecord(sp->ev0, sp->stream); (void)hipEventRecord(sp->ev1, sp->stream);
-    int rc = step_back(sp, rows_a + rows_b, now_ms(), err);
+    int rc = step_back(sp, rows_a + rows_b, now_ms(), err, nullptr);
     if (rc != M0_OK) m0_set_error(err);
     return rc;
 }
@@ -385,12 +386,21 @@
 }
 
 int m0_search_expand(m0_selfplay* sp, const float* logits, const float* values, int rows) {
+    return m0_search_expand_flagged(sp, logits, values, nullptr, rows);
+}
+
+int m0_search_expand_flagged(m0_selfplay* sp, const float* logits, const float* values, const uint32_t* row_nonfinite, int rows) {
     if (!sp) { m0_set_error("null argument"); return M0_ERR_INVALID; }
     std::lock_guard<std::mutex> lk(sp->mu);
     (void)hipSetDevice(sp->device);
     if (rows != sp->last_rows || rows > sp->rows_max) { m0_set_error("rows does not match the last select"); return M0_ERR_INVALID; }
     if (rows > 0 && (!logits || !values)) { m0_set_error("null argument"); return M0_ERR_INVALID; }
     upload_eval(sp, 0, logits, values, rows);
+    sp->d.row_nonfinite = nullptr;
+    if (row_nonfinite && rows > 0) {
+        (void)hipMemcpyAsync(sp->nonfinite_dev, row_nonfinite, (size_t)rows * 4, hipMemcpyHostToDevice, sp->stream);
+        sp->d.row_nonfinite = sp->nonfinite_dev;
+    }
     if (launch_expand(sp->d, sp->tc, sp->stream) != hipSuccess) { m0_set_error("expand launch failed"); return M0_ERR_HIP; }
     if (sync_games_d2h(sp) != 0) { m0_set_error(std::string("expand failed: ") + hipGetErrorString(hipGetLastError())); return M0_ERR_HIP; }
     sp->stats.evals += (uint64_t)rows;
diff --git a/matrix0_amd/csrc/net.h b/matrix0_amd/csrc/net.h
--- a/matrix0_amd/csrc/net.h
+++ b/matrix0_amd/csrc/net.h
@@ -72,7 +72,9 @@
     const std::vector<size_t>& device_buffer_bytes() const { return dev_sizes_; }
 
     int forward(const float* planes_dev, const _Float16* nhwc_dev, int B, float* logits_dev, float* value_dev,
-                float* ssl_dev, hipStream_t st, std::string& err);
+                float* ssl_dev, hipStream_t st, std::string& err, uint32_t* nonfinite_dev = nullptr);
+    const uint32_t* nonfinite_flags() const { return NF_; }
+    int workspace_rows() const { return wsM_; }
     int ensure_workspace(int B, std::string& err);
     int ssl_channels_total() const;
     const m0_net_cfg& cfg() const { return cfg_; }
@@ -92,7 +94,7 @@
     m0_net_cfg cfg_;
     int device_;
     hipStream_t stream_ = nullptr;
-    struct Switches { bool fuse_tail = true, fuse_attn = true; } sw_;
+    struct Switches { bool fuse_tail = true, fuse_attn = true, fork_heads = true; } sw_;
     struct Plan {
         bool fuse_tail = false;
         bool fuse_attn = false;
@@ -143,6 +145,11 @@
              *F3_ = nullptr, *F4_ = nullptr, *SH_ = nullptr, *SH2_ = nullptr, *SO_ = nullptr;
     float* VAL_ = nullptr;
     float* SPK_ = nullptr;
+    uint32_t* NF_ = nullptr;
+
+    hipStream_t side_ = nullptr;
+    hipEvent_t ev_fork_ = nullptr, ev_join_ = nullptr;
+    int ensure_side_stream(std::string& err);
 
     const HostTensor* get(const std::string& k, std::string& err);
     int pack_gemm(PackedGemm& g, const std::string& wkey, const std::string& bkey, int taps, int Cin_real,
diff --git a/matrix0_amd/csrc/net.hip b/matrix0_amd/csrc/net.hip
--- a/matrix0_amd/csrc/net.hip
+++ b/matrix0_amd/csrc/net.hip
@@ -28,6 +28,7 @@
     auto off = [](const char* name) { const char* e = getenv(name); return e && e[0] == '0'; };
     sw_.fuse_tail = !off("M0_FUSE_TAIL");
     sw_.fuse_attn = !off("M0_FUSE_ATTN");
+    sw_.fork_heads = !off("M0_FORK_HEADS");
     C_ = cfg.channels;
     Cp_ = (C_ > 256 && C_ < 320) ? 320 : C_;
     Cs_ = ceil_to(std::max(16, C_ / 2), 32);
@@ -54,10 +55,14 @@
     v->sd_.clear();
     v->pev_.clear(); v->pflop_.clear(); v->ptail_.clear(); v->pev_used_ = 0; v->profile_ = false;
     v->prof_ms_ = v->prof_flop_ = v->prof_tail_ms_ = 0; v->prof_launches_ = v->prof_tail_launches_ = 0;
+    v->side_ = nullptr; v->ev_fork_ = nullptr; v->ev_join_ = nullptr;
     return v;
 }
 
 Net::~Net() {
+    if (side_) { (void)hipStreamSynchronize(side_); (void)hipStreamDestroy(side_); }
+    if (ev_fork_) (void)hipEventDestroy(ev_fork_);
+    if (ev_join_) (void)hipEventDestroy(ev_join_);
     for (hipEvent_t e : pev_) (void)hipEventDestroy(e);
     for (void* p : dev_allocs_) (void)hipFree(p);
     for (void* p : ws_allocs_) (void)hipFree(p);
@@ -499,8 +504,9 @@
     SH_ = H(nb * 64 * Cs_); SH2_ = H(nb * 64 * Cs_); SO_ = H(nb * 64 * 32);
     VAL_ = F((size_t)Mfc * 32);
     SPK_ = F((size_t)8 * Mfc * ceil_to(2 * C_, 32));
+    NF_ = (uint32_t*)dalloc((size_t)Mfc * 4, true);
     if (!X0_ || !XA_ || !XB_ || !AA_ || !T1_ || !T2_ || !QKV_ || !O_ || !S1_ || !S2_ || !PH_ || !PH2_ || !VH_ ||
-        !VH2_ || !F1_ || !F2_ || !F3_ || !F4_ || !SH_ || !SH2_ || !SO_ || !VAL_ || !SPK_) {
+        !VH2_ || !F1_ || !F2_ || !F3_ || !F4_ || !SH_ || !SH2_ || !SO_ || !VAL_ || !SPK_ || !NF_) {
         err = "workspace hipMalloc failed";
         wsB_ = wsM_ = 0;
         return M0_ERR_HIP;
@@ -616,8 +622,19 @@
         }                                                                                 \
     } while (0)
 
+int Net::ensure_side_stream(std::string& err) {
+    if (side_) return M0_OK;
+    if (hipStreamCreateWithFlags(&side_, hipStreamNonBlocking) != hipSuccess ||
+        hipEventCreateWithFlags(&ev_fork_, hipEventDisableTiming) != hipSuccess ||
+        hipEventCreateWithFlags(&ev_join_, hipEventDisableTiming) != hipSuccess) {
+        err = "hipStreamCreate / hipEventCreate failed (forked heads)";
+        return M0_ERR_HIP;
+    }
+    return M0_OK;
+}
+
 int Net::forward(const float* planes_dev, const _Float16* nhwc_dev, int B, float* logits_dev, float* value_dev,
-                 float* ssl_dev, hipStream_t st, std::string& err) {
+                 float* ssl_dev, hipStream_t st, std::string& err, uint32_t* nonfinite_dev) {
     if (!finalized_) { err = "weights not finalized"; return M0_ERR_STATE; }
     if (B <= 0) { err = "batch must be positive"; return M0_ERR_INVALID; }
     TRY(ensure_workspace(B, err));
@@ -709,25 +726,38 @@
         KCHK(launch_conv_gemm(a, 1, st));
     } else {
         KCHK(conv_norm_act(ph_conv_, ph_n_, xa, PH2_, PH_, Mc, st));
+        KCHK(conv_norm_act(vh0_, vh1_n_, xa, VH2_, VH_, Mc, st));
+    }
+    hipStream_t vs = st;
+    if (sw_.fork_heads) {
+        TRY(ensure_side_stream(err));
+        KCHK(hipEventRecord(ev_fork_, st));
+        KCHK(hipStreamWaitEvent(side_, ev_fork_, 0));
+        vs = side_;
     }
     const bool factored = cfg_.policy_factor_rank > 0;
     if (factored) KCHK(run_gemm(pfc1_, gemm_args(pfc1_, PH2_, F1_, Mfc, ACT_RELU), st));
     const PackedGemm& plast = factored ? pfc2_ : pfc1_;
     GemmArgs pl = gemm_args(plast, factored ? F1_ : PH2_, logits_dev, Mfc);
     pl.Mvalid = B; pl.out_f32 = 1; pl.out_scale = logit_scale_;
+    pl.row_nonfinite = nonfinite_dev ? nonfinite_dev : NF_;
+    KCHK(hipMemsetAsync(pl.row_nonfinite, 0, (size_t)(nonfinite_dev ? B : Mfc) * 4, st));
     KCHK(run_gemm(plast, pl, st));
-    if (!joint) KCHK(conv_norm_act(vh0_, vh1_n_, xa, VH2_, VH_, Mc, st));
     _Float16* vflat = joint ? VH_ : VH2_;
-    KCHK(conv_norm_act(vh3_, vh4_n_, VH2_, vflat, VH_, Mc, st));
-    KCHK(run_gemm(vfc1_, gemm_args(vfc1_, vflat, F2_, Mfc, vact), st));
-    KCHK(run_gemm(vfc2_, gemm_args(vfc2_, F2_, F3_, Mfc, vact), st));
+    KCHK(conv_norm_act(vh3_, vh4_n_, VH2_, vflat, VH_, Mc, vs));
+    KCHK(run_gemm(vfc1_, gemm_args(vfc1_, vflat, F2_, Mfc, vact), vs));
+    KCHK(run_gemm(vfc2_, gemm_args(vfc2_, F2_, F3_, Mfc, vact), vs));
     GemmArgs vg = gemm_args(vgate_, F3_, F4_, Mfc, ACT_SIGMOID);
     vg.mul = F3_;
-    KCHK(run_gemm(vgate_, vg, st));
+    KCHK(run_gemm(vgate_, vg, vs));
     GemmArgs v3 = gemm_args(vfc3_, F4_, VAL_, Mfc, ACT_TANH);
     v3.out_f32 = 1;
-    KCHK(run_gemm(vfc3_, v3, st));
-    KCHK(hipMemcpy2DAsync(value_dev, 4, VAL_, 32 * 4, 4, B, hipMemcpyDeviceToDevice, st));
+    KCHK(run_gemm(vfc3_, v3, vs));
+    KCHK(hipMemcpy2DAsync(value_dev, 4, VAL_, 32 * 4, 4, B, hipMemcpyDeviceToDevice, vs));
+    if (vs != st) {
+        KCHK(hipEventRecord(ev_join_, vs));
+        KCHK(hipStreamWaitEvent(st, ev_join_, 0));
+    }
     if (ssl_dev && !ssl_.empty()) {
         const int ctot = ssl_channels_total();
         int coff = 0;
diff --git a/matrix0_amd/csrc/net_kernels.h b/matrix0_amd/csrc/net_kernels.h
--- a/matrix0_amd/csrc/net_kernels.h
+++ b/matrix0_amd/csrc/net_kernels.h
@@ -40,6 +40,7 @@
     void* out2;
     int ldo2;
     int nsplit;
+    uint32_t* row_nonfinite;
 };
 
 struct EwArgs {
diff --git a/matrix0_amd/csrc/net_kernels.hip b/matrix0_amd/csrc/net_kernels.hip
--- a/matrix0_amd/csrc/net_kernels.hip
+++ b/matrix0_amd/csrc/net_kernels.hip
@@ -1,7 +1,7 @@
 #include "kernel_common.h"
 #include "conv_epilogue.h"
 
-template <int TAPS, int WN, int NT, int KC, int EPI = 0, int ACT = 0>
+template <int TAPS, int WN, int NT, int KC, int EPI = 0, int ACT = 0, int NF = 0>
 __global__ __launch_bounds__(256 * WN) void conv_gemm_kernel(GemmArgs a) {
     constexpr int NB = WN * NT * 32;
     constexpr int NTHR = 256 * WN;
@@ -203,6 +203,9 @@
                 if (row < a.Mvalid) {
                     if (f32out) reinterpret_cast<float*>(a.out)[(size_t)row * ldo + col] = v;
                     else reinterpret_cast<_Float16*>(a.out)[(size_t)row * ldo + col] = (_Float16)v;
+                    if constexpr (NF != 0) {
+                        if ((__float_as_uint(v) & 0x7f800000u) == 0x7f800000u) a.row_nonfinite[row] = 1u;
+                    }
                 }
             });
         });
@@ -229,18 +232,18 @@
     return main_loop > staging ? main_loop : staging;
 }
 
-template <int TAPS, int WN, int NT, int KC, int EPI = 0, int ACT = 0>
+template <int TAPS, int WN, int NT, int KC, int EPI = 0, int ACT = 0, int NF = 0>
 static hipError_t launch_conv_gemm_t(const GemmArgs& a, hipStream_t st) {
     constexpr int NB = WN * NT * 32;
     size_t lds = conv_gemm_lds<TAPS, WN, NT, KC>(a.Cin);
     static DeviceOnce once;
     hipError_t e = once.run([] {
-        return hipFuncSetAttribute(reinterpret_cast<const void*>(&conv_gemm_kernel<TAPS, WN, NT, KC, EPI, ACT>),
+        return hipFuncSetAttribute(reinterpret_cast<const void*>(&conv_gemm_kernel<TAPS, WN, NT, KC, EPI, ACT, NF>),
                                    hipFuncAttributeMaxDynamicSharedMemorySize, 160 * 1024);
     });
     if (e != hipSuccess) return e;
     dim3 grid(a.Mrows / 256, a.Npad / NB);
-    hipLaunchKernelGGL((conv_gemm_kernel<TAPS, WN, NT, KC, EPI, ACT>), grid, dim3(256 * WN), lds, st, a);
+    hipLaunchKernelGGL((conv_gemm_kernel<TAPS, WN, NT, KC, EPI, ACT, NF>), grid, dim3(256 * WN), lds, st, a);
     return hipGetLastError();
 }
 template <int ACT>
@@ -270,6 +273,7 @@
 hipError_t launch_conv_gemm(const GemmArgs& a, int taps, hipStream_t st) {
     if (a.Mrows % 256 != 0 || a.Cin % 32 != 0 || a.Npad % 32 != 0) return hipErrorInvalidValue;
     const bool big = conv_gemm_tile_n(a.Cin, a.Npad) == 320;
+    if (a.row_nonfinite != nullptr && (big || taps != 1 || a.gn_gamma != nullptr || !a.out_f32)) return hipErrorInvalidValue;
     if (a.gn_gamma != nullptr && !big) {
         if (a.epi_act == ACT_SILU) return launch_conv_gemm_gn<ACT_SILU>(a, taps, st);
         if (a.epi_act == ACT_RELU) return launch_conv_gemm_gn<ACT_RELU>(a, taps, st);
@@ -283,8 +287,9 @@
         return launch_conv_gemm_t<9, 1, 1, 32>(a, st);
     } else if (taps == 1) {
         if (big) return a.w_pp ? hipErrorInvalidValue : launch_conv_big(a, 1, st);
-        if (a.Mrows / 256 >= 256 && a.Npad % 64 == 0) return launch_conv_gemm_t<1, 1, 2, 32>(a, st);
-        return launch_conv_gemm_t<1, 1, 1, 32>(a, st);
+        const bool wide = a.Mrows / 256 >= 256 && a.Npad % 64 == 0;
+        if (a.row_nonfinite != nullptr) return wide ? launch_conv_gemm_t<1, 1, 2, 32, 0, 0, 1>(a, st) : launch_conv_gemm_t<1, 1, 1, 32, 0, 0, 1>(a, st);
+        return wide ? launch_conv_gemm_t<1, 1, 2, 32>(a, st) : launch_conv_gemm_t<1, 1, 1, 32>(a, st);
     }
     return hipErrorInvalidValue;
 }
diff --git a/matrix0_amd/csrc/selfplay.hip b/matrix0_amd/csrc/selfplay.hip
--- a/matrix0_amd/csrc/selfplay.hip
+++ b/matrix0_amd/csrc/selfplay.hip
@@ -318,8 +318,9 @@
     if (sp->counted) g_engines_with_net[sp->device].fetch_sub(1);
 }
 
-int step_back(m0_selfplay* sp, int rows, double t0, std::string& err) {
+int step_back(m0_selfplay* sp, int rows, double t0, std::string& err, const uint32_t* row_nonfinite) {
     (void)hipEventRecord(sp->ev2, sp->stream);
+    sp->d.row_nonfinite = row_nonfinite;
     if (launch_expand(sp->d, sp->tc, sp->stream) != hipSuccess) { err = "expand launch failed"; return M0_ERR_HIP; }
     (void)hipEventRecord(sp->ev3, sp->stream);
     if (sync_games_d2h(sp) != 0) { err = std::string("step failed: ") + hipGetErrorString(hipGetLastError()); return M0_ERR_HIP; }
@@ -389,12 +390,13 @@
         m0_net_lock(sp->nethandle);
         int rc = M0_OK;
         if (tail_rows > 0) (void)hipEventRecord(sp->ev_sel, sp->stream);
-        rc = sp->net->forward(nullptr, sp->d.x0, main_rows, sp->logits_dev, sp->values_dev, ssl, sp->stream, err);
+        rc = sp->net->forward(nullptr, sp->d.x0, main_rows, sp->logits_dev, sp->values_dev, ssl, sp->stream, err, sp->nonfinite_dev);
         if (rc == M0_OK && tail_rows > 0) {
             (void)hipStreamWaitEvent(sp->stream_tail, sp->ev_sel, 0);
             const size_t sslw = ssl ? (size_t)sp->net->ssl_channels_total() * 64 : 0;
             rc = sp->net_tail->forward(nullptr, sp->d.x0 + (size_t)main_rows * 64 * 32, tail_rows, sp->logits_dev + (size_t)main_rows * 4672,
-                                       sp->values_dev + main_rows, ssl ? ssl + (size_t)main_rows * sslw : nullptr, sp->stream_tail, err);
+                                       sp->values_dev + main_rows, ssl ? ssl + (size_t)main_rows * sslw : nullptr, sp->stream_tail, err,
+                                       sp->nonfinite_dev + main_rows);
             (void)hipEventRecord(sp->ev_tail, sp->stream_tail);
             (void)hipStreamWaitEvent(sp->stream, sp->ev_tail, 0);
         }
@@ -407,13 +409,13 @@
         const size_t b = (size_t)sp->d.net_row_base;
         m0_net_lock(sp->nethandle_b);
         int rc = sp->net_b->forward(nullptr, sp->d.x0 + b * 64 * 32, sp->rows2[1], sp->logits_dev + b * 4672,
-                                    sp->values_dev + b, nullptr, sp->stream, err);
+                                    sp->values_dev + b, nullptr, sp->stream, err, sp->nonfinite_dev + b);
         m0_net_unlock(sp->nethandle_b);
         if (rc != M0_OK) return rc;
         rows += sp->rows2[1];
     }
     gate.release();
-    return step_back(sp, rows, t0, err);
-}
-
-}
+    return step_back(sp, rows, t0, err, sp->nonfinite_dev);
+}
+
+}
diff --git a/matrix0_amd/csrc/selfplay_engine.h b/matrix0_amd/csrc/selfplay_engine.h
--- a/matrix0_amd/csrc/selfplay_engine.h
+++ b/matrix0_amd/csrc/selfplay_engine.h
@@ -71,6 +71,7 @@
     std::vector<RootResult> hres;
     float* logits_dev = nullptr;
     float* values_dev = nullptr;
+    uint32_t* nonfinite_dev = nullptr;
     float* ssl_dev = nullptr;
     m0::Pos* ssl_pos_dev = nullptr;
     float* ssl_out_dev = nullptr;
@@ -116,6 +117,6 @@
 int start_first_games(m0_selfplay* sp);
 int run_select(m0_selfplay* sp, int* rows_out);
 int one_step(m0_selfplay* sp, std::string& err);
-int step_back(m0_selfplay* sp, int rows, double t0, std::string& err);
+int step_back(m0_selfplay* sp, int rows, double t0, std::string& err, const uint32_t* row_nonfinite);
 
 }
diff --git a/matrix0_amd/csrc/tree.h b/matrix0_amd/csrc/tree.h
--- a/matrix0_amd/csrc/tree.h
+++ b/matrix0_amd/csrc/tree.h
@@ -141,6 +141,7 @@
     _Float16* x0;
     const float* logits;
     const float* values;
+    const uint32_t* row_nonfinite;
     int G;
     int L;
 };
diff --git a/matrix0_amd/csrc/tree_expand.hip b/matrix0_amd/csrc/tree_expand.hip
--- a/matrix0_amd/csrc/tree_expand.hip
+++ b/matrix0_amd/csrc/tree_expand.hip
@@ -20,9 +20,12 @@
     const float* row;
     const float* legal;
     float* store;
+    const uint32_t* nonfinite;
 };
-__device__ __forceinline__ LeafLogits logits_of_row(const float* row, float* store) { return LeafLogits{row, nullptr, store}; }
-__device__ __forceinline__ LeafLogits logits_of_cache(const float* payload) { return LeafLogits{nullptr, payload + EC_LOGITS, nullptr}; }
+__device__ __forceinline__ LeafLogits logits_of_row(const float* row, float* store, const uint32_t* nonfinite) {
+    return LeafLogits{row, nullptr, store, nonfinite};
+}
+__device__ __forceinline__ LeafLogits logits_of_cache(const float* payload) { return LeafLogits{nullptr, payload + EC_LOGITS, nullptr, nullptr}; }
 constexpr int CPL = M0_MAX_CHILDREN / 64;
 static_assert(M0_POLICY_SIZE % 4 == 0, "logit rows are read as 16-byte pieces");
 
@@ -228,7 +231,7 @@
     const int lane = E.lane;
     if (n <= 0) return true;
     bool bad = false;
-    if (!src.legal) bad = row_nonfinite(src.row, lane);
+    if (!src.legal) bad = src.nonfinite ? *src.nonfinite != 0u : row_nonfinite(src.row, lane);
     bad = __any(bad);
     if (lane == 0) E.X->bad = bad ? 1 : 0;
     float pr[CPL];
@@ -253,7 +256,7 @@
 }
 
 __device__ __forceinline__ void expand_evaluated(const TreeDev& d, const TreeCfg& c, const ExpandEnv& E, int g, const Sample& smp,
-                                                 const uint16_t* moves, const float* lg, float v) {
+                                                 const uint16_t* moves, const float* lg, const uint32_t* nonfinite, float v) {
     const Arena& A = E.A;
     GameDev* gd = E.gd;
     const int lane = E.lane, kind = smp.kind, leaf = smp.leaf;
@@ -266,7 +269,7 @@
         cw = ec_payload(d.ec, ce);
         ec_invalidate(d.ec, ce, lane);
     }
-    const bool ok = expand_node(E, c, leaf, pos, moves, smp.nlegal, logits_of_row(lg, cw), kind == SK_ROOT_INIT,
+    const bool ok = expand_node(E, c, leaf, pos, moves, smp.nlegal, logits_of_row(lg, cw, nonfinite), kind == SK_ROOT_INIT,
                                 !(kind == SK_ROOT_INIT && gd->root_fresh));
     if (c.eval_cache && kind == SK_EVAL && lane == 0 && A.nch[leaf] < 0) A.cbase[leaf] = -1;
     const int sig = cw ? legal_sig(moves, smp.nlegal, lane) : 0;
@@ -337,7 +340,7 @@
             const int leaf = S[s].leaf, depth = S[s].depth, row = S[s].row;
             const float* lg = d.logits + (size_t)row * M0_POLICY_SIZE;
             const float v = d.values[row];
-            if (A.nch[leaf] < 0) expand_evaluated(d, c, E, g, S[s], moves, lg, v);
+            if (A.nch[leaf] < 0) expand_evaluated(d, c, E, g, S[s], moves, lg, d.row_nonfinite ? d.row_nonfinite + row : nullptr, v);
             ++evals;
             if (kind == SK_EVAL) {
                 backprop(A, path, depth, (double)v, lane, may_repeat, NoMirror{});
```

New measurement: 1.135. No clear change (-0.1%).
